# mala-lab/GGAD

Hardware: AMD Instinct MI355X
Metric: training nodes/sec (DGraph-Fin mini-batch GGAD) (higher is better)
Workload: dtype f32; 1 GPU; DGraph-Fin-size synthetic graph, mini-batch GGAD (GCN encoder); nodes=3700550, directed_entries=72953930, feat=17, emb=64, batch=150+50, graph=powerlaw(alpha=2.1,max_degree=2000), chunk_batches=150, hop2=ldsw, overlap=False, dense_cus=0, chain=0, dense_steps=XCD-resident chunk kernel: one launch per chunk on 28 CUs of one XCD, parallelism=dp1, optimizer=adam(lr=1e-3,wd=0.007), batch_streams=the reference's stream

## Files before the change

### ggad_amd/_lib.py

```python
from __future__ import annotations

import ctypes
import os
from ctypes import POINTER, c_char_p, c_float, c_int32, c_int64, c_uint32, c_uint64, c_void_p

HERE = os.path.dirname(os.path.abspath(__file__))
LIB_PATH = os.environ.get("GGAD_LIB_PATH") or os.path.join(HERE, "libggad_hip.so")


class GgadLibraryError(RuntimeError):
    pass


GGAD_OK, GGAD_E_INVALID, GGAD_E_LAUNCH, GGAD_E_CAPACITY, GGAD_E_UNSUPPORTED = 0, -1, -2, -3, -4


class GgadKernelError(RuntimeError):
    pass


GEMM_ROUTES = ("NONE", "SLAB", "BRES", "WGRAD_TN", "SMALL", "DMA", "DMA_SPLITK", "TILED", "TILED_SPLITK")


def gemm_last_route():
    v = int(load().ggad_gemm_last_route())
    return GEMM_ROUTES[v & 0xFF], v >> 8


ABI_VERSION = 11
_P = c_void_p
EXCHANGE_CB = ctypes.CFUNCTYPE(c_int32, c_void_p)
_I = c_int32
_L = c_int64
_F = c_float

SIGNATURES = {
    "ggad_abi_version": (c_int32, []),
    "ggad_last_error": (c_char_p, []),
    "ggad_max_embed_dim": (c_int32, []),
    "ggad_max_feat_dim": (c_int32, []),
    "ggad_mb_wide_max_embed_dim": (c_int32, []),
    "ggad_mb_wide_supported": (c_int32, [c_int32, c_int32]),
    "ggad_mb_supported": (c_int32, [c_int32, c_int32]),
    "ggad_scan_workspace_elems": (c_int64, [_L]),
    "ggad_exclusive_scan_i32": (c_int32, [_P, _P, _L, _P, _P]),
    "ggad_mb_chunk_len": (c_int32, []),
    "ggad_mb_slice_len": (c_int32, []),
    "ggad_mb_group_words": (c_int32, []),
    "ggad_mb_item_words": (c_int32, []),
    "ggad_mb_set_gather_options": (c_int32, [c_int32, c_int32]),
    "ggad_mb_plan_counter_elems": (c_int32, []),
    "ggad_mb_plan_build": (c_int32, [_P, _P, _P, _I, _P, _P, _P, _P, _P, _P]),
    "ggad_event_create": (c_int32, [_I, _P]),
    "ggad_event_destroy": (c_int32, [_P]),
    "ggad_event_record": (c_int32, [_P, _P]),
    "ggad_event_synchronize": (c_int32, [_P]),
    "ggad_event_elapsed_ms": (c_int32, [_P, _P, _P]),
    "ggad_mb_count2": (c_int32, [_P, _P, _P, _P, _P, _L, _L, _P, _P, _P]),
    "ggad_mb_gather2": (c_int32, [_P, _P, _P, _I, _I, _P, _P, _P, _P, _L, _L, _P, _P, _P]),
    "ggad_mb_plan_reset": (c_int32, [_P, _P, _P, _P, _P, _P, _L, _L, _P, _P, _I, _P]),
    "ggad_mb_tile_offsets_elems": (c_int64, [_L, _I]),
    "ggad_mb_tile_offsets": (c_int32, [_P, _P, _L, _I, _P, _P]),
    "ggad_mb_tile_major_workspace_elems": (c_int64, [_L, _I]),
    "ggad_mb_tile_major": (c_int32, [_P, _P, _L, _I, _P, _P, _P, _P, _P]),
    "ggad_mb_ldsw_tile_shift": (c_int32, []),
    "ggad_mb_ldsw_max_owners": (c_int32, []),
    "ggad_mb_ldsw_seg_elems": (c_int64, [_L, _L]),
    "ggad_mb_dw_part_elems": (c_int64, [_I, _I, _I]),
    "ggad_mb_train_chunk": (c_int32, [_P, _I, _P, _P, _P, _P, _I, _I, _P]),
    "ggad_mb_train_chunk_dp": (c_int32, [_P, _I, _P, _P, _P, _P, _I, c_float, EXCHANGE_CB, _P, _P]),
    "ggad_stream_create_cu_mask": (c_int32, [_P, _I, _P]),
    "ggad_stream_destroy": (c_int32, [_P]),
    "ggad_device_cu_count": (c_int32, [_I, _P]),
    "ggad_xchg_create": (c_int32, [_I, _I, _L, _P]),
    "ggad_xchg_handle_bytes": (c_int32, []),
    "ggad_xchg_handle": (c_int32, [_P, _P]),
    "ggad_xchg_connect": (c_int32, [_P, _P]),
    "ggad_xchg_error": (c_int32, [_P, _P]),
    "ggad_xchg_destroy": (c_int32, [_P]),
    "ggad_xchg_adam": (c_int32, [_P, _P, _P, _P, _I, _I, _F, _F, _F, _P, _P, _P]),
    "ggad_mb_train_chunk_xchg": (c_int32, [_P, _I, _P, _P, _P, _P, _I, c_float, _P, _P]),
    "ggad_mb_xcd_grid": (c_int32, []),
    "ggad_xcd_first_of_stream": (c_int32, [_P, _P]),
    "ggad_mb_xcd_workspace_elems": (c_int64, [_I, _I, _I, _L, _L]),
    "ggad_mb_train_chunk_xcd": (c_int32, [_P, _I, _P, _I, _I, _I, _I, _L, _L, _P, _I, _P, c_float, _P, _I, _P, _P]),
    "ggad_mb_xcd_record_elems": (c_int64, [_L, _L]),
    "ggad_mb_xcd_prepare": (c_int32, [_P, _I, _P, _I, _I, _I, _L, _L, _P, _P]),
    "ggad_mb_xcd_status": (c_int32, [_P, _P, _P]),
    "ggad_mb_xcd_clear_error": (c_int32, [_P, _I, _P]),
    "ggad_mb_param_count": (c_int64, [_I, _I]),
    "ggad_mb_param_block_elems": (c_int64, [_I, _I]),
    "ggad_mb_params_sync": (c_int32, [_P, _I, _I, _P]),
    "ggad_mb_project": (c_int32, [_P, _I, _I, _P, _P, _I, _I, _P, _P]),
    "ggad_mb_fwd_rows": (c_int32, [_P, _I, _I, _P, _P, _P, _P, _P, _I, _I, _I, _P, _P, _P, _P]),
    "ggad_mb_loss_workspace_elems": (c_int64, [_I]),
    "ggad_mb_loss": (c_int32, [_P, _I, _I, _P, _P, _P, _P, _P, _P, _P, _I, _I, _P, _P, _P, _P, _P, _P, _P, _P, _P, _P]),
    "ggad_mb_row_coefs": (c_int32, [_P, _I, _I, _P, _P, _I, _I, _P, _P, _P, _P, _P, _P, _P, _P, _P]),
    "ggad_mb_bwd_parts": (c_int32, []),
    "ggad_mb_bwd_flat": (c_int32, [_I, _I, _P, _P, _P, _P, _P, _I, _I, _I, _I, _P, _P, _P, _P]),
    "ggad_mb_grad_reduce": (c_int32, [_I, _I, _P, _I, _I, _P, _P, _P, _P, _P, _P, _P]),
    "ggad_mb_adam": (c_int32, [_P, _P, _P, _P, _I, _I, _F, _F, _F, _P, _P]),
    "ggad_mb_train_step": (c_int32, [_P, _I, _P]),
    "ggad_mb_encode": (c_int32, [_P, _I, _I, _P, _I, _P, _P]),
    "ggad_seg_mean": (c_int32, [_P, _I, _P, _P, _I, _P, _P]),
    "ggad_seg_wsum": (c_int32, [_P, _I, _P, _P, _P, _I, _P, _P]),
# ... 277 lines not shown
```

### ggad_amd/build.py

```python
from __future__ import annotations

import hashlib
import os
import shutil
import subprocess
import sys

HERE = os.path.dirname(os.path.abspath(__file__))
CSRC = os.path.join(HERE, "csrc")
LIB = os.path.join(HERE, "libggad_hip.so")
STAMP = os.path.join(HERE, ".libggad_hip.stamp")
SOURCES = ["runtime.cpp", "plan_build.cpp", "exchange.cpp", "sampler.cpp", "sampler_x86.cpp", "spmm_panel_build.cpp", "spmm_ring_build.cpp", "plan.hip", "hop2_ldsw.hip", "step.hip", "step_wide.hip", "step_xcd.hip", "fullgraph.hip", "gemm.hip", "gemm_slab.hip", "mlp.hip", "baselines.hip", "anomalydae.hip", "aegis.hip", "gaan.hip", "dominant.hip", "rng.hip", "pcgnn.hip", "pcgnn_head.hip", "sage.hip", "aegis_mb.hip", "recon_mb.hip", "tam.hip", "tam_nsgt.hip", "rank_metrics.hip", "topk.hip", "select.hip", "explain.hip"]
HOST_ONLY = {"sampler.cpp", "sampler_x86.cpp", "spmm_panel_build.cpp", "spmm_ring_build.cpp"}
HEADERS = ["common.h", "handoff.h", "step_common.h", "rank_common.h", "libggad_hip.map", os.path.join("..", "..", "include", "ggad_hip.h")]
FLAGS = ["--offload-arch=gfx950", "-O3", "-std=c++17", "-fPIC", "-ffp-contract=on", "-fno-fast-math",
         "-Wall", "-Wno-unused-function"] + os.environ.get("GGAD_EXTRA_HIPFLAGS", "").split()


def _hipcc() -> str:
    for c in (shutil.which("hipcc"), "/opt/rocm/bin/hipcc"):
        if c and os.path.exists(c):
            return c
    raise RuntimeError("hipcc not found; libggad_hip.so cannot be built")


def _digest(srcs) -> str:
    h = hashlib.sha256()
    for name in list(srcs) + HEADERS:
        with open(os.path.join(CSRC, name), "rb") as fh:
            h.update(fh.read())
    h.update(" ".join(FLAGS).encode())
    return h.hexdigest()


def build(force: bool = False, verbose: bool = True) -> str:
    srcs = [s for s in SOURCES if os.path.exists(os.path.join(CSRC, s))]
    dig = _digest(srcs)
    if not force and os.path.exists(LIB) and os.path.exists(STAMP) and open(STAMP).read().strip() == dig:
        return LIB
    hipcc = _hipcc()
    objs = []
    bdir = os.path.join(HERE, "build")
    os.makedirs(bdir, exist_ok=True)
    procs = []
    for s in srcs:
        obj = os.path.join(bdir, os.path.splitext(s)[0] + ".o")
        objs.append(obj)
        if s in HOST_ONLY:
            cmd = [hipcc, "-O3", "-std=c++17", "-fPIC", "-Wall", "-x", "c++", "-c", os.path.join(CSRC, s), "-o", obj]
        else:
            cmd = [hipcc] + FLAGS + ["-x", "hip", "-c", os.path.join(CSRC, s), "-o", obj]
        if verbose:
            print("[ggad build]", " ".join(cmd), flush=True)
        procs.append((s, subprocess.Popen(cmd)))
    for s, p in procs:
        if p.wait() != 0:
            raise RuntimeError(f"hipcc failed on {s}")
    cmd = [hipcc, "--offload-arch=gfx950", "-shared", "-fPIC", "-Wl,--version-script=" + os.path.join(CSRC, "libggad_hip.map"), "-o", LIB] + objs
    if verbose:
        print("[ggad build]", " ".join(cmd), flush=True)
    subprocess.check_call(cmd)
    with open(STAMP, "w") as fh:
        fh.write(dig)
    return LIB


if __name__ == "__main__":
# ... 2 lines not shown
```

### ggad_amd/csrc/common.h

```cpp
#pragma once
#include <hip/hip_runtime.h>
#include <stdint.h>
#include <mutex>
#include "../../include/ggad_hip.h"

#define GGAD_WAVE 64
#define GGAD_MAX_D 64
#define GGAD_MAX_F 1024

void ggad_set_error(hipError_t e, const char *where);

#define GGAD_CHECK_LAUNCH(where)                 \
  do {                                           \
    hipError_t _e = hipGetLastError();           \
    if (_e != hipSuccess) {                      \
      ggad_set_error(_e, where);                 \
      return GGAD_E_LAUNCH;                      \
    }                                            \
  } while (0)

#define GGAD_REQUIRE(cond) \
  do {                     \
    if (!(cond)) return GGAD_E_INVALID; \
  } while (0)
// ... 23 lines not shown
#pragma unroll
  for (int off = 32; off >= 1; off >>= 1) v += __shfl_xor(v, off, GGAD_WAVE);
  return v;
}
__device__ __forceinline__ int wave_sum_i(int v) {
#pragma unroll
  for (int off = 32; off >= 1; off >>= 1) v += __shfl_xor(v, off, GGAD_WAVE);
  return v;
}

__device__ __forceinline__ void ggad_adam_elem(float &pi, float &mi, float &vi, float g, float wd, float sc0, float sc1) {
  float gi = fmaf(wd, pi, g);
  mi = fmaf(gi - mi, 0.1f, mi);
  vi = fmaf(0.001f * gi, gi, vi * 0.999f);
  const float denom = sqrtf(vi) / sc1 + 1e-8f;
  pi = pi - sc0 * (mi / denom);
}

__device__ __forceinline__ int lower_bound_i32(const int32_t *__restrict__ a, int lo, int hi, int key) {
  while (lo < hi) {
    int mid = (lo + hi) >> 1;
    if (a[mid] < key) lo = mid + 1; else hi = mid;
  }
  return lo;
}

__device__ __forceinline__ bool ggad_vblock(int skip, unsigned &vb, unsigned &vg) {
  const unsigned b = blockIdx.x, n = gridDim.x;
  if (skip < 0) { vb = b; vg = n; return true; }
  const unsigned sk = (unsigned)skip;
  if ((b & 7u) == sk) return false;
  vb = b - ((b >> 3) + ((b & 7u) > sk ? 1u : 0u));
  vg = n - ((n >> 3) + ((n & 7u) > sk ? 1u : 0u));
  return true;
}
static inline unsigned ggad_skip_grid(unsigned want, int skip) { return skip < 0 ? want : (unsigned)(((uint64_t)(want + 1) * 8 + 6) / 7); }

constexpr int GGAD_CTR_STRIDE = 16;
constexpr int GGAD_CTR_GROUPS = 0 * GGAD_CTR_STRIDE, GGAD_CTR_ITEMS = 1 * GGAD_CTR_STRIDE, GGAD_CTR_PART = 2 * GGAD_CTR_STRIDE,
              GGAD_CTR_CURSOR = 3 * GGAD_CTR_STRIDE, GGAD_CTR_PC = 4 * GGAD_CTR_STRIDE,
              GGAD_CTR_BIG = 5 * GGAD_CTR_STRIDE,
              GGAD_CTR_RANGE0 = 6 * GGAD_CTR_STRIDE,
              GGAD_CTR_PROF = 14 * GGAD_CTR_STRIDE;
constexpr int GGAD_RANGES = 8;
constexpr int GGAD_RANGE_DEG = 256;
constexpr int GGAD_PLAN_COUNTERS = 16 * GGAD_CTR_STRIDE;

struct ggad_plan_view {
  const int32_t *batch_ptr, *batch_ent_ptr, *nodes, *row_slot, *ent_ptr, *row_ck_ptr, *ck_rc, *ck_e0;
  int32_t n_batches, n_rows, n_ents, n_chunks;
  int32_t seg_stride;
  int64_t pair_bound;
};
int ggad_int_hop1(const ggad_mb_plan *P, const ggad_plan_view &V, int ldsw, int reset_now, hipStream_t st);
int ggad_int_global_hop2(const ggad_mb_plan *P, const ggad_plan_view &V, hipStream_t st, hipEvent_t ev0, hipEvent_t ev1);
int ggad_int_ldsw_hop2(const ggad_mb_plan *P, const ggad_plan_view &V, hipStream_t st, hipEvent_t ev0, hipEvent_t ev1);
int ggad_int_range_deg();

int ggad_int_gemm_slab(const float *A, const float *B, float *C, int M, int N, int K, int64_t lda, int64_t sbk, int64_t sbn, int64_t ldc,
                       const float *bias, int relu, hipStream_t st, const float *prelu_a = nullptr, float *C2 = nullptr, int64_t ldc2 = 0);

int64_t ggad_int_wgrad_tn_ws(int R, int m, int n);
int ggad_int_wgrad_tn(const float *P, int64_t ldp, const float *Q, int64_t ldq, int R, int m, int n, float *D, float *ws, hipStream_t st,
                      int *vpq = nullptr);

constexpr int GGAD_MB_BWD_PARTS = 256;
struct ggad_xchg_view;
bool ggad_int_wide_ok(int D, int F);
int ggad_int_wide_project(const float *params, int32_t D, int32_t F, const float *x2, const int32_t *ent_own, int32_t ent0,
                          int32_t n_ents, float *h2, ggad_stream_t stream);
int ggad_int_wide_fwd_rows(const float *params, int32_t D, int32_t F, const float *x1, const float *h2, const int32_t *ent_ptr,
                           const int32_t *ent_own, const int32_t *labels, int32_t row0, int32_t n_rows, int32_t ent0, float *h1,
                           float *nbar, float *gen, ggad_stream_t stream);
int ggad_int_wide_loss(const float *params, int32_t D, int32_t F, const float *h1, const float *nbar, const float *gen,
                       const int32_t *labels, const int32_t *pos_meta, const int32_t *row_pos, const int32_t *ent_ptr,
                       int32_t row0, int32_t n_rows, float *loss_ws, float *losses8, float *d_h1, float *d_gen, float *d_nbar,
                       float *dz, float *coef_a, float *coef_g, int32_t *step_counter, ggad_stream_t stream);
int ggad_int_wide_row_coefs(const float *params, int32_t D, int32_t F, const int32_t *labels, const int32_t *ent_ptr,
                            int32_t row0, int32_t n_rows, const float *h1, const float *gen, const float *d_h1,
                            const float *d_gen, const float *d_nbar, float *dz, float *coef_a, float *coef_g,
                            ggad_stream_t stream);
int ggad_int_wide_bwd_flat(int32_t D, int32_t F, const float *x1, const float *x2, const float *h2, const int32_t *ent_own,
                           const int32_t *ent_row, int32_t row0, int32_t n_rows, int32_t ent0, int32_t n_ents,
                           const float *coef_a, const float *coef_g, float *dw_part, ggad_stream_t stream);
int ggad_int_wide_grad_reduce(int32_t D, int32_t F, const int32_t *pos_meta, int32_t row0, int32_t n_rows, const float *losses8,
                              const float *nbar, const float *dw_part, const float *dz, const float *loss_ws, float *grads,
                              int mode, float *params, float *m, float *v, float lr, float wd, const int32_t *step_counter,
                              const ggad_xchg_view *xv, uint32_t xstep, float grad_scale, ggad_stream_t stream);
int ggad_int_wide_rows(const float *params, int32_t D, int32_t F, const float *x1, int32_t n_rows, float *out, int score,
                       ggad_stream_t stream);

constexpr int GGAD_XCHG_MAX_WORLD = 16;
struct ggad_xchg_view {
  float *peer[GGAD_XCHG_MAX_WORLD];
  int32_t rank, world;
  int64_t n;
  int32_t *err;
  unsigned long long timeout_ticks;
};
struct ggad_xchg {
  ggad_xchg_view view;
  void *local;
  size_t bytes;
  uint32_t step;
  bool opened[GGAD_XCHG_MAX_WORLD];
};
static inline size_t ggad_xchg_granules(int world, int64_t n) { return (size_t)2 * world * (size_t)n; }
```

### ggad_amd/csrc/hop2_ldsw.hip

```cpp
#include <algorithm>
#include <atomic>
#include <climits>
#include <mutex>

#include "common.h"

namespace {

#ifdef GGAD_G2_PROF
struct G2Prof { unsigned long long a[8], t; };
#define G2_ARG , G2Prof &prof
#define G2_PASS , prof
#define G2_MARK(i) do { __builtin_amdgcn_sched_barrier(0); __builtin_amdgcn_s_waitcnt(0); const unsigned long long t_ = wall_clock64(); \
                        prof.a[i] += t_ - prof.t; prof.t = t_; __builtin_amdgcn_sched_barrier(0); } while (0)
#define TC_MARK(i) do { __syncthreads(); if (threadIdx.x == 0) { const unsigned long long t_ = wall_clock64(); tcp[i] += t_ - tct; tct = t_; } } while (0)
#else
#define G2_ARG
#define G2_PASS
#define G2_MARK(i)
#define TC_MARK(i)
#endif

constexpr int SLICE = 256;
constexpr int GRP_W = 10;
constexpr int ITEM_GRAB = 4;

__global__ void __launch_bounds__(256) k_tile_offsets(const int32_t *__restrict__ rowptr, const int32_t *__restrict__ col,
                                                      int64_t n_nodes, int n_tiles, int shift, int32_t *__restrict__ off) {
  const int64_t u = (int64_t)blockIdx.x * blockDim.x + threadIdx.x;
  if (u >= n_nodes) return;
  const int s = rowptr[u], e = rowptr[u + 1];
  int32_t *o = off + u * (n_tiles + 1);
  int t = 0;
  for (int i = s; i < e; ++i) {
    const int tile = col[i] >> shift;
    while (t <= tile) { o[t] = i - s; ++t; }
  }
  while (t <= n_tiles) { o[t] = e - s; ++t; }
}

__global__ void __launch_bounds__(256) k_tm_blocksum(const int32_t *__restrict__ off, int64_t n_nodes, int n_tiles, int32_t *__restrict__ bsum) {
  __shared__ int wsum[4][64];
  const int lane = lane_id(), w = threadIdx.x >> 6;
  const int NT1 = n_tiles + 1;
  const int64_t u0 = (int64_t)blockIdx.x * 256 + 64 * w;
  for (int t0 = 0; t0 < n_tiles; t0 += 64) {
    const int t = t0 + lane;
    int acc = 0;
    if (t < n_tiles)
      for (int i = 0; i < 64 && u0 + i < n_nodes; ++i) { const int32_t *o = off + (u0 + i) * NT1 + t; acc += o[1] - o[0]; }
    wsum[w][lane] = acc;
    __syncthreads();
    if (w == 0 && t < n_tiles) bsum[(int64_t)blockIdx.x * n_tiles + t] = wsum[0][lane] + wsum[1][lane] + wsum[2][lane] + wsum[3][lane];
    __syncthreads();
  }
}

__global__ void __launch_bounds__(1024) k_tm_scan(int32_t *__restrict__ bsum, int64_t n_blocks, int n_tiles, int32_t *__restrict__ tile_base) {
// ... 10 lines not shown
    }
    for (; b < n_blocks; ++b) { const int v = bsum[b * n_tiles + t]; bsum[b * n_tiles + t] = run; run += v; }
    tot[t] = run;
  }
  __syncthreads();
  if (threadIdx.x == 0) {
    int run = 0;
    for (int t = 0; t < n_tiles; ++t) { tile_base[t] = run; run += tot[t]; }
    tile_base[n_tiles] = run;
  }
}

__global__ void __launch_bounds__(256) k_tm_fill(const int32_t *__restrict__ rowptr, const int32_t *__restrict__ col,
                                                 const int32_t *__restrict__ off, int64_t n_nodes, int n_tiles,
                                                 const int32_t *__restrict__ bsum, const int32_t *__restrict__ tile_base,
                                                 int32_t *__restrict__ tile_start, int32_t *__restrict__ col_t) {
  __shared__ int wsum[4][64];
  const int lane = lane_id(), w = threadIdx.x >> 6;
  const int NT1 = n_tiles + 1;
  const int64_t u0 = (int64_t)blockIdx.x * 256 + 64 * w;
  for (int t0 = 0; t0 <= n_tiles; t0 += 64) {
    const int t = t0 + lane;
    int acc = 0;
    if (t < n_tiles)
      for (int i = 0; i < 64 && u0 + i < n_nodes; ++i) { const int32_t *o = off + (u0 + i) * NT1 + t; acc += o[1] - o[0]; }
    wsum[w][lane] = acc;
    __syncthreads();
    if (t < n_tiles) {
      int pos = tile_base[t] + bsum[(int64_t)blockIdx.x * n_tiles + t];
      for (int ww = 0; ww < w; ++ww) pos += wsum[ww][lane];
      for (int i = 0; i < 64 && u0 + i < n_nodes; ++i) {
        const int64_t u = u0 + i;
        const int32_t *o = off + u * NT1 + t;
        const int o0 = o[0], o1 = o[1];
        tile_start[u * NT1 + t] = pos;
        const int32_t *src = col + rowptr[u] + o0;
        for (int j = 0; j < o1 - o0; ++j) col_t[pos + j] = src[j];
        pos += o1 - o0;
      }
    } else if (t == n_tiles) {
      for (int i = 0; i < 64 && u0 + i < n_nodes; ++i) tile_start[(u0 + i) * NT1 + t] = 0;
    }
    __syncthreads();
  }
}

constexpr int TW_SHIFT = 15;
constexpr int TW_TILE = 1 << TW_SHIFT;
constexpr int TW_MAXOWN = 6144;
constexpr int TW_T = 1024;
constexpr int TW_BRK = 1536;

constexpr int TT_SLAB = 128;
__global__ void __launch_bounds__(256) k_seg_transpose(const int32_t *__restrict__ tile_off, const int32_t *__restrict__ tile_start,
                                                       int n_tiles, const int32_t *__restrict__ ent_own,
                                                       const int32_t *__restrict__ ent_col, int n_ents, int64_t seg_stride,
                                                       int32_t *__restrict__ seg_t, int skip) {
  __shared__ int tl[TT_SLAB][65];
  unsigned vbx, vgx;
  if (!ggad_vblock(skip, vbx, vgx)) return;
  const int p0 = vbx * 64;
  if (p0 >= n_ents) return;
  const int lane = lane_id(), wid = threadIdx.x >> 6;
  const int NT1 = n_tiles + 1;
  int u_l = 0, own_l = 0;
  if (p0 + lane < n_ents) { own_l = ent_own[p0 + lane] == p0 + lane ? 1 : 0; u_l = own_l ? ent_col[p0 + lane] : 0; }
  for (int which = 0; which < (tile_start ? 2 : 1); ++which) {
  const int32_t *table = which ? tile_start : tile_off;
  int32_t *plane = seg_t + (which ? (int64_t)NT1 * seg_stride : 0);
  for (int t0 = 0; t0 < NT1; t0 += TT_SLAB) {
    int v0[16], v1[16];
    const int c0 = min(t0 + lane, NT1 - 1), c1 = min(t0 + 64 + lane, NT1 - 1);
#pragma unroll
    for (int jj = 0; jj < 16; ++jj) {
      const int j = wid + 4 * jj;
      const int u = __shfl(u_l, j, GGAD_WAVE);
      const int32_t *row = table + (int64_t)u * NT1;
      v0[jj] = row[c0];
      v1[jj] = row[c1];
    }
#pragma unroll
    for (int jj = 0; jj < 16; ++jj) {
      const int j = wid + 4 * jj;
      const int own = __shfl(own_l, j, GGAD_WAVE);
      if (t0 + lane < NT1) tl[lane][j] = own ? v0[jj] : 0;
      if (t0 + 64 + lane < NT1) tl[64 + lane][j] = own ? v1[jj] : 0;
    }
    __syncthreads();
    const int nt = min(TT_SLAB, NT1 - t0);
    for (int idx = threadIdx.x; idx < nt * 64; idx += 256) {
      const int tt = idx >> 6, j = idx & 63;
      if (p0 + j < n_ents) plane[(int64_t)(t0 + tt) * seg_stride + p0 + j] = tl[tt][j];
    }
    __syncthreads();
  }
  }
}

__device__ __forceinline__ int block_excl_scan_1024(int v, int *warp_buf, int *total) {
  const int lane = lane_id(), wid = threadIdx.x >> 6;
  int inc = v;
#pragma unroll
  for (int off = 1; off < 64; off <<= 1) {
    const int t = __shfl_up(inc, off, 64);
    if (lane >= off) inc += t;
  }
  if (lane == 63) warp_buf[wid] = inc;
  __syncthreads();
  int base = 0, tot = 0;
#pragma unroll
  for (int w = 0; w < 16; ++w) { const int sv = warp_buf[w]; if (w < wid) base += sv; tot += sv; }
  __syncthreads();
  *total = tot;
  return base + inc - v;
}

__global__ void __launch_bounds__(TW_T) k_tile_counts(const int32_t *__restrict__ col, const int32_t *__restrict__ seg_t,
                                                      int64_t n_cap, const int32_t *__restrict__ own_rp,
                                                      const int32_t *__restrict__ batch_ent_ptr,
                                                      const int32_t *__restrict__ pw_base, uint16_t *__restrict__ pc, int n_tiles,
                                                      int n_batches, int32_t *__restrict__ counters, int skip, int tile_major) {
  extern __shared__ __attribute__((aligned(16))) uint32_t lds_u[];
  uint32_t *cnt = lds_u;
  int *offs = reinterpret_cast<int *>(lds_u + TW_TILE / 2);
  int *segbeg = offs + TW_MAXOWN + 1;
  int *dst = segbeg + TW_MAXOWN;
  int *brk = dst + TW_MAXOWN;
  __shared__ int wbuf[16];
  unsigned vbx, vgx;
  if (!ggad_vblock(skip, vbx, vgx)) return;
  int t, b;
  const bool class_map = (tile_major & 2) != 0;
  tile_major &= 1;
  if (class_map) {
    const int nx = skip < 0 ? 8 : 7, c = (int)(blockIdx.x & 7u);
    const int ci = c - ((skip >= 0 && c > skip) ? 1 : 0);
    const unsigned j = blockIdx.x >> 3;
    const int nt_c = ci < n_tiles ? (n_tiles - ci + nx - 1) / nx : 0;
    if (j >= (unsigned)nt_c * (unsigned)n_batches) return;
    t = ci + nx * (int)(j / (unsigned)n_batches);
    b = (int)(j % (unsigned)n_batches);
  } else {
    if (vbx >= (unsigned)n_tiles * (unsigned)n_batches) return;
    t = (int)(vbx % (unsigned)n_tiles); b = (int)(vbx / (unsigned)n_tiles);
  }
  const int o0 = batch_ent_ptr[b], o1 = batch_ent_ptr[b + 1];
  const int n_own_all = o1 - o0;
  const int32_t *seg_lo = seg_t + (int64_t)t * n_cap, *seg_hi = seg_lo + n_cap;
  const int32_t *seg_st = tile_major ? seg_t + (int64_t)(n_tiles + 1 + t) * n_cap : own_rp;
// ... 286 lines not shown
    const bool mine = blk + lane < n1;
    lids[lane] = k_nx;
    __builtin_amdgcn_fence(__ATOMIC_RELEASE, "wavefront");
    __builtin_amdgcn_wave_barrier();
    int id[16];
#pragma unroll
    for (int c = 0; c < 4; ++c) {
      const mi4 iv = *reinterpret_cast<const mi4 *>(lids + 16 * g + 4 * c);
#pragma unroll
      for (int q = 0; q < 4; ++q) id[4 * c + q] = iv[q];
    }
    mf2 x[16];
#pragma unroll
    for (int i = 0; i < 16; ++i) x[i] = *reinterpret_cast<const mf2 *>(fb + ((uint32_t)id[i] << 7));
#pragma unroll
    for (int j = 0; j < G; ++j)
      lw[j * MF_WS + lane] = (j < n_occ && mine) ? inv_sr / sqrtf((float)c_nx[j]) : 0.0f;
    __builtin_amdgcn_fence(__ATOMIC_RELEASE, "wavefront");
    __builtin_amdgcn_wave_barrier();
    float wa[16];
#pragma unroll
    for (int c = 0; c < 4; ++c) {
      const mf4 wv = *reinterpret_cast<const mf4 *>(lw + aa * MF_WS + 16 * g + 4 * c);
#pragma unroll
      for (int q = 0; q < 4; ++q) wa[4 * c + q] = a < G ? wv[q] : 0.0f;
    }
    __builtin_amdgcn_wave_barrier();
    {
      const int ix = min(blk + 64 + lane, last);
      k_nx = col[s + ix];
#pragma unroll
      for (int j = 0; j < G; ++j) c_nx[j] = pc[pb[j] + ix];
    }
    G2_MARK(3);
#pragma unroll
    for (int i = 0; i < 16; ++i) {
      acc0 = __builtin_amdgcn_mfma_f32_16x16x4f32(wa[i], x[i].x, acc0, 0, 0, 0);
      acc1 = __builtin_amdgcn_mfma_f32_16x16x4f32(wa[i], x[i].y, acc1, 0, 0, 0);
    }
    G2_MARK(4);
  }
#pragma unroll
  for (int j = 0; j < G; ++j) {
    const int src = (lane >> 1) + 16 * (j >> 2);
    const float v0 = __shfl(acc0[j & 3], src & 63, GGAD_WAVE), v1 = __shfl(acc1[j & 3], src & 63, GGAD_WAVE);
    tot[j] = (lane & 1) ? v1 : v0;
  }
}

__device__ __forceinline__ int range_tile(int r, int n_tiles) { return (int)(((int64_t)r * n_tiles) / GGAD_RANGES); }

__global__ void __launch_bounds__(256) k_build_groups(const int32_t *__restrict__ ent_own, const int32_t *__restrict__ ent_col,
                                                      const int32_t *__restrict__ own_deg, int n_ents,
                                                      int32_t *__restrict__ node_head, const int32_t *__restrict__ own_next,
                                                      const int32_t *__restrict__ tile_off, int n_tiles,
                                                      int32_t *__restrict__ grp, int32_t *__restrict__ items,
                                                      int32_t *__restrict__ big, int32_t *__restrict__ gbnd,
                                                      int32_t *__restrict__ counters, int range_deg, int skip) {
  unsigned vbx, vgx;
  if (!ggad_vblock(skip, vbx, vgx)) return;
  const int e = vbx * 256 + threadIdx.x;
  const int lane = lane_id();
  int u = 0, m = 0, ng = 0, ns = 0, deg = 0;
  if (e < n_ents && ent_own[e] == e) {
    u = ent_col[e];
    if (node_head[u] == e + 1) {
      for (int cur = e + 1; cur != 0; cur = own_next[cur - 1]) ++m;
      ng = (m + 7) >> 3;
      deg = own_deg[e];
      ns = deg > range_deg ? GGAD_RANGES : (deg > SLICE ? (deg + SLICE - 1) / SLICE : 1);
    }
  }
  const bool is_big = deg > range_deg;
  const int c1 = is_big ? 0 : ng * ns, c2 = ns > 1 ? m * ns : 0, c3 = is_big ? ng : 0;
  int v0 = ng, v1 = c1, v2 = c2, v3 = c3;
#pragma unroll
  for (int off = 1; off < GGAD_WAVE; off <<= 1) {
    const int t0 = __shfl_up(v0, off, GGAD_WAVE), t1 = __shfl_up(v1, off, GGAD_WAVE), t2 = __shfl_up(v2, off, GGAD_WAVE),
              t3 = __shfl_up(v3, off, GGAD_WAVE);
    if (lane >= off) { v0 += t0; v1 += t1; v2 += t2; v3 += t3; }
  }
  __shared__ int wg_tot[4][5];
  const int wid = threadIdx.x >> 6;
  if (lane == GGAD_WAVE - 1) { wg_tot[0][wid] = v0; wg_tot[1][wid] = v1; wg_tot[2][wid] = v2; wg_tot[3][wid] = v3; }
  __syncthreads();
  if (threadIdx.x < 4) {
    const int k = threadIdx.x;
    int sum = 0;
    for (int w = 0; w < 4; ++w) { const int t = wg_tot[k][w]; wg_tot[k][w] = sum; sum += t; }
    int32_t *ctr = counters + (k == 0 ? GGAD_CTR_GROUPS : (k == 1 ? GGAD_CTR_ITEMS : (k == 2 ? GGAD_CTR_PART : GGAD_CTR_BIG)));
    wg_tot[k][4] = sum > 0 ? atomicAdd(ctr, sum) : 0;
  }
  __syncthreads();
  const int b0 = wg_tot[0][4] + wg_tot[0][wid], b1 = wg_tot[1][4] + wg_tot[1][wid], b2 = wg_tot[2][4] + wg_tot[2][wid],
            b3 = wg_tot[3][4] + wg_tot[3][wid];
  if (ng == 0) return;
  const int gbase = b0 + v0 - ng, ibase = b1 + v1 - c1, pbase = b2 + v2 - c2, bbase = b3 + v3 - c3;
  int bnd[GGAD_RANGES + 1];
  if (is_big) {
    const int32_t *row = tile_off + (int64_t)u * (n_tiles + 1);
#pragma unroll
    for (int r = 0; r <= GGAD_RANGES; ++r) bnd[r] = row[range_tile(r, n_tiles)];
  }
  int cur = e + 1;
  for (int g = 0; g < ng; ++g) {
    int32_t *rec = grp + (int64_t)(gbase + g) * GRP_W;
#pragma unroll
    for (int j = 0; j < 8; ++j) {
      int v = -1;
      if (cur != 0) { v = cur - 1; cur = own_next[v]; }
      rec[j] = v;
    }
    rec[8] = pbase + g * 8 * ns;
    rec[9] = ns;
    if (is_big) {
      big[bbase + g] = gbase + g;
      int32_t *bo = gbnd + (int64_t)(bbase + g) * (GGAD_RANGES + 1);
#pragma unroll
      for (int r = 0; r <= GGAD_RANGES; ++r) bo[r] = bnd[r];
    } else {
      for (int sl = 0; sl < ns; ++sl) {
        int32_t *it = items + (int64_t)(ibase + sl * ng + g) * 2;
        it[0] = gbase + g;
        it[1] = sl;
      }
    }
  }
  node_head[u] = 0;
}

template <int FT, bool MF>
__global__ void __launch_bounds__(256) k_gather2_items(const int32_t *__restrict__ col, const float *__restrict__ feat, int F_rt,
                                                       int stride, const int32_t *__restrict__ own_rp,
                                                       const int32_t *__restrict__ own_deg, const int32_t *__restrict__ pw_base,
                                                       const uint16_t *__restrict__ pc, const int32_t *__restrict__ grp,
                                                       const int32_t *__restrict__ items, const int32_t *__restrict__ big,
                                                       const int32_t *__restrict__ gbnd, int32_t *__restrict__ counters,
                                                       float *__restrict__ x2, float *__restrict__ part2, int affine, int take_cap, int skip) {
  static_assert(ITEM_GRAB == 4 && GRP_W <= 10, "lane layout of the metadata loads: 16 lanes per item of a grab (10, 11: range bounds)");
  unsigned vbx, vgx;
  if (!ggad_vblock(skip, vbx, vgx)) return;
  const int F = FT ? FT : F_rt;
  const int lane = lane_id();
  __shared__ __attribute__((aligned(16))) float mf_lds[MF ? 4 * MF_LDS : 4];
  float *lw = mf_lds + (MF ? (threadIdx.x >> 6) * MF_LDS : 0);
  const int n_small = counters[GGAD_CTR_ITEMS], n_big = counters[GGAD_CTR_BIG];
  const int q_l = lane >> 4, r_l = lane & 15;
  unsigned xcc;
  asm volatile("s_getreg_b32 %0, hwreg(HW_REG_XCC_ID)" : "=s"(xcc));
  xcc &= GGAD_RANGES - 1;
  if (!affine) xcc = (vbx / GGAD_RANGES) & (GGAD_RANGES - 1);
  const int n_waves_all = (int)vgx * 4;
#ifdef GGAD_G2_PROF
  G2Prof prof = {};
  const unsigned long long t_begin = wall_clock64();
  prof.t = t_begin;
#endif
  for (int ph = 0; ph <= GGAD_RANGES; ++ph) {
    const int cls = ph == 0 ? (int)xcc : (ph == 1 ? GGAD_RANGES : (int)((xcc + ph - 1) & (GGAD_RANGES - 1)));
    const bool bigc = cls < GGAD_RANGES;
    const int n_items = bigc ? n_big : n_small;
    if (n_items == 0) continue;
    int32_t *cursor = counters + (bigc ? GGAD_CTR_RANGE0 + cls * GGAD_CTR_STRIDE : GGAD_CTR_CURSOR);
// ... 45 lines not shown
#pragma unroll
      for (int j = 0; j < 8; ++j) {
        e[j] = __builtin_amdgcn_readlane(rv, q * 16 + j);
        pb[j] = __builtin_amdgcn_readlane(pbv, q * 16 + j);
        n += e[j] >= 0 ? 1 : 0;
      }
      const int pbase = __builtin_amdgcn_readlane(rv, q * 16 + 8), ns = __builtin_amdgcn_readlane(rv, q * 16 + 9);
      const int sl = __builtin_amdgcn_readlane(iv, q * 16 + 1);
      int s, n0, n1, deg;
      item_span(q, s, n0, n1, deg);
      const float inv_sr = 1.0f / sqrtf((float)deg);
      const int k_first = k_ahead;
      if (q + 1 < ITEM_GRAB && base + q + 1 < last) {
        int s_, a_, b_, d_;
        item_span(q + 1, s_, a_, b_, d_);
        k_ahead = first_ids(s_, a_, b_);
      }
      float tot[8];
      if (MF) {
        if (n == 1) { float t1[1]; gather_slice_mfma<1>(col, feat, s, n0, n1, inv_sr, n, pb, pc, lane, lw, k_first, t1 G2_PASS); tot[0] = t1[0]; }
        else if (n == 2) { float t2[2]; gather_slice_mfma<2>(col, feat, s, n0, n1, inv_sr, n, pb, pc, lane, lw, k_first, t2 G2_PASS); tot[0] = t2[0]; tot[1] = t2[1]; }
        else if (n <= 4) { float t4[4]; gather_slice_mfma<4>(col, feat, s, n0, n1, inv_sr, n, pb, pc, lane, lw, k_first, t4 G2_PASS);
#pragma unroll
          for (int j = 0; j < 4; ++j) tot[j] = t4[j]; }
        else gather_slice_mfma<8>(col, feat, s, n0, n1, inv_sr, n, pb, pc, lane, lw, k_first, tot G2_PASS);
      } else
      if (n == 1) { float t1[1]; gather_slice<1, FT>(col, feat, F, stride, s, n0, n1, inv_sr, n, pb, pc, lane, k_first, t1 G2_PASS); tot[0] = t1[0]; }
      else if (n == 2) { float t2[2]; gather_slice<2, FT>(col, feat, F, stride, s, n0, n1, inv_sr, n, pb, pc, lane, k_first, t2 G2_PASS); tot[0] = t2[0]; tot[1] = t2[1]; }
      else if (n <= 4) { float t4[4]; gather_slice<4, FT>(col, feat, F, stride, s, n0, n1, inv_sr, n, pb, pc, lane, k_first, t4 G2_PASS);
#pragma unroll
        for (int j = 0; j < 4; ++j) tot[j] = t4[j]; }
      else gather_slice<8, FT>(col, feat, F, stride, s, n0, n1, inv_sr, n, pb, pc, lane, k_first, tot G2_PASS);
#pragma unroll
      for (int j = 0; j < 8; ++j) {
        if (j < n && lane < F) {
          if (ns == 1) x2[(int64_t)e[j] * F + lane] = (deg == 0) ? inv_sr * 0.0f : tot[j];
          else part2[((int64_t)pbase + (int64_t)j * ns + sl) * F + lane] = tot[j];
        }
      }
      G2_MARK(5);
    }
    }
  }
  }
#ifdef GGAD_G2_PROF
  if (lane == 0) {
    prof.a[6] = wall_clock64() - t_begin;
    unsigned long long *out = reinterpret_cast<unsigned long long *>(counters + GGAD_CTR_PROF);
    for (int k = 0; k < 7; ++k) atomicAdd(out + k, prof.a[k]);
  }
#endif
}

__global__ void __launch_bounds__(256) k_gather2_combine(const int32_t *__restrict__ grp, const int32_t *__restrict__ counters,
                                                         const float *__restrict__ part2, int F, float *__restrict__ x2, int skip) {
  unsigned vbx, vgx;
  if (!ggad_vblock(skip, vbx, vgx)) return;
  const int lane = lane_id();
  const int n_groups = counters[GGAD_CTR_GROUPS];
  const int rpi = 64 / F;
  const int g = lane / F, f = lane - g * F;
  for (int gi = vbx * 4 + (threadIdx.x >> 6); gi < n_groups; gi += vgx * 4) {
    const int rv = (lane < GRP_W) ? grp[(int64_t)gi * GRP_W + lane] : -1;
    const int ns = __builtin_amdgcn_readlane(rv, 9);
    if (ns <= 1) continue;
    const int pbase = __builtin_amdgcn_readlane(rv, 8);
    for (int j0 = 0; j0 < 8; j0 += rpi) {
      const int j = j0 + g;
      const int ej = __shfl(rv, j & 7, GGAD_WAVE);
      if (g < rpi && j < 8 && ej >= 0) {
        float acc = 0.0f;
#pragma unroll 4
        for (int sl = 0; sl < ns; ++sl) acc += part2[((int64_t)pbase + (int64_t)j * ns + sl) * F + f];
        x2[(int64_t)ej * F + f] = acc;
      }
    }
  }
}

__global__ void __launch_bounds__(256) k_gather2_w(const int32_t *__restrict__ col, const float *__restrict__ feat, int F, int stride,
                                                   const int32_t *__restrict__ ent_own, int n_ents,
                                                   const int32_t *__restrict__ own_rp, const int32_t *__restrict__ own_deg,
                                                   const int32_t *__restrict__ pw_base, const uint16_t *__restrict__ pc,
                                                   float *__restrict__ x2, int skip) {
  unsigned vbx, vgx;
  if (!ggad_vblock(skip, vbx, vgx)) return;
  const int e0 = vbx * 4 + (threadIdx.x >> 6);
  if (e0 >= n_ents || ent_own[e0] != e0) return;
  const int lane = lane_id();
  const int s = own_rp[e0];
  const int deg = own_deg[e0];
  const int pb0 = pw_base[e0];
  const float inv_sr = 1.0f / sqrtf((float)deg);
  if (F <= 64) {
    const int pb[8] = {pb0, 0, 0, 0, 0, 0, 0, 0};
    float total = 0.0f;
#ifdef GGAD_G2_PROF
    G2Prof prof = {};
#endif
    for (int n0 = 0; n0 < deg; n0 += SLICE) {
      float t1[1];
      const int kf = col[s + min(n0 + lane, max(min(deg, n0 + SLICE) - 1, 0))];
      if (F == 17) gather_slice<1, 17>(col, feat, F, stride, s, n0, min(deg, n0 + SLICE), inv_sr, 1, pb, pc, lane, kf, t1 G2_PASS);
      else gather_slice<1, 0>(col, feat, F, stride, s, n0, min(deg, n0 + SLICE), inv_sr, 1, pb, pc, lane, kf, t1 G2_PASS);
      total += t1[0];
    }
    if (deg == 0) total = inv_sr * 0.0f;
    if (lane < F) x2[(int64_t)e0 * F + lane] = total;
    return;
  }
  for (int fbase = 0; fbase < F; fbase += 64) {
    const int fw = min(64, F - fbase);
    float total = 0.0f;
    for (int n0 = 0; n0 < deg; n0 += SLICE) {
      const int n1 = min(deg, n0 + SLICE);
      float acc = 0.0f;
      for (int blk = n0; blk < n1; blk += 64) {
        const int idx = blk + lane;
        int k = 0;
        float w = 0.0f;
        if (idx < n1) { k = col[s + idx]; w = inv_sr / sqrtf((float)pc[pb0 + idx]); }
        const int count = min(64, n1 - blk);
        for (int t = 0; t < count; ++t) {
          const int kk = __shfl(k, t, GGAD_WAVE);
          const float ws = __shfl(w, t, GGAD_WAVE);
          const float x = lane < fw ? feat[(int64_t)kk * stride + fbase + lane] : 0.0f;
          acc = fmaf(ws, x, acc);
        }
      }
      total += acc;
    }
    if (deg == 0) total = inv_sr * 0.0f;
    if (lane < fw) x2[(int64_t)e0 * F + fbase + lane] = total;
  }
}

std::atomic<int> g_mfma_batches{[] { const char *e = getenv("GGAD_GATHER_MFMA_BATCHES"); return e ? atoi(e) : 0; }()};
std::atomic<int> g_range_deg{[] { const char *e = getenv("GGAD_RANGE_DEG"); return e ? atoi(e) : 0; }()};

}

int ggad_int_range_deg() { return g_range_deg.load() > 0 ? std::max(g_range_deg.load(), GGAD_RANGE_DEG) : INT32_MAX; }

int ggad_int_ldsw_hop2(const ggad_mb_plan *P, const ggad_plan_view &V, hipStream_t st, hipEvent_t ev0, hipEvent_t ev1) {
  if (V.n_ents == 0 || V.n_batches == 0) return GGAD_OK;
  const int n_tiles = (int)((P->n_nodes + TW_TILE - 1) >> TW_SHIFT);
  const int skip = P->xcd_skip >= 0 && P->xcd_skip < 8 ? P->xcd_skip : -1;
  const bool tile_major = P->tile_start != nullptr && P->col_t != nullptr;
  k_seg_transpose<<<dim3(ggad_skip_grid((unsigned)((V.n_ents + 63) / 64), skip)), dim3(256), 0, st>>>(
      P->tile_off, tile_major ? P->tile_start : nullptr, n_tiles, P->ent_own, P->ent_col, V.n_ents, V.seg_stride, P->seg_t, skip);
  const size_t lds = (size_t)(TW_TILE / 2) * 4 + (size_t)(3 * TW_MAXOWN + 1) * 4 + (size_t)TW_BRK * 4;
  {
    static std::mutex mu;
    static int state[64] = {};
    int dev = 0;
    if (hipGetDevice(&dev) != hipSuccess || dev < 0 || dev >= 64) return GGAD_E_INVALID;
    std::lock_guard<std::mutex> lock(mu);
    if (state[dev] == 0) {
      const bool ok = hipFuncSetAttribute((const void *)k_tile_counts, hipFuncAttributeMaxDynamicSharedMemorySize, (int)lds) == hipSuccess;
      (void)hipGetLastError();
      state[dev] = ok ? 1 : -1;
    }
    if (state[dev] != 1) { ggad_set_error(hipErrorInvalidValue, "mb_plan_build: this device cannot give k_tile_counts its LDS"); return GGAD_E_LAUNCH; }
  }
  if (P->ev_tile0) (void)hipEventRecord(static_cast<hipEvent_t>(P->ev_tile0), st);
  static const int tc_map = [] { const char *e = getenv("GGAD_TC_MAP"); return e ? atoi(e) : -1; }();
  const bool class_map = tc_map >= 0 ? tc_map != 0 : tile_major;
  const unsigned tc_grid = class_map ? 8u * (unsigned)((n_tiles + (skip < 0 ? 8 : 7) - 1) / (skip < 0 ? 8 : 7)) * (unsigned)V.n_batches
                                      : ggad_skip_grid((unsigned)n_tiles * (unsigned)V.n_batches, skip);
  k_tile_counts<<<dim3(tc_grid), dim3(TW_T), lds, st>>>(tile_major ? P->col_t : P->col, P->seg_t, V.seg_stride, P->own_rp, V.batch_ent_ptr,
                                                        P->pw_base, P->pc, n_tiles, V.n_batches, P->counters, skip, (tile_major ? 1 : 0) | (class_map ? 2 : 0));
  if (P->ev_tile1) (void)hipEventRecord(static_cast<hipEvent_t>(P->ev_tile1), st);
  if (ev0) (void)hipEventRecord(ev0, st);
  const int F = P->feat_dim;
  if (P->node_major && F <= 64) {
    const int range_deg = ggad_int_range_deg();
    static const int affine = [] { const char *e = getenv("GGAD_RANGE_AFFINE"); return e ? atoi(e) : 1; }();
    int32_t *big = P->items + 2 * (int64_t)P->item_cap, *gbnd = P->items + 3 * (int64_t)P->item_cap;
    k_build_groups<<<dim3(ggad_skip_grid((unsigned)((V.n_ents + 255) / 256), skip)), dim3(256), 0, st>>>(
        P->ent_own, P->ent_col, P->own_deg, V.n_ents, P->node_head, P->own_next, P->tile_off, n_tiles, P->grp, P->items, big, gbnd,
        P->counters, range_deg, skip);
    const int64_t max_items = (int64_t)V.n_ents + (V.pair_bound > 0 ? V.pair_bound : P->pair_cap) / SLICE;
    static const int env_wg = [] { const char *e = getenv("GGAD_G2_WG_PER_CU"); return e ? atoi(e) : 0; }();
    static const int env_cap = [] { const char *e = getenv("GGAD_G2_TAKE_CAP"); return e ? atoi(e) : 0; }();
    const bool small_launch = V.n_batches <= 32;
    const int wg_per_cu = env_wg > 0 ? env_wg : (small_launch ? 3 : 4);
    const int take_cap = env_cap > 0 ? env_cap : (small_launch ? 8 : 12);
    const unsigned wgs = (unsigned)std::min<int64_t>((max_items + 4 * ITEM_GRAB - 1) / (4 * ITEM_GRAB), 256 * wg_per_cu);
    if (F == 17 && P->feat_stride == 32 && V.n_batches >= g_mfma_batches.load())
      k_gather2_items<17, true><<<dim3(ggad_skip_grid(wgs, skip)), dim3(256), 0, st>>>(P->col, P->feat, F, P->feat_stride, P->own_rp, P->own_deg,
                                                                                       P->pw_base, P->pc, P->grp, P->items, big, gbnd, P->counters,
                                                                                       P->x2, P->part2, affine, take_cap, skip);
    else if (F == 17)
      k_gather2_items<17, false><<<dim3(ggad_skip_grid(wgs, skip)), dim3(256), 0, st>>>(P->col, P->feat, F, P->feat_stride, P->own_rp, P->own_deg,
                                                                                 P->pw_base, P->pc, P->grp, P->items, big, gbnd, P->counters,
                                                                                 P->x2, P->part2, affine, take_cap, skip);
    else
      k_gather2_items<0, false><<<dim3(ggad_skip_grid(wgs, skip)), dim3(256), 0, st>>>(P->col, P->feat, F, P->feat_stride, P->own_rp, P->own_deg,
                                                                                P->pw_base, P->pc, P->grp, P->items, big, gbnd, P->counters,
                                                                                P->x2, P->part2, affine, take_cap, skip);
    const unsigned cg = (unsigned)std::min<int64_t>(((int64_t)V.n_ents + 3) / 4, 16384);
    k_gather2_combine<<<dim3(ggad_skip_grid(cg, skip)), dim3(256), 0, st>>>(P->grp, P->counters, P->part2, F, P->x2, skip);
  } else {
    k_gather2_w<<<dim3(ggad_skip_grid((unsigned)((V.n_ents + 3) / 4), skip)), dim3(256), 0, st>>>(
        P->col, P->feat, F, P->feat_stride, P->ent_own, V.n_ents, P->own_rp, P->own_deg, P->pw_base, P->pc, P->x2, skip);
  }
  if (ev1) (void)hipEventRecord(ev1, st);
  GGAD_CHECK_LAUNCH("mb_plan_build (ldsw 2-hop)");
  return GGAD_OK;
}

extern "C" {

int ggad_mb_ldsw_tile_shift(void) { return TW_SHIFT; }
int ggad_mb_ldsw_max_owners(void) { return TW_MAXOWN; }
int32_t ggad_mb_slice_len(void) { return SLICE; }
int32_t ggad_mb_group_words(void) { return GRP_W; }
int ggad_mb_set_gather_options(int32_t mfma_min_batches, int32_t range_deg) {
  if (mfma_min_batches >= 0) g_mfma_batches.store(mfma_min_batches);
  if (range_deg >= 0) g_range_deg.store(range_deg);
  return GGAD_OK;
}
int32_t ggad_mb_item_words(void) { return 3 + GGAD_RANGES + 1; }
int32_t ggad_mb_plan_counter_elems(void) { return GGAD_PLAN_COUNTERS; }
int64_t ggad_mb_tile_offsets_elems(int64_t n_nodes, int32_t tile_shift) {
  return n_nodes * (((n_nodes + (1LL << tile_shift) - 1) >> tile_shift) + 1);
}
int64_t ggad_mb_ldsw_seg_elems(int64_t n_nodes, int64_t n_entries_cap) {
  return 2 * (((n_nodes + TW_TILE - 1) >> TW_SHIFT) + 1) * ((n_entries_cap + 63) / 64 * 64);
}

int ggad_mb_tile_offsets(const int32_t *rowptr, const int32_t *col, int64_t n_nodes, int32_t tile_shift, int32_t *tile_off,
                         ggad_stream_t stream) {
  GGAD_REQUIRE(rowptr && col && tile_off && n_nodes >= 0 && tile_shift >= 8 && tile_shift <= 24);
  if (n_nodes == 0) return GGAD_OK;
  const int n_tiles = (int)((n_nodes + (1LL << tile_shift) - 1) >> tile_shift);
  k_tile_offsets<<<dim3((unsigned)((n_nodes + 255) / 256)), dim3(256), 0, as_stream(stream)>>>(rowptr, col, n_nodes, n_tiles,
                                                                                               tile_shift, tile_off);
  GGAD_CHECK_LAUNCH("mb_tile_offsets");
  return GGAD_OK;
}


int64_t ggad_mb_tile_major_workspace_elems(int64_t n_nodes, int32_t tile_shift) {
  if (n_nodes < 0 || tile_shift < 8 || tile_shift > 24) return 0;
  const int64_t n_tiles = (n_nodes + (1LL << tile_shift) - 1) >> tile_shift;
  return ((n_nodes + 255) / 256) * n_tiles + n_tiles + 1;
}

int ggad_mb_tile_major(const int32_t *rowptr, const int32_t *col, int64_t n_nodes, int32_t tile_shift, const int32_t *tile_off,
                       int32_t *tile_start, int32_t *col_t, int32_t *workspace, ggad_stream_t stream) {
  GGAD_REQUIRE(rowptr && col && tile_off && tile_start && col_t && workspace && n_nodes >= 0 && tile_shift >= 8 && tile_shift <= 24);
  if (n_nodes == 0) return GGAD_OK;
  const int n_tiles = (int)((n_nodes + (1LL << tile_shift) - 1) >> tile_shift);
  const int64_t n_blocks = (n_nodes + 255) / 256;
// ... 12 lines not shown
```

### ggad_amd/csrc/plan.hip

```cpp
#include "common.h"

namespace {

constexpr int SCAN_T = 256;
constexpr int SCAN_ITEMS = 8;
constexpr int SCAN_TILE = SCAN_T * SCAN_ITEMS;

__device__ __forceinline__ int block_exclusive_scan(int v, int *total) {
  __shared__ int wsum[SCAN_T / GGAD_WAVE];
  const int lane = lane_id(), wid = threadIdx.x / GGAD_WAVE;
  int inc = v;
#pragma unroll
  for (int off = 1; off < GGAD_WAVE; off <<= 1) {
    int t = __shfl_up(inc, off, GGAD_WAVE);
    if (lane >= off) inc += t;
  }
  if (lane == GGAD_WAVE - 1) wsum[wid] = inc;
  __syncthreads();
  int base = 0, tot = 0;
#pragma unroll
  for (int w = 0; w < SCAN_T / GGAD_WAVE; ++w) {
    int s = wsum[w];
    if (w < wid) base += s;
    tot += s;
  }
  __syncthreads();
  *total = tot;
  return base + inc - v;
}

__global__ void __launch_bounds__(SCAN_T) scan_tile_sums(const int32_t *__restrict__ in, int64_t n, int32_t *__restrict__ tile_sum) {
  const int64_t base = (int64_t)blockIdx.x * SCAN_TILE + (int64_t)threadIdx.x * SCAN_ITEMS;
  int s = 0;
#pragma unroll
  for (int i = 0; i < SCAN_ITEMS; ++i) s += (base + i < n) ? in[base + i] : 0;
  int tot;
  block_exclusive_scan(s, &tot);
  if (threadIdx.x == 0) tile_sum[blockIdx.x] = tot;
}

__global__ void __launch_bounds__(SCAN_T) scan_tile_offsets(int32_t *__restrict__ tile_sum, int n_tiles, int32_t *__restrict__ total_out) {
  int v[SCAN_ITEMS];
  const int base = threadIdx.x * SCAN_ITEMS;
  int s = 0;
#pragma unroll
  for (int i = 0; i < SCAN_ITEMS; ++i) { v[i] = (base + i < n_tiles) ? tile_sum[base + i] : 0; s += v[i]; }
  int tot;
  int ex = block_exclusive_scan(s, &tot);
#pragma unroll
  for (int i = 0; i < SCAN_ITEMS; ++i) { if (base + i < n_tiles) tile_sum[base + i] = ex; ex += v[i]; }
  if (threadIdx.x == 0) *total_out = tot;
}

__global__ void __launch_bounds__(SCAN_T) scan_apply(const int32_t *__restrict__ in, int32_t *__restrict__ out, int64_t n,
                                                     const int32_t *__restrict__ tile_off) {
  const int64_t base = (int64_t)blockIdx.x * SCAN_TILE + (int64_t)threadIdx.x * SCAN_ITEMS;
  int v[SCAN_ITEMS];
  int s = 0;
#pragma unroll
  for (int i = 0; i < SCAN_ITEMS; ++i) { v[i] = (base + i < n) ? in[base + i] : 0; s += v[i]; }
  int tot;
  int ex = block_exclusive_scan(s, &tot) + tile_off[blockIdx.x];
#pragma unroll
  for (int i = 0; i < SCAN_ITEMS; ++i) { if (base + i < n) out[base + i] = ex; ex += v[i]; }
}

__device__ __forceinline__ void gather_block(const float *__restrict__ feat, int F, int fbase, int rpi, int g, int f,
                                             bool lane_active, int j, float w, int count, float &acc) {
  const int iters = (count + rpi - 1) / rpi;
  int t = 0;
  for (; t + 4 <= iters; t += 4) {
    float x[4], ww[4];
#pragma unroll
    for (int u = 0; u < 4; ++u) {
      const int src = (t + u) * rpi + g;
      const int jj = __shfl(j, src & 63, GGAD_WAVE);
      const float ws = __shfl(w, src & 63, GGAD_WAVE);
      ww[u] = (src < count) ? ws : 0.0f;
      x[u] = (lane_active && src < count) ? feat[(int64_t)jj * F + fbase + f] : 0.0f;
    }
#pragma unroll
    for (int u = 0; u < 4; ++u) acc = fmaf(ww[u], x[u], acc);
  }
  for (; t < iters; ++t) {
    const int src = t * rpi + g;
    const int jj = __shfl(j, src & 63, GGAD_WAVE);
    const float ws = __shfl(w, src & 63, GGAD_WAVE);
    const float ww = (src < count) ? ws : 0.0f;
    const float x = (lane_active && src < count) ? feat[(int64_t)jj * F + fbase + f] : 0.0f;
    acc = fmaf(ww, x, acc);
  }
}

__device__ __forceinline__ float reduce_groups(float acc, int F, int rpi) {
  float tot = acc;
  for (int gg = 1; gg < rpi; ++gg) tot += __shfl(acc, (lane_id() + gg * F) & 63, GGAD_WAVE);
  return tot;
}

__global__ void __launch_bounds__(256) k_expand(const int32_t *__restrict__ rowptr, const int32_t *__restrict__ col,
                                                const int32_t *__restrict__ nodes, const int32_t *__restrict__ row_slot,
                                                const int32_t *__restrict__ ent_ptr, const int32_t *__restrict__ ck_rc,
                                                const int32_t *__restrict__ ck_e0, int n_chunks, int64_t n_nodes,
                                                int32_t *__restrict__ ent_col, int32_t *__restrict__ ent_slot,
                                                int32_t *__restrict__ ent_row, int32_t *__restrict__ cnt1,
                                                int32_t *__restrict__ own1, int32_t *__restrict__ counters, int skip) {
  unsigned vbx, vgx;
  if (!ggad_vblock(skip, vbx, vgx)) return;
  if (vbx == 0 && threadIdx.x < GGAD_PLAN_COUNTERS && counters != nullptr) counters[threadIdx.x] = 0;
  const int ck = (int)((vbx * 256u + threadIdx.x) >> 4);
  const int i = threadIdx.x & 15;
  if (ck >= n_chunks) return;
  const int rc = ck_rc[ck];
  if (i >= (rc & 63)) return;
  const int row = rc >> 6;
  const int e = ck_e0[ck] + i;
  const int e_row = ent_ptr[row];
  const int r = ent_ptr[row + 1] - e_row;
  const int idx = e - e_row;
  const int v = nodes[row];
  const int s = rowptr[v];
  const int deg = rowptr[v + 1] - s;
  int j;
  if (r == deg) {
    j = col[s + idx];
  } else {
    const int a = idx > 0 ? col[s + idx - 1] : -1;
    const int b = idx < deg ? col[s + idx] : 0x7fffffff;
    j = (b < v) ? b : (a < v ? v : a);
  }
  const int slot = row_slot[row];
  ent_col[e] = j;
  ent_slot[e] = slot;
  ent_row[e] = row;
  const int64_t soff = (int64_t)slot * n_nodes;
  const int old = atomicAdd(&cnt1[soff + j], 1);
  if (old == 0) own1[soff + j] = e;
}

__global__ void __launch_bounds__(256) k_gather1c(const float *__restrict__ feat, int F, int stride,
                                                  const int32_t *__restrict__ row_slot, const int32_t *__restrict__ ent_ptr,
                                                  const int32_t *__restrict__ row_ck_ptr, const int32_t *__restrict__ ck_rc,
                                                  const int32_t *__restrict__ ck_e0, int n_chunks, int64_t n_nodes,
                                                  const int32_t *__restrict__ cnt1, const int32_t *__restrict__ own1,
                                                  const int32_t *__restrict__ ent_col, int32_t *__restrict__ ent_own,
                                                  int32_t *__restrict__ ent_c1, float *__restrict__ part1, int pstride,
                                                  float *__restrict__ x1, const int32_t *__restrict__ rowptr,
                                                  int32_t *__restrict__ own_deg, int32_t *__restrict__ own_rp,
                                                  int32_t *__restrict__ pw_base, int32_t *__restrict__ node_head,
                                                  int32_t *__restrict__ own_next, int32_t *__restrict__ counters, int ldsw, int skip) {
// ... 59 lines not shown
  for (int c4 = 0; c4 < 4; ++c4) {
    const int len_c = __shfl(len, c4 * 16, GGAD_WAVE);
    if (len_c == 0) continue;
    const int row_c = __shfl(row, c4 * 16, GGAD_WAVE);
    const bool single = (row_ck_ptr[row_c + 1] - row_ck_ptr[row_c]) == 1;
    const int iters = (len_c + rpi - 1) / rpi;
    for (int fc = 0; fc < fchunks; ++fc) {
      const int fbase = fc * 64;
      const int fw = F <= 64 ? F : min(64, F - fbase);
      const int g = lane / fw, f = lane - g * fw;
      const bool act = g < rpi;
      const int gl = act ? g : rpi - 1;
      const int fo = act ? f : 0;
      float acc = 0.0f;
      int t = 0;
      for (; t + 6 <= iters; t += 6) {
        float x[6], ww[6];
#pragma unroll
        for (int q = 0; q < 6; ++q) {
          const int si = (t + q) * rpi + g;
          const int jj = __shfl(j, (c4 * 16 + (t + q) * rpi + gl) & 63, GGAD_WAVE);
          const float ws = __shfl(w, (c4 * 16 + si) & 63, GGAD_WAVE);
          ww[q] = (act && si < len_c) ? ws : 0.0f;
          x[q] = feat[(int64_t)jj * stride + fbase + fo];
        }
#pragma unroll
        for (int q = 0; q < 6; ++q) acc = fmaf(ww[q], ww[q] != 0.0f ? x[q] : 0.0f, acc);
      }
      for (; t < iters; ++t) {
        const int si = t * rpi + g;
        const int jj = __shfl(j, (c4 * 16 + t * rpi + gl) & 63, GGAD_WAVE);
        const float ws = __shfl(w, (c4 * 16 + si) & 63, GGAD_WAVE);
        const float wv = (act && si < len_c) ? ws : 0.0f;
        const float x = feat[(int64_t)jj * stride + fbase + fo];
        acc = fmaf(wv, wv != 0.0f ? x : 0.0f, acc);
      }
      const float tot = (F <= 64) ? reduce_groups(acc, fw, rpi) : acc;
      if (lane < fw) {
        if (single) x1[(int64_t)row_c * F + fbase + lane] = tot;
        else part1[(int64_t)(wave * 4 + c4) * pstride + fbase + lane] = tot;
      }
    }
  }
}

__global__ void __launch_bounds__(256) k_combine1_reset(int row_blocks, int n_rows, const int32_t *__restrict__ row_ck_ptr,
                                                        const float *__restrict__ part1, int pstride, int F,
                                                        float *__restrict__ x1, int do_reset, int n_ents,
                                                        const int32_t *__restrict__ ent_col,
                                                        const int32_t *__restrict__ ent_slot, int64_t n_nodes,
                                                        int32_t *__restrict__ cnt1, int skip) {
  unsigned vbx, vgx;
  if (!ggad_vblock(skip, vbx, vgx)) return;
  if ((int)vbx >= row_blocks) {
    if (!do_reset) return;
    const int e = (vbx - row_blocks) * 256 + threadIdx.x;
    if (e < n_ents) cnt1[(int64_t)ent_slot[e] * n_nodes + ent_col[e]] = 0;
    return;
  }
  const int row = vbx * 4 + (threadIdx.x >> 6);
  if (row >= n_rows) return;
  const int c0 = row_ck_ptr[row];
  const int nck = row_ck_ptr[row + 1] - c0;
  if (nck <= 1) return;
  const int lane = lane_id();
  const int rpi = F <= 64 ? 64 / F : 1;
  const int fchunks = F <= 64 ? 1 : (F + 63) / 64;
  for (int fc = 0; fc < fchunks; ++fc) {
    const int fbase = fc * 64;
    const int fw = F <= 64 ? F : min(64, F - fbase);
    const int g = lane / fw, f = lane - g * fw;
    float acc = 0.0f;
    if (g < rpi) {
      const float *__restrict__ src = part1 + (int64_t)c0 * pstride + fbase + f;
      int c = g;
      for (; c + 7 * rpi < nck; c += 8 * rpi) {
        float v[8];
#pragma unroll
        for (int u = 0; u < 8; ++u) v[u] = src[(int64_t)(c + u * rpi) * pstride];
#pragma unroll
        for (int u = 0; u < 8; ++u) acc += v[u];
      }
      for (; c < nck; c += rpi) acc += src[(int64_t)c * pstride];
    }
    const float tot = (F <= 64) ? reduce_groups(acc, fw, rpi) : acc;
    if (lane < fw) x1[(int64_t)row * F + fbase + lane] = tot;
  }
}

__global__ void __launch_bounds__(256) k_seg_mean(const float *__restrict__ feat, int F, const int32_t *__restrict__ seg_ptr,
                                                  const int32_t *__restrict__ seg_col, const float *__restrict__ seg_w,
                                                  int n_rows, float *__restrict__ out) {
  const int row = blockIdx.x * (blockDim.x / GGAD_WAVE) + threadIdx.x / GGAD_WAVE;
  if (row >= n_rows) return;
  const int lane = lane_id();
  const int e0 = seg_ptr[row], e1 = seg_ptr[row + 1];
  const int r = e1 - e0;
  const float inv = 1.0f / (float)r;
  const int rpi = F <= 64 ? 64 / F : 1;
  const int fchunks = F <= 64 ? 1 : (F + 63) / 64;
  for (int fc = 0; fc < fchunks; ++fc) {
    const int fbase = fc * 64;
    const int fw = F <= 64 ? F : min(64, F - fbase);
    const int g = lane / fw, f = lane - g * fw;
    const bool lane_active = g < rpi;
    float acc = 0.0f;
    for (int blk = 0; blk < r; blk += GGAD_WAVE) {
      const int idx = blk + lane;
      int j = 0; float w = 0.0f;
      if (idx < r) { j = seg_col[e0 + idx]; w = seg_w ? seg_w[e0 + idx] : inv; }
      gather_block(feat, F, fbase, rpi, g, f, lane_active, j, w, min(GGAD_WAVE, r - blk), acc);
    }
    float tot = (F <= 64) ? reduce_groups(acc, fw, rpi) : acc;
    if (r == 0) tot = inv * 0.0f;
    if (lane < fw) out[(int64_t)row * F + fbase + lane] = tot;
  }
}

__global__ void __launch_bounds__(256) k_count2(const int32_t *__restrict__ rowptr, const int32_t *__restrict__ col,
                                                const int32_t *__restrict__ ent_col, const int32_t *__restrict__ ent_slot,
                                                const int32_t *__restrict__ ent_total, int64_t n_nodes,
                                                const int32_t *__restrict__ own1, int32_t *__restrict__ cnt2) {
  const int e = blockIdx.x * (blockDim.x / GGAD_WAVE) + threadIdx.x / GGAD_WAVE;
  if (e >= *ent_total) return;
  const int u = ent_col[e];
  const int64_t soff = (int64_t)ent_slot[e] * n_nodes;
  if (own1[soff + u] != e) return;
  const int s = rowptr[u], t = rowptr[u + 1];
  for (int i = s + lane_id(); i < t; i += GGAD_WAVE) atomicAdd(&cnt2[soff + col[i]], 1);
}

__global__ void __launch_bounds__(256) k_gather2(const int32_t *__restrict__ rowptr, const int32_t *__restrict__ col,
                                                 const float *__restrict__ feat, int F, int stride, const int32_t *__restrict__ ent_col,
                                                 const int32_t *__restrict__ ent_slot, const int32_t *__restrict__ ent_own,
                                                 const int32_t *__restrict__ ent_total, int64_t n_nodes,
                                                 const int32_t *__restrict__ cnt2, float *__restrict__ x2) {
  const int e = blockIdx.x * (blockDim.x / GGAD_WAVE) + threadIdx.x / GGAD_WAVE;
  if (e >= *ent_total) return;
  if (ent_own[e] != e) return;
  const int lane = lane_id();
  const int u = ent_col[e];
  const int64_t soff = (int64_t)ent_slot[e] * n_nodes;
  const int s = rowptr[u], t = rowptr[u + 1];
  const int deg = t - s;
  const float inv_sr = 1.0f / sqrtf((float)deg);
  const int rpi = F <= 64 ? 64 / F : 1;
  const int fchunks = F <= 64 ? 1 : (F + 63) / 64;
  for (int fc = 0; fc < fchunks; ++fc) {
    const int fbase = fc * 64;
    const int fw = F <= 64 ? F : min(64, F - fbase);
    const int g = lane / fw, f = lane - g * fw;
    const bool lane_active = g < rpi;
    float acc = 0.0f;
    for (int blk = 0; blk < deg; blk += GGAD_WAVE) {
      const int idx = blk + lane;
      int k = 0; float w = 0.0f;
      if (idx < deg) {
        k = col[s + idx];
        w = inv_sr / sqrtf((float)cnt2[soff + k]);
      }
      gather_block(feat, stride, fbase, rpi, g, f, lane_active, k, w, min(GGAD_WAVE, deg - blk), acc);
    }
    float tot = (F <= 64) ? reduce_groups(acc, fw, rpi) : acc;
    if (deg == 0) tot = inv_sr * 0.0f;
    if (lane < fw) x2[(int64_t)e * F + fbase + lane] = tot;
  }
}

__global__ void __launch_bounds__(256) k_plan_reset(const int32_t *__restrict__ rowptr, const int32_t *__restrict__ col,
                                                    const int32_t *__restrict__ ent_col, const int32_t *__restrict__ ent_slot,
                                                    const int32_t *__restrict__ ent_own, const int32_t *__restrict__ ent_total,
                                                    int64_t n_nodes, int32_t *__restrict__ cnt1, int32_t *__restrict__ cnt2,
                                                    int with_hop2) {
  const int e = blockIdx.x * (blockDim.x / GGAD_WAVE) + threadIdx.x / GGAD_WAVE;
  if (e >= *ent_total) return;
  const int u = ent_col[e];
  const int64_t soff = (int64_t)ent_slot[e] * n_nodes;
  if (lane_id() == 0) cnt1[soff + u] = 0;
  if (!with_hop2 || ent_own[e] != e) return;
  const int s = rowptr[u], t = rowptr[u + 1];
  for (int i = s + lane_id(); i < t; i += GGAD_WAVE) cnt2[soff + col[i]] = 0;
}

}

int ggad_int_hop1(const ggad_mb_plan *P, const ggad_plan_view &V, int ldsw, int reset_now, hipStream_t st) {
  if (V.n_chunks == 0) return GGAD_OK;
  const unsigned eb = (unsigned)((V.n_chunks + 15) / 16);
  const int skip = P->xcd_skip >= 0 && P->xcd_skip < 8 ? P->xcd_skip : -1;
  if (ldsw && !(P->node_major && P->feat_dim <= 64)) ldsw = 2;
  k_expand<<<dim3(ggad_skip_grid(eb, skip)), dim3(256), 0, st>>>(P->rowptr, P->col, V.nodes, V.row_slot, V.ent_ptr, V.ck_rc, V.ck_e0, V.n_chunks,
                                            P->n_nodes, P->ent_col, P->ent_slot, P->ent_row, P->cnt1, P->own1, P->counters, skip);
  k_gather1c<<<dim3(ggad_skip_grid(eb, skip)), dim3(256), 0, st>>>(P->feat, P->feat_dim, P->feat_stride, V.row_slot, V.ent_ptr, V.row_ck_ptr, V.ck_rc,
                                              V.ck_e0, V.n_chunks, P->n_nodes, P->cnt1, P->own1, P->ent_col, P->ent_own, P->ent_c1,
                                              P->ck_part, P->ck_part_stride, P->x1, P->rowptr, P->own_deg, P->own_rp, P->pw_base,
                                              P->node_head, P->own_next, P->counters, ldsw, skip);
  const int row_blocks = (V.n_rows + 3) / 4;
  const int ent_blocks = reset_now ? (V.n_ents + 255) / 256 : 0;
  k_combine1_reset<<<dim3(ggad_skip_grid((unsigned)(row_blocks + ent_blocks), skip)), dim3(256), 0, st>>>(
      row_blocks, V.n_rows, V.row_ck_ptr, P->ck_part, P->ck_part_stride, P->feat_dim, P->x1, reset_now, V.n_ents, P->ent_col,
      P->ent_slot, P->n_nodes, P->cnt1, skip);
  GGAD_CHECK_LAUNCH("mb_plan_build (1-hop)");
  return GGAD_OK;
}

int ggad_int_global_hop2(const ggad_mb_plan *P, const ggad_plan_view &V, hipStream_t st, hipEvent_t ev0, hipEvent_t ev1) {
  if (V.n_ents == 0) return GGAD_OK;
  const int32_t *tot = V.ent_ptr + V.n_rows;
  ggad_stream_t s = reinterpret_cast<ggad_stream_t>(st);
  int rc = ggad_mb_count2(P->rowptr, P->col, P->ent_col, P->ent_slot, tot, V.n_ents, P->n_nodes, P->own1, P->cnt2, s);
  if (rc) return rc;
  if (ev0) (void)hipEventRecord(ev0, st);
  rc = ggad_mb_gather2(P->rowptr, P->col, P->feat, P->feat_dim, P->feat_stride, P->ent_col, P->ent_slot, P->ent_own, tot, V.n_ents,
                       P->n_nodes, P->cnt2, P->x2, s);
  if (rc) return rc;
  if (ev1) (void)hipEventRecord(ev1, st);
  const double walk_bytes = (double)V.n_ents * (double)P->mean_nbr_deg * 64.0;
  const bool memset_cnt2 = walk_bytes > (double)V.n_batches * (double)P->n_nodes * 8.0;
  if (memset_cnt2) {
    const hipError_t me = hipMemsetAsync(P->cnt2, 0, (size_t)V.n_batches * (size_t)P->n_nodes * sizeof(int32_t), st);
    if (me != hipSuccess) { ggad_set_error(me, "mb_plan_build (memset cnt2)"); return GGAD_E_LAUNCH; }
  }
  return ggad_mb_plan_reset(P->rowptr, P->col, P->ent_col, P->ent_slot, P->ent_own, tot, V.n_ents, P->n_nodes, P->cnt1, P->cnt2,
                            memset_cnt2 ? 0 : 1, s);
}

extern "C" {

int64_t ggad_scan_workspace_elems(int64_t n) { return (n + SCAN_TILE - 1) / SCAN_TILE + 1; }

int ggad_exclusive_scan_i32(const int32_t *in, int32_t *out, int64_t n, int32_t *workspace, ggad_stream_t stream) {
  GGAD_REQUIRE(in && out && workspace && n >= 0);
  const int64_t tiles = (n + SCAN_TILE - 1) / SCAN_TILE;
  GGAD_REQUIRE(tiles <= SCAN_TILE);
  hipStream_t st = as_stream(stream);
  if (n == 0) {
    (void)hipMemsetAsync(out, 0, sizeof(int32_t), st);
    GGAD_CHECK_LAUNCH("scan memset");
    return GGAD_OK;
  }
  scan_tile_sums<<<dim3((unsigned)tiles), dim3(SCAN_T), 0, st>>>(in, n, workspace);
  scan_tile_offsets<<<dim3(1), dim3(SCAN_T), 0, st>>>(workspace, (int)tiles, out + n);
  scan_apply<<<dim3((unsigned)tiles), dim3(SCAN_T), 0, st>>>(in, out, n, workspace);
  GGAD_CHECK_LAUNCH("exclusive_scan");
  return GGAD_OK;
}

int32_t ggad_mb_chunk_len(void) { return 16; }

// ... 54 lines not shown
```

### ggad_amd/csrc/plan_build.cpp

```cpp
#include <algorithm>
#include <chrono>
#include <cstdint>
#include <cstdio>
#include <cstdlib>
#include <cstring>
#include <vector>

#include "common.h"

namespace {
inline int64_t align4(int64_t x) { return (x + 3) & ~(int64_t)3; }
}

extern "C" {

int ggad_event_create(int32_t timing, void **out) {
  if (!out) return GGAD_E_INVALID;
  hipEvent_t ev = nullptr;
  const hipError_t e = hipEventCreateWithFlags(&ev, timing ? hipEventDefault : hipEventDisableTiming);
  if (e != hipSuccess) { ggad_set_error(e, "event_create"); return GGAD_E_LAUNCH; }
  *out = ev;
  return GGAD_OK;
}
int ggad_event_destroy(void *event) {
  if (!event) return GGAD_OK;
  const hipError_t e = hipEventDestroy(static_cast<hipEvent_t>(event));
  if (e != hipSuccess) { ggad_set_error(e, "event_destroy"); return GGAD_E_LAUNCH; }
  return GGAD_OK;
}
int ggad_event_record(void *event, ggad_stream_t stream) {
  if (!event) return GGAD_E_INVALID;
  const hipError_t e = hipEventRecord(static_cast<hipEvent_t>(event), as_stream(stream));
  if (e != hipSuccess) { ggad_set_error(e, "event_record"); return GGAD_E_LAUNCH; }
  return GGAD_OK;
}
int ggad_event_synchronize(void *event) {
  if (!event) return GGAD_E_INVALID;
  const hipError_t e = hipEventSynchronize(static_cast<hipEvent_t>(event));
  if (e != hipSuccess) { ggad_set_error(e, "event_synchronize"); return GGAD_E_LAUNCH; }
  return GGAD_OK;
}
int ggad_event_elapsed_ms(void *start, void *stop, float *ms_host) {
  if (!start || !stop || !ms_host) return GGAD_E_INVALID;
  const hipError_t e = hipEventElapsedTime(ms_host, static_cast<hipEvent_t>(start), static_cast<hipEvent_t>(stop));
  if (e != hipSuccess) { ggad_set_error(e, "event_elapsed_ms"); return GGAD_E_LAUNCH; }
  return GGAD_OK;
}

int ggad_mb_plan_build(const ggad_mb_plan *P, const int64_t *nodes_host, const int32_t *batch_ptr_host, int32_t n_batches,
                       const int64_t *labels_host, ggad_mb_plan_info *info, int64_t *ent_ptr_host_out,
                       int64_t *batch_ent_ptr_host_out, int32_t *batch_max_row_host_out, ggad_stream_t stream) {
  GGAD_REQUIRE(P && nodes_host && batch_ptr_host && info);
  GGAD_REQUIRE(P->rowptr && P->col && P->feat && P->closed_deg_host && P->stage_host && P->stage && P->stage_event);
  GGAD_REQUIRE(P->cnt1 && P->own1 && P->ent_col && P->ent_slot && P->ent_row && P->ent_own && P->ent_c1 && P->x1 && P->ck_part);
  GGAD_REQUIRE(P->feat_dim >= 1 && P->feat_dim <= GGAD_MAX_F && P->feat_stride >= P->feat_dim && P->n_nodes >= 1);
  GGAD_REQUIRE(P->ck_part_stride >= (P->feat_dim < 64 ? 64 : P->feat_dim));
  GGAD_REQUIRE(n_batches >= 1 && n_batches <= P->max_batches && batch_ptr_host[0] == 0);
  const bool train = P->train != 0;
  if (train) GGAD_REQUIRE(labels_host && P->x2 && (P->hop2 == 1 || P->hop2 == 2));
  std::memset(info, 0, sizeof(*info));
  static const bool timing = getenv("GGAD_BUILD_TIMING") != nullptr;
  const auto tt0 = std::chrono::steady_clock::now();
  const int nb = n_batches;
  const int64_t rows = batch_ptr_host[nb];
  GGAD_REQUIRE(rows >= 1 && rows < (1 << 25));
  for (int b = 0; b < nb; ++b) GGAD_REQUIRE(batch_ptr_host[b + 1] > batch_ptr_host[b]);
  const int CL = 16;
  const int SL = ggad_mb_slice_len();

  int64_t n_ents = 0, n_chunks = 0, bound = 0;
  int64_t max_batch_ents = 0;
  const bool want_ldsw = train && P->hop2 == 1;
  if (want_ldsw) GGAD_REQUIRE(P->pair_bound_host && P->tile_off && P->own_deg && P->own_rp && P->pw_base && P->node_head &&
                              P->own_next && P->grp && P->counters);
  static thread_local std::vector<int32_t> row_deg;
  if ((int64_t)row_deg.size() < rows) row_deg.resize((size_t)rows);
  constexpr int PF = 24;
  const int64_t *pack = P->node_pack_host;
  constexpr int64_t PACK_MASK = (1LL << 40) - 1;
  for (int64_t i = 0; i < rows && i < PF; ++i) {
    const int64_t v = nodes_host[i];
    GGAD_REQUIRE(v >= 0 && v < P->n_nodes);
    if (pack) { __builtin_prefetch(&pack[v]); continue; }
    __builtin_prefetch(&P->closed_deg_host[v]);
    if (want_ldsw) __builtin_prefetch(&P->pair_bound_host[v]);
  }
  for (int b = 0; b < nb; ++b) {
    int64_t be = 0;
    for (int64_t i = batch_ptr_host[b]; i < batch_ptr_host[b + 1]; ++i) {
      if (i + PF < rows) {
        const int64_t vn = nodes_host[i + PF];
        GGAD_REQUIRE(vn >= 0 && vn < P->n_nodes);
        if (pack) __builtin_prefetch(&pack[vn]);
        else {
          __builtin_prefetch(&P->closed_deg_host[vn]);
          if (want_ldsw) __builtin_prefetch(&P->pair_bound_host[vn]);
        }
      }
      const int64_t v = nodes_host[i];
      const int64_t pk = pack ? pack[v] : 0;
      const int64_t r = pack ? (pk >> 40) : P->closed_deg_host[v];
      row_deg[(size_t)i] = (int32_t)r;
      be += r;
      n_chunks += (r + CL - 1) / CL;
      if (want_ldsw) bound += pack ? (pk & PACK_MASK) : P->pair_bound_host[v];
    }
    n_ents += be;
    max_batch_ents = std::max(max_batch_ents, be);
  }
  GGAD_REQUIRE(n_ents < (1LL << 31) - 1);
  int mode = train ? P->hop2 : 0;
  if (mode == 1 && (max_batch_ents >= 65536 || bound >= (1LL << 31) - 1 || P->n_nodes * (int64_t)P->feat_stride * 4 >= (1LL << 32)))
    mode = 2;
  const int64_t off_bp = 0, off_bep = align4(nb + 1), off_nodes = off_bep + align4(nb + 1), off_labels = off_nodes + align4(rows),
                off_meta = off_labels + align4(rows), off_rpos = off_meta + align4(rows), off_slot = off_rpos + align4(rows),
                off_eptr = off_slot + align4(rows), off_ckp = off_eptr + align4(rows + 1), off_ckrc = off_ckp + align4(rows + 1),
                off_cke0 = off_ckrc + align4(n_chunks), stage_need = off_cke0 + align4(n_chunks);
  const int64_t seg_stride = (n_ents + 63) / 64 * 64;
  const int64_t n_tiles1 = ((P->n_nodes + (1LL << ggad_mb_ldsw_tile_shift()) - 1) >> ggad_mb_ldsw_tile_shift()) + 1;
  info->pair_bound = bound;
  info->n_batches = nb;
  info->n_rows = (int32_t)rows;
  info->n_ents = (int32_t)n_ents;
  info->n_chunks = (int32_t)n_chunks;
  info->mode = mode;
  info->off_batch_ptr = off_bp; info->off_batch_ent_ptr = off_bep; info->off_nodes = off_nodes; info->off_labels = off_labels;
  info->off_pos_meta = off_meta; info->off_row_pos = off_rpos; info->off_row_slot = off_slot; info->off_ent_ptr = off_eptr;
  info->off_row_ck_ptr = off_ckp; info->off_ck_rc = off_ckrc; info->off_ck_e0 = off_cke0;
  info->need_rows = rows; info->need_ents = n_ents; info->need_chunks = n_chunks; info->need_stage = stage_need;
  if (mode == 1) {
    info->need_pairs = bound;
    info->need_items = n_ents + bound / SL;
    info->need_part2 = (2 + (ggad_int_range_deg() == INT32_MAX ? 0 : (int64_t)GGAD_RANGES * SL / GGAD_RANGE_DEG)) * (bound / SL) + 8;
    info->need_seg = ((P->tile_start && P->col_t) ? 2 : 1) * n_tiles1 * seg_stride;
  }
  info->need_cnt2 = (mode == 2 && P->cnt2 == nullptr) ? 1 : 0;
  if (rows > P->rows_cap || n_ents > P->ent_cap || n_chunks > P->ck_cap || stage_need > P->stage_cap || info->need_cnt2 ||
      (mode == 1 && (info->need_pairs > P->pair_cap || info->need_items > P->item_cap || info->need_part2 > P->part2_cap ||
                     info->need_seg > P->seg_cap)))
    return GGAD_E_CAPACITY;
  if (mode == 1) GGAD_REQUIRE(P->seg_t && P->pc && P->items && P->part2);

  const auto tt1 = std::chrono::steady_clock::now();
  hipStream_t st = as_stream(stream);
  hipError_t he = hipEventSynchronize(static_cast<hipEvent_t>(P->stage_event));
  if (he != hipSuccess) { ggad_set_error(he, "mb_plan_build (stage event)"); return GGAD_E_LAUNCH; }
  const auto tt2 = std::chrono::steady_clock::now();
  int32_t *S = P->stage_host;
  int32_t *bp = S + off_bp, *bep = S + off_bep, *nd = S + off_nodes, *lb = S + off_labels, *meta = S + off_meta,
          *rpos = S + off_rpos, *slot = S + off_slot, *eptr = S + off_eptr, *ckp = S + off_ckp, *ckrc = S + off_ckrc,
          *cke0 = S + off_cke0;
  int64_t e = 0, c = 0;
  for (int b = 0; b < nb; ++b) {
    const int r0 = batch_ptr_host[b], r1 = batch_ptr_host[b + 1];
    bp[b] = r0;
    bep[b] = (int32_t)e;
    if (batch_ent_ptr_host_out) batch_ent_ptr_host_out[b] = e;
    int max_r = 0;
    for (int i = r0; i < r1; ++i) {
      const int32_t v = (int32_t)nodes_host[i];
      const int r = row_deg[(size_t)i];
      nd[i] = v;
      slot[i] = b;
      eptr[i] = (int32_t)e;
      ckp[i] = (int32_t)c;
      if (ent_ptr_host_out) ent_ptr_host_out[i] = e;
      for (int k = 0; k < r; k += CL) {
        ckrc[c] = (i << 6) | std::min(CL, r - k);
        cke0[c] = (int32_t)(e + k);
        ++c;
      }
      e += r;
      max_r = std::max(max_r, r);
    }
    if (batch_max_row_host_out) batch_max_row_host_out[b] = max_r;
    if (train) {
      int q = 0;
      for (int pass = 0; pass < 2; ++pass)
        for (int i = r0; i < r1; ++i) {
          const int64_t l = labels_host[i];
          if (l != 0 && l != 1) return GGAD_E_INVALID;
          if ((int)l != pass) continue;
          meta[r0 + q] = (i << 2) | ((int)l << 1);
          rpos[i] = q;
          ++q;
        }
      for (int i = r0; i < r1; ++i) {
        lb[i] = (int32_t)labels_host[i];
        meta[i] |= (int32_t)labels_host[i];
      }
    }
  }
  bp[nb] = (int32_t)rows;
  bep[nb] = (int32_t)e;
  eptr[rows] = (int32_t)e;
  ckp[rows] = (int32_t)c;
  if (batch_ent_ptr_host_out) batch_ent_ptr_host_out[nb] = e;
  if (ent_ptr_host_out) ent_ptr_host_out[rows] = e;
  const auto tt3 = std::chrono::steady_clock::now();
  he = hipMemcpyAsync(P->stage, S, (size_t)stage_need * sizeof(int32_t), hipMemcpyHostToDevice, st);
  if (he != hipSuccess) { ggad_set_error(he, "mb_plan_build (upload)"); return GGAD_E_LAUNCH; }
  he = hipEventRecord(static_cast<hipEvent_t>(P->stage_event), st);
  if (he != hipSuccess) { ggad_set_error(he, "mb_plan_build (stage event record)"); return GGAD_E_LAUNCH; }

  const auto tt4 = std::chrono::steady_clock::now();
  ggad_plan_view V;
  const int32_t *D = P->stage;
  V.batch_ptr = D + off_bp; V.batch_ent_ptr = D + off_bep; V.nodes = D + off_nodes; V.row_slot = D + off_slot;
  V.ent_ptr = D + off_eptr; V.row_ck_ptr = D + off_ckp; V.ck_rc = D + off_ckrc; V.ck_e0 = D + off_cke0;
  V.n_batches = nb; V.n_rows = (int32_t)rows; V.n_ents = (int32_t)n_ents; V.n_chunks = (int32_t)n_chunks;
  V.seg_stride = (int32_t)seg_stride;
  V.pair_bound = bound;
  int rc = ggad_int_hop1(P, V, mode == 1 ? 1 : 0, mode != 2 ? 1 : 0, st);
  if (rc) return rc;
  hipEvent_t ev0 = static_cast<hipEvent_t>(P->ev_gather0), ev1 = static_cast<hipEvent_t>(P->ev_gather1);
  if (mode == 1) rc = ggad_int_ldsw_hop2(P, V, st, ev0, ev1);
  else if (mode == 2) rc = ggad_int_global_hop2(P, V, st, ev0, ev1);
  if (timing) {
    const auto tt5 = std::chrono::steady_clock::now();
    auto us = [](auto a, auto b) { return std::chrono::duration<double, std::micro>(b - a).count(); };
    fprintf(stderr, "[ggad_mb_plan_build] %d batches: sizes %.1f  stage-event wait %.1f  fill %.1f  copy + event %.1f  launches %.1f us (%lld KB staged)\n", nb,
            us(tt0, tt1), us(tt1, tt2), us(tt2, tt3), us(tt3, tt4), us(tt4, tt5), (long long)(stage_need * 4 / 1024));
  }
  return rc;
}

}
```

### ggad_amd/csrc/step_xcd.hip

```cpp
#include <algorithm>
#include <cstdlib>

#include "common.h"
#include <cstddef>
#include "step_common.h"

namespace {

constexpr int GGAD_MAX_DEVICES = 16;
constexpr int XW = 8;
constexpr int XT = XW * GGAD_WAVE;
constexpr int XMAXWG = 32;
constexpr int XMINWG = 18;
constexpr int XFT = 17;

constexpr int XPC = 2;
constexpr int XHUB = 32;
constexpr int XRA = 512;
constexpr int XBT = 256;
constexpr int FCS = GGAD_MAX_D + 1;

struct XcdCtrl {
  unsigned reg[8][16];
  unsigned slot[64];
  unsigned err, survivors, xcc, placed;
  unsigned long long prof[16];
  unsigned done, helpers, pad[2];
};
static_assert(sizeof(XcdCtrl) <= 1020 && sizeof(XcdCtrl) % 16 == 0, "control block is 256 floats of the workspace");
constexpr int XCD_STICKY_WORD = 255;
__device__ __forceinline__ void xcd_fail(XcdCtrl *C, unsigned code) {
  C->err = code;
  atomicCAS(reinterpret_cast<unsigned *>(C) + XCD_STICKY_WORD, 0u, code);
}

struct XcdArgs {
  ggad_mb_step s;
  const int32_t *batch_ptr;
  int n_batches, log_base, ld_o;
  float *loss_log;
  XcdCtrl *ctrl;
  float *pos_scal, *pos_o, *gw_row, *dw_part;
  const int32_t *ck_rec, *pos_rec;
  const int32_t *batch_n0;
  const float *adam_sc;
  ggad_xchg_view X;
  uint32_t xstep0;
  float grad_scale;
  unsigned long long timeout_ticks;
  unsigned launch_id;
  int dbg;
  int nv, want_xcd;
};

__device__ __forceinline__ float cld(const float *p) { return __hip_atomic_load(p, __ATOMIC_RELAXED, __HIP_MEMORY_SCOPE_AGENT); }
struct f2 { float x, y; };
// ... 48 lines not shown
  float a[XKS];
  float b[4];
};
__device__ __forceinline__ void load_piece_raw(const float *__restrict__ xp, int n, int lane, PieceX &P) {
  const int a = lane & 15, g = lane >> 4;
  const unsigned ra = (unsigned)min(a, n - 1) * XFT;
#pragma unroll
  for (int j = 0; j < XKS; ++j) {
    const int f = 4 * j + g;
    P.a[j] = *lane_at(xp, 4u * (ra + (unsigned)(f < XFT ? f : 0)));
  }
#pragma unroll
  for (int v = 0; v < 4; ++v) {
    const int e = 4 * g + v;
    P.b[v] = *lane_at(xp, 4u * ((unsigned)min(e, n - 1) * XFT + (unsigned)a));
  }
}
__device__ __forceinline__ void mask_piece_x(int n, int lane, PieceX &P) {
  const int a = lane & 15, g = lane >> 4;
#pragma unroll
  for (int j = 0; j < XKS; ++j) P.a[j] = (a < n && 4 * j + g < XFT) ? P.a[j] : 0.0f;
#pragma unroll
  for (int v = 0; v < 4; ++v) P.b[v] = 4 * g + v < n ? P.b[v] : 0.0f;
}
__device__ __forceinline__ void load_piece_x(const float *__restrict__ xp, int n, int lane, PieceX &P) {
  load_piece_raw(xp, n, lane, P);
  __builtin_amdgcn_sched_barrier(0);
  mask_piece_x(n, lane, P);
}
__device__ __forceinline__ void piece_fwd(const PieceX &P, const float (&WB)[XKS][XNT], f4 (&h)[XNT]) {
#pragma unroll
  for (int t = 0; t < XNT; ++t) h[t] = f4{0.0f, 0.0f, 0.0f, 0.0f};
#pragma unroll
  for (int j = 0; j < XKS; ++j)
#pragma unroll
    for (int t = 0; t < XNT; ++t) h[t] = __builtin_amdgcn_mfma_f32_16x16x4f32(P.a[j], WB[j][t], h[t], 0, 0, 0);
}

__device__ __forceinline__ float lds_matvec(const float *m, int stride, float v) {
  float a = 0.0f;
#pragma unroll
  for (int c = 0; c < GGAD_MAX_D; c += 16) {
    float fv[16];
#pragma unroll
    for (int k = 0; k < 16; ++k) fv[k] = m[(c + k) * stride];
    __builtin_amdgcn_sched_barrier(0);
#pragma unroll
    for (int k = 0; k < 16; ++k) a = fmaf(fv[k], rl(v, c + k), a);
    __builtin_amdgcn_sched_barrier(0);
  }
  return a;
}

constexpr int REC = 8;
struct RowIn { float H1, NB, Gl, pp, nbq, c2, xr; };

__device__ __forceinline__ void adam_apply(float *__restrict__ params, float *__restrict__ m, float *__restrict__ v, ParamLayout L,
                                           int i, float p, float mi, float vi, float g, float wd, float step_size, float bc2s) {
  g = fmaf(wd, p, g);
  mi = fmaf(g - mi, 0.1f, mi);
  vi = fmaf(0.001f * g, g, vi * 0.999f);
  const float denom = sqrtf(vi) / bc2s + 1e-8f;
  p = p - step_size * (mi / denom);
  const int D = L.D, F = L.F;
  int it = -1;
  if (i >= L.o_W() && i < L.o_fc()) {
    const int u = i - L.o_W(); const int d = u / F, f = u - d * F;
    it = L.o_Wt() + f * D + d;
  } else if (i >= L.o_fc()) {
    const int u = i - L.o_fc(); const int d = u / D, d2 = u - d * D;
    it = L.o_fcT() + d2 * D + d;
  }
  *lane_at(params, 4u * (unsigned)i) = p; *lane_at(m, 4u * (unsigned)i) = mi; *lane_at(v, 4u * (unsigned)i) = vi;
  if (it >= 0) *lane_at(params, 4u * (unsigned)it) = p;
}

template <int MODE, int DT>
__global__ void __launch_bounds__(XT) k_train_chunk_xcd(XcdArgs A) {
  __shared__ int s_rank;
  __shared__ float wt_lds[XFT * GGAD_MAX_D];
  __shared__ float w_lds[GGAD_MAX_D];
  __shared__ float fct[GGAD_MAX_D * FCS];
  __shared__ float accw[XW][XFT * XLS];
  __shared__ int ra_lds[XRA];
  __shared__ float t_lds[8];
  __shared__ float sc[2];
  __shared__ int hub_first[2 * XW], hub_n[2 * XW], hub_any;
  __shared__ float hub_part[XW][GGAD_WAVE];
  __shared__ int bt_row0[XBT + 1], bt_ck0[XBT + 1], bt_n0[XBT + 1];
  XcdCtrl *C = A.ctrl;
  if (threadIdx.x == 0) {
    unsigned xcc;
    asm volatile("s_getreg_b32 %0, hwreg(HW_REG_XCC_ID)" : "=s"(xcc));
    xcc &= 7u;
    int r = -1;
    if ((int)xcc == A.want_xcd) {
      r = (int)__hip_atomic_fetch_add(&C->reg[xcc][0], 1u, __ATOMIC_RELAXED, __HIP_MEMORY_SCOPE_AGENT);
      const unsigned long long t0 = wall_clock64();
      while (r < A.nv && cldu(&C->reg[xcc][0]) < (unsigned)A.nv) {
        __builtin_amdgcn_s_sleep(2);
        if (cldu(&C->err) != 0 || wall_clock64() - t0 > A.timeout_ticks) { xcd_fail(C, 2); C->done = 1; r = -1; break; }
      }
      if (r >= A.nv) { xcd_fail(C, 3); r = -1; }
      if (r == 0) {
        C->survivors = (unsigned)A.nv; C->xcc = xcc;
        __hip_atomic_store(&C->placed, A.launch_id, __ATOMIC_RELEASE, __HIP_MEMORY_SCOPE_AGENT);
      }
// ... 540 lines not shown
            nbr[u] = cld(lane_at(S.nbar + (int64_t)ra * D, d4));
          }
#pragma unroll
          for (int u = 0; u < EU; ++u) {
            if (j0 + u * XW < n1) {
              const float dzm = on ? dzr[u] : 0.0f;
#pragma unroll
              for (int k = 0; k < 3; ++k) gf[k] = fmaf(rl(dzm, min(ddk[k], GGAD_MAX_D - 1)), nbr[u], gf[k]);
            }
          }
        }
      }
      if (vw < XFT) {
#pragma unroll
        for (int k = 0; k < PWN; ++k) gW += (wid * PWN + k < nv) ? pw[k] : 0.0f;
      } else if (vw == XFT) {
        for (int i0 = wid; i0 < B; i0 += XW * EU) {
          float gr[EU];
#pragma unroll
          for (int u = 0; u < EU; ++u) gr[u] = cld(lane_at(A.gw_row + (int64_t)min(i0 + u * XW, B - 1) * GGAD_WAVE, lane4));
#pragma unroll
          for (int u = 0; u < EU; ++u) gw += (i0 + u * XW < B) ? gr[u] : 0.0f;
        }
      }
      asm volatile("" : "+v"(ap), "+v"(am), "+v"(av));
      __syncthreads();
      accw[wid][lane] = gW; accw[wid][64 + lane] = gw;
#pragma unroll
      for (int k = 0; k < 3; ++k) accw[wid][128 + 64 * k + lane] = gf[k];
      __syncthreads();
      if (pidx >= 0) {
        float g = 0.0f;
#pragma unroll
        for (int k = 0; k < XW; ++k) g += accw[k][sel + lane];
        *lane_at(S.grads, 4u * (unsigned)pidx) = g;
        if (MODE == 2) g = xchg_sum(A.X, A.xstep0 + (uint32_t)b + 1u, pidx, g) * A.grad_scale;
        adam_apply(params, S.exp_avg, S.exp_avg_sq, L, pidx, ap, am, av, g, S.weight_decay, sc[0], sc[1]);
      }
    }
    XCD_TICK(6)
    XCD_BARRIER()
    XCD_TICK(7)
    if (more) {
#pragma unroll
      for (int j = 0; j < XPC; ++j) { recv[j] = recn[j]; xc[j] = xn[j]; mask_piece_x(piece_n(recv[j]), lane, xc[j]); }
      posv = posn;
    }
  }
  if (prof_on && rank == prof_rank && threadIdx.x == prof_thread)
    for (int k = 0; k < 16; ++k) C->prof[k] = prof_lds[k];
  if (rank == 0 && threadIdx.x == 0) C->done = 1;
}

struct XcdPrepArgs {
  const int32_t *batch_ptr, *ent_ptr, *row_ck_ptr, *ck_rc, *ck_e0, *ent_own, *labels, *pos_meta, *row_pos;
  float *x2;
  int32_t *ck_rec, *pos_rec, *batch_n0;
  float *adam_sc;
  const int32_t *step_counter;
  float lr;
  int n_batches, n_rows, n_pieces, n_ents;
  unsigned *ctrl_clear;
  int ctrl_words;
};
__global__ void __launch_bounds__(256) k_xcd_prep(XcdPrepArgs P) {
  const int tid = blockIdx.x * 256 + threadIdx.x;
  if (P.ctrl_clear && tid < P.ctrl_words) P.ctrl_clear[tid] = 0u;
  auto batch_row0 = [&](int row) {
    int lo = 0, hi = P.n_batches;
    while (hi - lo > 1) { const int mid = (lo + hi) >> 1; if (P.batch_ptr[mid] <= row) lo = mid; else hi = mid; }
    return P.batch_ptr[lo];
  };
  if (P.adam_sc && tid < P.n_batches) {
    const double ts = (double)(*P.step_counter + tid + 1);
    const double bc1 = 1.0 - pow(0.9, ts), bc2 = 1.0 - pow(0.999, ts);
    P.adam_sc[2 * tid] = (float)((double)P.lr / bc1);
    P.adam_sc[2 * tid + 1] = (float)sqrt(bc2);
  }
  if (tid < P.n_pieces) {
    const int c = tid;
    const int rc = P.ck_rc[c], row = rc >> 6;
    const int row0 = batch_row0(row);
    const int q1 = P.row_pos[row];
    int32_t *o = P.ck_rec + (int64_t)c * REC;
    o[0] = rc;
    o[1] = P.ck_e0[c];
    o[2] = (P.labels[row] & 1) | ((c == P.row_ck_ptr[row]) ? 2 : 0) | ((P.pos_meta[row0 + q1] & 1) << 2);
    o[3] = P.ent_ptr[row + 1] - P.ent_ptr[row];
    o[4] = q1;
    o[5] = P.pos_meta[row];
    o[6] = 0; o[7] = 0;
  }
  if (tid < P.n_rows) {
    const int row = tid;
    const int meta = P.pos_meta[row];
    int32_t *o = P.pos_rec + (int64_t)row * REC;
    o[0] = meta;
    o[1] = P.row_ck_ptr[row];
    o[2] = P.row_ck_ptr[row + 1] - P.row_ck_ptr[row];
    o[3] = P.ent_ptr[row + 1] - P.ent_ptr[row];
    int sa = 0, ns = 0, rs = 1;
    if (meta & 2) {
      const int src = meta >> 2;
      sa = P.row_ck_ptr[src]; ns = P.row_ck_ptr[src + 1] - sa; rs = P.ent_ptr[src + 1] - P.ent_ptr[src];
    }
    o[4] = sa; o[5] = ns; o[6] = rs; o[7] = 0;
    int lo = 0, hi = P.n_batches;
    while (hi - lo > 1) { const int mid = (lo + hi) >> 1; if (P.batch_ptr[mid] <= row) lo = mid; else hi = mid; }
    const int r0 = P.batch_ptr[lo], r1 = P.batch_ptr[lo + 1];
    if ((meta & 2) && (row == r0 || !(P.pos_meta[row - 1] & 2))) P.batch_n0[lo] = row - r0;
    if (!(meta & 2) && row == r1 - 1) P.batch_n0[lo] = r1 - r0;
  }
  const int f = min((int)(threadIdx.x & 31), XFT - 1);
  const bool fl = (threadIdx.x & 31) < XFT;
  const int64_t stride = ((int64_t)gridDim.x * 256) >> 5;
  for (int64_t e0 = tid >> 5; e0 < P.n_ents; e0 += 4 * stride) {
    int64_t e[4];
    int o[4];
    float v[4];
#pragma unroll
    for (int q = 0; q < 4; ++q) { e[q] = min(e0 + q * stride, (int64_t)P.n_ents - 1); o[q] = P.ent_own[e[q]]; }
#pragma unroll
    for (int q = 0; q < 4; ++q) v[q] = P.x2[(int64_t)o[q] * XFT + f];
#pragma unroll
    for (int q = 0; q < 4; ++q)
      if (fl && e0 + q * stride < P.n_ents && o[q] != (int)e[q]) P.x2[e[q] * XFT + f] = v[q];
  }
}

struct XcdWarmArgs {
  XcdCtrl *ctrl;
  const int32_t *batch_ptr, *ent_ptr, *row_ck_ptr, *ck_rc, *ck_e0, *ent_own, *labels, *pos_meta, *row_pos;
  const float *x1, *x2;
  int n_batches, ahead;
  unsigned launch_id;
  unsigned long long timeout_ticks;
};
constexpr int XWARM = 8;

__device__ __forceinline__ void warm_range(const void *base, int64_t byte0, int64_t byte1, int r, int lane) {
  const char *p = reinterpret_cast<const char *>(base);
  const int64_t l0 = byte0 >> 7, l1 = (byte1 + 127) >> 7;
  for (int64_t l = l0 + r + (int64_t)XWARM * lane; l < l1; l += (int64_t)XWARM * GGAD_WAVE) {
    const int v = *reinterpret_cast<const volatile int *>(p + (l << 7));
    asm volatile("" ::"v"(v));
  }
}

__global__ void __launch_bounds__(GGAD_WAVE) k_xcd_warm(XcdWarmArgs P) {
  XcdCtrl *C = P.ctrl;
  const int lane = lane_id();
  unsigned xcc;
  asm volatile("s_getreg_b32 %0, hwreg(HW_REG_XCC_ID)" : "=s"(xcc));
  xcc &= 7u;
  const unsigned long long t0 = wall_clock64();
  while (__hip_atomic_load(&C->placed, __ATOMIC_ACQUIRE, __HIP_MEMORY_SCOPE_AGENT) != P.launch_id) {
    __builtin_amdgcn_s_sleep(8);
    if (cldu(&C->done) != 0 || cldu(&C->err) != 0 || wall_clock64() - t0 > P.timeout_ticks) return;
  }
  if (cldu(&C->xcc) != xcc) return;
  int r = 0;
  if (lane == 0) r = (int)__hip_atomic_fetch_add(&C->helpers, 1u, __ATOMIC_RELAXED, __HIP_MEMORY_SCOPE_AGENT);
  r = __builtin_amdgcn_readfirstlane(r);
  if (r >= XWARM) return;
  for (int s = 0; s < P.n_batches; ++s) {
// ... 13 lines not shown
    warm_range(P.pos_meta, (int64_t)row0 * 4, (int64_t)row1 * 4, r, lane);
    warm_range(P.row_pos, (int64_t)row0 * 4, (int64_t)row1 * 4, r, lane);
    warm_range(P.ent_ptr, (int64_t)row0 * 4, (int64_t)row1 * 4 + 4, r, lane);
    warm_range(P.row_ck_ptr, (int64_t)row0 * 4, (int64_t)row1 * 4 + 4, r, lane);
  }
}

}

__global__ void k_xcd_probe(int32_t *out) {
  if (threadIdx.x == 0) {
    unsigned xcc;
    asm volatile("s_getreg_b32 %0, hwreg(HW_REG_XCC_ID)" : "=s"(xcc));
    out[blockIdx.x] = (int32_t)(xcc & 7u);
  }
}

extern "C" {

int32_t ggad_mb_xcd_grid(void) { return 8 * XMAXWG; }

int ggad_xcd_first_of_stream(int32_t *first_host, ggad_stream_t stream) {
  GGAD_REQUIRE(first_host);
  int32_t *d = nullptr;
  if (hipMalloc(&d, 16 * sizeof(int32_t)) != hipSuccess) return GGAD_E_LAUNCH;
  hipStream_t st = as_stream(stream);
  int32_t h[16];
  int rc = GGAD_OK;
  k_xcd_probe<<<dim3(16), dim3(GGAD_WAVE), 0, st>>>(d);
  if (hipGetLastError() != hipSuccess || hipMemcpyAsync(h, d, sizeof(h), hipMemcpyDeviceToHost, st) != hipSuccess ||
      hipStreamSynchronize(st) != hipSuccess)
    rc = GGAD_E_LAUNCH;
  (void)hipFree(d);
  if (rc != GGAD_OK) return rc;
  for (int b = 0; b < 16; ++b)
    if (h[b] != ((h[0] + b) & 7)) return GGAD_E_INVALID;
  *first_host = h[0];
  return GGAD_OK;
}

int64_t ggad_mb_xcd_workspace_elems(int32_t max_rows, int32_t D, int32_t F, int64_t rows_cap, int64_t pieces_cap) {
  if (max_rows < 1 || D < 1 || F < 1 || rows_cap < 0 || pieces_cap < 0) return 0;
  const int64_t ld = ((int64_t)max_rows + 3) / 4 * 4;
  return 256 + (int64_t)max_rows * 8 + 8 * ld + (int64_t)max_rows * GGAD_WAVE + (int64_t)XMAXWG * F * GGAD_WAVE +
         (rows_cap + pieces_cap + 2) * REC + 3 * (rows_cap + 1);
}

int64_t ggad_mb_xcd_record_elems(int64_t rows_cap, int64_t pieces_cap) {
  if (rows_cap < 0 || pieces_cap < 0) return 0;
  return (rows_cap + pieces_cap + 2) * REC + (rows_cap + 1);
}

namespace {
inline void record_views(int32_t *recs, int64_t rows_cap, int64_t pieces_cap, int32_t *&pos_rec, int32_t *&ck_rec, int32_t *&batch_n0) {
  pos_rec = recs;
  ck_rec = recs + (rows_cap + 1) * REC;
  batch_n0 = recs + (rows_cap + pieces_cap + 2) * REC;
}
int launch_records(const ggad_mb_step &s, int32_t n_batches, const int32_t *batch_ptr_dev, int32_t n_rows, int32_t n_pieces, int32_t n_ents,
                   int32_t *pos_rec, int32_t *ck_rec, int32_t *batch_n0, float *adam_sc, hipStream_t st, void *ctrl_clear = nullptr) {
  XcdPrepArgs Q;
  Q.ctrl_clear = static_cast<unsigned *>(ctrl_clear);
  Q.ctrl_words = (int)(sizeof(XcdCtrl) / sizeof(unsigned));
  Q.batch_ptr = batch_ptr_dev; Q.ent_ptr = s.ent_ptr; Q.row_ck_ptr = s.row_ck_ptr; Q.ck_rc = s.ck_rc; Q.ck_e0 = s.ck_e0;
  Q.ent_own = s.ent_own; Q.labels = s.labels; Q.pos_meta = s.pos_meta; Q.row_pos = s.row_pos;
  Q.x2 = const_cast<float *>(s.x2);
  Q.ck_rec = ck_rec; Q.pos_rec = pos_rec; Q.batch_n0 = batch_n0;
  Q.adam_sc = adam_sc; Q.step_counter = s.step_counter; Q.lr = s.lr;
  Q.n_batches = n_batches; Q.n_rows = n_rows; Q.n_pieces = n_pieces; Q.n_ents = n_ents;
  const int64_t work = std::max<int64_t>(std::max<int64_t>(std::max<int64_t>(std::max<int64_t>(n_rows, n_pieces), (int64_t)n_ents * 8), n_batches),
                                         ctrl_clear ? Q.ctrl_words : 0);
  const unsigned blocks = (unsigned)std::min<int64_t>((work + 255) / 256, 8192);
  k_xcd_prep<<<dim3(blocks > 0 ? blocks : 1), dim3(256), 0, st>>>(Q);
  GGAD_CHECK_LAUNCH("mb_train_chunk_xcd (records)");
  return GGAD_OK;
}
}

int ggad_mb_xcd_prepare(const ggad_mb_step *tmpl, int32_t n_batches, const int32_t *batch_ptr_dev, int32_t n_rows, int32_t n_pieces,
                        int32_t n_ents, int64_t rows_cap, int64_t pieces_cap, int32_t *records, ggad_stream_t stream) {
  GGAD_REQUIRE(tmpl && batch_ptr_dev && records && n_batches >= 0 && n_rows >= 0 && n_pieces >= 0 && n_ents >= 0);
  GGAD_REQUIRE(n_rows <= rows_cap && n_pieces <= pieces_cap && (int64_t)n_ents * XFT < ((int64_t)1 << 31));
  const ggad_mb_step &s = *tmpl;
  GGAD_REQUIRE(s.x2 && s.ent_ptr && s.ent_own && s.labels && s.pos_meta && s.row_pos && s.row_ck_ptr && s.ck_rc && s.ck_e0 && s.F == XFT);
  if (n_batches == 0) return GGAD_OK;
  int32_t *pos_rec, *ck_rec, *batch_n0;
  record_views(records, rows_cap, pieces_cap, pos_rec, ck_rec, batch_n0);
  return launch_records(s, n_batches, batch_ptr_dev, n_rows, n_pieces, n_ents, pos_rec, ck_rec, batch_n0, nullptr, as_stream(stream));
}

int ggad_mb_train_chunk_xcd(const ggad_mb_step *tmpl, int32_t n_batches, const int32_t *batch_ptr_dev, int32_t max_rows,
                            int32_t n_rows, int32_t n_pieces, int32_t n_ents, int64_t rows_cap, int64_t pieces_cap, float *loss_log,
                            int32_t log_base, float *workspace, float grad_scale, ggad_xchg *xchg, int32_t n_wg, const int32_t *records,
                            ggad_stream_t stream) {
  GGAD_REQUIRE(tmpl && batch_ptr_dev && loss_log && workspace && n_batches >= 0 && log_base >= 0 && max_rows >= 1);
  GGAD_REQUIRE(n_rows >= 0 && n_pieces >= 0 && n_ents >= 0 && n_rows <= rows_cap && n_pieces <= pieces_cap);
  GGAD_REQUIRE((int64_t)n_ents * XFT < ((int64_t)1 << 31) && (int64_t)n_pieces * 64 < ((int64_t)1 << 31));
  const ggad_mb_step &s = *tmpl;
  GGAD_REQUIRE(s.params && s.exp_avg && s.exp_avg_sq && s.grads && s.step_counter && s.x1 && s.x2 && s.ent_ptr && s.ent_own &&
               s.labels && s.pos_meta && s.row_pos && s.h1 && s.nbar && s.gen && s.dz && s.row_ck_ptr && s.ck_rc && s.ck_e0 &&
               s.chunk_part);
  GGAD_REQUIRE(s.F == XFT && s.D >= 1 && s.D <= GGAD_MAX_D && ((uintptr_t)workspace & 15) == 0);
  GGAD_REQUIRE(max_rows <= (1 << 24));
  if (n_batches == 0) return GGAD_OK;
  XcdArgs A;
  A.s = s;
  A.batch_ptr = batch_ptr_dev;
  A.n_batches = n_batches; A.log_base = log_base;
  A.ld_o = (max_rows + 3) / 4 * 4;
  A.loss_log = loss_log;
  A.ctrl = reinterpret_cast<XcdCtrl *>(workspace);
// ... 113 lines not shown
```

### ggad_amd/minibatch.py

```python
from __future__ import annotations

import ctypes
import os
import sys
import time
from typing import Callable, Optional, Sequence

import numpy as np
import torch

from . import _lib
from ._lib import call, ptr
from .graph import DeviceGraph


def _i32(n, device):
    return torch.empty(int(max(n, 1)), dtype=torch.int32, device=device)


def _f32(n, device):
    return torch.empty(int(max(n, 1)), dtype=torch.float32, device=device)


_BUILD_TIMING = bool(os.environ.get("GGAD_BUILD_TIMING"))
# ... 57 lines not shown
        return base[r0:r0 + nb].reshape(-1)
    except (AttributeError, IndexError, TypeError):
        return None


def _check_i32(x: int) -> None:
    if x >= 2 ** 31:
        raise ValueError("chunk too large for int32 entry indices; use fewer batches per chunk")


class BatchChunk:

    HOP2_MODES = {"ldsw": 1, "global": 2}

    def __init__(self, graph: DeviceGraph, feat: torch.Tensor, embed_dim: int, max_batches: int,
                 rows_cap: int, ent_cap: int, train: bool = True, feat_dim: Optional[int] = None,
                 hop2: str = "ldsw", node_major: bool = True):
        self.lib = _lib.load()
        self.g = graph
        self.feat = feat
        self.stride = int(feat.shape[1])
        self.F = int(feat_dim) if feat_dim is not None else self.stride
        if hop2 not in self.HOP2_MODES:
            raise ValueError("hop2 must be 'ldsw' (LDS counting, default) or 'global' (device atomics)")
        self.hop2 = hop2
        self.node_major = bool(node_major)
        self.xcd_skip = -1
        self.D = int(embed_dim)
        self.dev = feat.device
        self.train = bool(train)
        self.max_batches = int(max_batches)
        _check_i32(self.max_batches * graph.n)
        d = self.dev
        self.cnt1 = torch.zeros(self.max_batches * graph.n, dtype=torch.int32, device=d)
        self.own1 = torch.zeros(self.max_batches * graph.n, dtype=torch.int32, device=d)
        self.cnt2 = None
        if self.train and self.hop2 == "global":
            self.cnt2 = torch.zeros(self.max_batches * graph.n, dtype=torch.int32, device=d)
        self.counters = torch.zeros(int(self.lib.ggad_mb_plan_counter_elems()), dtype=torch.int32, device=d)
        self.cl = int(self.lib.ggad_mb_chunk_len())
        self.part_stride = max(64, self.F)
        self.generation = 0
        self.rows_cap = self.ent_cap = self.ck_cap = self.stage_cap = 0
        self.pair_cap = self.item_cap = self.part2_cap = self.seg_cap = 0
        self._stage_event = ctypes.c_void_p()
        _lib.check(self.lib.ggad_event_create(0, ctypes.byref(self._stage_event)), "ggad_event_create")
        self.info = _lib.MbPlanInfo()
        self.plan = _lib.MbPlan()
        self.gather2_events = None
        self.tile_events = None
        self.n_batches = self.n_rows = self.n_ents = self.n_chunks = 0
        self.last_hop2 = "none"
        self.build_count = 0
        self.x2 = self.pc = self.part2 = self.seg_t = self.items = self.grp = None
        if self.train and self.hop2 == "ldsw":
            self.node_head = torch.zeros(graph.n, dtype=torch.int32, device=d)
        self._alloc(rows_cap, ent_cap, ent_cap // self.cl + rows_cap + 8, 0, 0, 0, 0, 0)
        self._bp_host = np.zeros(self.max_batches + 1, dtype=np.int32)
        self._bep_host = np.zeros(self.max_batches + 1, dtype=np.int64)
        self._bmr_host = np.zeros(self.max_batches, dtype=np.int32)

    @property
    def batch_ptr_host(self) -> np.ndarray:
        return self._bp_host[:self.n_batches + 1]

    @property
    def batch_ent_host(self) -> np.ndarray:
        return self._bep_host[:self.n_batches + 1]

    @property
    def batch_max_row(self) -> np.ndarray:
        return self._bmr_host[:self.n_batches]

    @property
    def ent_ptr_host(self) -> np.ndarray:
        return self._ep_host[:self.n_rows + 1]

    def __del__(self):
        try:
            if getattr(self, "_stage_event", None) is not None and self._stage_event.value:
                self.lib.ggad_event_destroy(self._stage_event)
        except Exception:
            pass

    def _alloc(self, rows, ents, chunks, stage, pairs, items, part2, seg) -> None:
        d = self.dev
        if self.generation > 0 and d.type == "cuda":
            torch.cuda.synchronize(d)
        grow = lambda need, have: int(need * 1.25) + 64 if need > have else have
        rows_cap, ent_cap, ck_cap = grow(rows, self.rows_cap), grow(ents, self.ent_cap), grow(chunks, self.ck_cap)
        stage_need = max(stage, 2 * (self.max_batches + 8) + 7 * (rows_cap + 8) + 2 * (ck_cap + 8))
        if rows_cap != self.rows_cap:
            self.rows_cap = rows_cap
            self.x1 = _f32(rows_cap * self.F, d)
            self._ep_host = np.zeros(rows_cap + 1, dtype=np.int64)
            if self.train:
                n = rows_cap * self.D
                self.h1, self.nbar, self.gen = _f32(n, d), _f32(n, d), _f32(n, d)
                self.dz, self.coef_a, self.coef_g = _f32(n, d), _f32(n, d), _f32(n, d)
        if ent_cap != self.ent_cap:
            self.ent_cap = ent_cap
            self.ent_col, self.ent_slot, self.ent_row = _i32(ent_cap, d), _i32(ent_cap, d), _i32(ent_cap, d)
            self.ent_own, self.ent_c1 = _i32(ent_cap, d), _i32(ent_cap, d)
            if self.train:
                self.x2 = _f32(ent_cap * self.F, d)
                if self.hop2 == "ldsw":
# ... 51 lines not shown
        P.pair_cap, P.item_cap, P.part2_cap, P.seg_cap = self.pair_cap, self.item_cap, self.part2_cap, self.seg_cap
        P.feat_dim, P.feat_stride, P.max_batches, P.rows_cap = self.F, self.stride, self.max_batches, self.rows_cap
        P.ck_part_stride = self.part_stride
        P.train, P.hop2, P.node_major = int(self.train), self.HOP2_MODES[self.hop2], int(self.node_major)
        P.mean_nbr_deg = float(g.mean_nbr_deg)
        P.xcd_skip = int(getattr(self, "xcd_skip", -1))

    def build(self, batches: Sequence[np.ndarray], labels: Optional[Sequence[np.ndarray]] = None) -> None:
        nb = len(batches)
        if nb > self.max_batches or nb == 0:
            raise ValueError(f"chunk holds 1..{self.max_batches} batches, got {nb}")
        self._t_build0 = time.perf_counter()
        bp = self._bp_host
        nodes = _rows_as_flat(batches)
        if nodes is not None and (not self.train or labels is not None):
            lab = _rows_as_flat(labels) if self.train else None
            if not self.train or (lab is not None and len(lab) == len(nodes)):
                w = len(batches[0])
                bp[:nb + 1] = np.arange(0, (nb + 1) * w, w, dtype=np.int32) if w > 0 else 0
                if w == 0:
                    raise ValueError("empty batch")
                self.build_arrays(nodes, bp, nb, lab)
                return
        sizes = np.fromiter((len(b) for b in batches), dtype=np.int64, count=nb)
        if (sizes == 0).any():
            raise ValueError("empty batch")
        nodes = np.concatenate(batches).astype(np.int64, copy=False)
        lab = None
        if self.train:
            if labels is None:
                raise ValueError("training chunk needs labels")
            lab = np.concatenate(labels).astype(np.int64, copy=False)
            if len(lab) != len(nodes):
                raise ValueError("labels / batches length mismatch")
        bp[0] = 0
        np.cumsum(sizes, out=bp[1:nb + 1])
        self.build_arrays(nodes, bp, nb, lab)

    def build_arrays(self, nodes: np.ndarray, bp: np.ndarray, nb: int, lab: Optional[np.ndarray]) -> None:
        if bp is not self._bp_host:
            self._bp_host[:nb + 1] = bp[:nb + 1]
            bp = self._bp_host
        rows = int(bp[nb])
        if rows > self.rows_cap:
            self._alloc(rows, 0, 0, 0, 0, 0, 0, 0)
        P, I = self.plan, self.info
        P.xcd_skip = int(self.xcd_skip)
        if self.gather2_events is not None:
            P.ev_gather0, P.ev_gather1 = self.gather2_events
        else:
            P.ev_gather0 = P.ev_gather1 = None
        P.ev_tile0, P.ev_tile1 = self.tile_events if self.tile_events is not None else (None, None)
        stream = _lib.current_stream()
        for attempt in range(3):
            if _BUILD_TIMING:
                print("[BatchChunk.build] python before the native call %.1f us" % ((time.perf_counter() - self._t_build0) * 1e6), file=sys.stderr)
            rc = self.lib.ggad_mb_plan_build(ctypes.byref(P), _addr(nodes), _addr(bp), nb, _addr(lab) if lab is not None else None,
                                             ctypes.byref(I), _addr(self._ep_host), _addr(self._bep_host), _addr(self._bmr_host), stream)
            if rc != -3:
                break
            _check_i32(int(I.need_ents))
            if I.need_cnt2 and self.cnt2 is None:
                self.cnt2 = torch.zeros(self.max_batches * self.g.n, dtype=torch.int32, device=self.dev)
            f = 1.1 * min(64.0, self.max_batches / max(1, nb)) if nb < self.max_batches else 1.0
            lim = 1_600_000_000
            if self.dev.type == "cuda":
                free = torch.cuda.mem_get_info(self.dev)[0]
                per_f = 2.0 * int(I.need_pairs) + 48.0 * int(I.need_items) + 4.0 * self.stride * int(I.need_part2) + 1.0
                f = max(1.0, min(f, 0.25 * free / per_f))
            self._alloc(I.need_rows, I.need_ents, I.need_chunks, I.need_stage, max(int(I.need_pairs), min(lim, int(I.need_pairs * f))),
                        max(int(I.need_items), min(lim // 16, int(I.need_items * f))),
                        max(int(I.need_part2), min(lim // 32, int(I.need_part2 * f))), max(int(I.need_seg), int(I.need_seg * min(f, self.ent_cap / max(1, int(I.need_ents))))))
        if rc == -1:
            raise ValueError("ggad_mb_plan_build: a batch node id is out of range, a label is not 0/1, or the plan descriptor is incomplete")
        _lib.check(rc, "ggad_mb_plan_build")
        self.n_batches, self.n_rows, self.n_ents, self.n_chunks = nb, int(I.n_rows), int(I.n_ents), int(I.n_chunks)
        self.last_hop2 = ("none", "ldsw", "global")[int(I.mode)]
        self.build_count += 1
        st = self.stage
        R, C = self.n_rows, self.n_chunks
        self.batch_ptr = st[I.off_batch_ptr:I.off_batch_ptr + nb + 1]
        self.batch_ent_ptr = st[I.off_batch_ent_ptr:I.off_batch_ent_ptr + nb + 1]
        self.nodes = st[I.off_nodes:I.off_nodes + R]
        self.labels = st[I.off_labels:I.off_labels + R]
        self.pos_meta = st[I.off_pos_meta:I.off_pos_meta + R]
        self.row_pos = st[I.off_row_pos:I.off_row_pos + R]
        self.row_slot = st[I.off_row_slot:I.off_row_slot + R]
        self.ent_ptr = st[I.off_ent_ptr:I.off_ent_ptr + R + 1]
        self.row_ck_ptr = st[I.off_row_ck_ptr:I.off_row_ck_ptr + R + 1]
        self.ck_rc = st[I.off_ck_rc:I.off_ck_rc + max(C, 1)]
        self.ck_e0 = st[I.off_ck_e0:I.off_ck_e0 + max(C, 1)]

    def reset(self) -> None:
        """Kept for callers of the previous interface: the plan leaves its counter slots clean by itself."""

    def owner_entries(self) -> torch.Tensor:
        e = torch.arange(self.n_ents, device=self.dev, dtype=torch.int32)
        return e[self.ent_own[:self.n_ents] == e].long()

    def ent_total_ptr(self) -> int:
        return self.ent_ptr.data_ptr() + 4 * self.n_rows

    def batch_rows(self, b: int):
        return int(self.batch_ptr_host[b]), int(self.batch_ptr_host[b + 1])

    def batch_ents(self, b: int):
        return int(self.batch_ent_host[b]), int(self.batch_ent_host[b + 1])

    def max_batch_ents(self) -> int:
        return int(np.diff(self.batch_ent_host).max()) if self.n_batches else 0


def reduce_gradients(grads: torch.Tensor, world_size: int, allreduce: Optional[Callable]) -> float:
    if world_size > 1:
        if allreduce is None:
            raise ValueError("world_size > 1 needs an all-reduce callable")
        allreduce(grads)
    return 1.0 / world_size


class MiniBatchEngine:

    def __init__(self, feat_dim: int, embed_dim: int, device, lr: float = 1e-3, weight_decay: float = 0.007,
                 chain: int = 0, resident: Optional[bool] = None):
        self.lib = _lib.load()
        self.chain = int(chain)
        if self.chain not in (0, 2, 3):
            raise ValueError("chain must be 0, 2 or 3")
        self.F, self.D = int(feat_dim), int(embed_dim)
        import os
        can = int(feat_dim) == 17 and int(embed_dim) <= 64 and self.chain == 0
# ... 113 lines not shown
        self.ensure_capacity(ch, log_base + ch.n_batches)
        stream = _lib.current_stream()
        if self.resident and allreduce is None and (world_size == 1 or exchange is not None) \
                and getattr(ch, "row_ck_ptr", None) is not None:
            s = self.step_desc(ch, 0, log_base)
            recs = None
            if getattr(ch, "xcd_prepared", None) == (ch.build_count, self._xcd_caps):
                recs = ptr(ch.xcd_recs)
            _lib.check(self.lib.ggad_mb_train_chunk_xcd(ctypes.byref(s), ch.n_batches, ptr(ch.batch_ptr), self._xcd_rows,
                                                         ch.n_rows, ch.n_chunks, ch.n_ents, self._xcd_caps[0], self._xcd_caps[1],
                                                         self.loss_log.data_ptr(), log_base, ptr(self.xcd_ws), 1.0 / world_size,
                                                         exchange.handle if exchange is not None else None, int(self.xcd_wgs), recs,
                                                         stream),
                       "ggad_mb_train_chunk_xcd")
            return
        if exchange is not None:
            if self.D > int(self.lib.ggad_max_embed_dim()):
                raise ValueError(f"the one-shot exchange takes emb_size <= {int(self.lib.ggad_max_embed_dim())}; use the all-reduce path")
            s = self.step_desc(ch, 0, log_base)
            bp, ep, mr = ch._bp_host, ch._bep_host, ch._bmr_host
            _lib.check(self.lib.ggad_mb_train_chunk_xchg(ctypes.byref(s), ch.n_batches, bp.ctypes.data, ep.ctypes.data,
                                                         mr.ctypes.data, self.loss_log.data_ptr(), log_base, 1.0 / world_size,
                                                         exchange.handle, stream), "ggad_mb_train_chunk_xchg")
            return
        fuse = 1 if (allreduce is None and world_size == 1) else 0
        if fuse:
            s = self.step_desc(ch, 0, log_base)
            bp, ep, mr = ch._bp_host, ch._bep_host, ch._bmr_host
            _lib.check(self.lib.ggad_mb_train_chunk(ctypes.byref(s), ch.n_batches, bp.ctypes.data, ep.ctypes.data, mr.ctypes.data,
                                                    self.loss_log.data_ptr(), log_base, 1, stream), "ggad_mb_train_chunk")
            return
        scale = 1.0 / world_size
        if world_size > 1 and allreduce is None:
            raise ValueError("world_size > 1 needs an all-reduce callable")
        err = []

        def exchange(_user):
            try:
                if allreduce is not None:
                    allreduce(self.grads)
                return 0
            except BaseException as exc:
                err.append(exc)
                return 1
        cb = _lib.EXCHANGE_CB(exchange)
        s = self.step_desc(ch, 0, log_base)
        bp, ep, mr = ch._bp_host, ch._bep_host, ch._bmr_host
        rc = self.lib.ggad_mb_train_chunk_dp(ctypes.byref(s), ch.n_batches, bp.ctypes.data, ep.ctypes.data, mr.ctypes.data,
                                             self.loss_log.data_ptr(), log_base, scale, cb, None, stream)
        if err:
            raise err[0]
        _lib.check(rc, "ggad_mb_train_chunk_dp")

    def xcd_prepare(self, ch: BatchChunk) -> None:
        if not (self.resident and ch.train and getattr(ch, "row_ck_ptr", None) is not None and ch.n_batches > 0):
            return
        if os.environ.get("GGAD_XCD_PREP_ON_PLAN", "1") == "0":
            return
        caps = self._xcd_caps
        if self.xcd_ws is None or caps[0] < ch.n_rows or caps[1] < ch.n_chunks:
            return
        need = int(self.lib.ggad_mb_xcd_record_elems(*caps))
        recs = getattr(ch, "xcd_recs", None)
        if recs is None or recs.numel() < need:
            if recs is not None:
                torch.cuda.synchronize(self.dev)
            ch.xcd_recs = torch.empty(need, dtype=torch.int32, device=self.dev)
        s = self.step_desc(ch, 0, 0)
        _lib.check(self.lib.ggad_mb_xcd_prepare(ctypes.byref(s), ch.n_batches, ptr(ch.batch_ptr), ch.n_rows, ch.n_chunks, ch.n_ents,
                                                caps[0], caps[1], ptr(ch.xcd_recs), _lib.current_stream()), "ggad_mb_xcd_prepare")
        ch.xcd_prepared = (ch.build_count, caps)

    def xcd_status(self) -> dict:
        if self.xcd_ws is None:
            raise RuntimeError("no XCD-resident launch has run")
        out = (ctypes.c_int64 * 19)()
        _lib.check(self.lib.ggad_mb_xcd_status(ptr(self.xcd_ws), out, _lib.current_stream()), "ggad_mb_xcd_status")
        names = ("A", "bar1", "R", "bar2", "C", "bar3", "E", "bar4")
        return dict(error=int(out[0]), workgroups=int(out[1]), xcc=int(out[2]),
                    phase_us={n: out[3 + k] / 100.0 for k, n in enumerate(names)},
                    sub_us=[out[11 + k] / 100.0 for k in range(8)])

    def set_resident_error(self, code: int = 0) -> None:
        if self.xcd_ws is not None:
            _lib.check(self.lib.ggad_mb_xcd_clear_error(ptr(self.xcd_ws), int(code), _lib.current_stream()), "ggad_mb_xcd_clear_error")

    def check_resident(self) -> None:
        if self.xcd_ws is not None:
            st = self.xcd_status()
            if st["error"]:
                raise RuntimeError(f"ggad_amd: XCD-resident chunk kernel timed out (code {st['error']}, {st['workgroups']} workgroups)")

    def forward_batch(self, ch: BatchChunk, b: int) -> None:
        self.ensure_capacity(ch, 1)
        r0, r1 = ch.batch_rows(b)
        e0, e1 = ch.batch_ents(b)
        call("ggad_mb_project", ptr(self.params), self.D, self.F, ptr(ch.x2), ptr(ch.ent_own), e0, e1 - e0, ptr(self.h2))
        call("ggad_mb_fwd_rows", ptr(self.params), self.D, self.F, ptr(ch.x1), ptr(self.h2), ptr(ch.ent_ptr), ptr(ch.ent_own),
             ptr(ch.labels), r0, r1 - r0, e0, ptr(ch.h1), ptr(ch.nbar), ptr(ch.gen))

    def score_chunk(self, ch: BatchChunk, out: torch.Tensor) -> None:
        call("ggad_mb_score", ptr(self.params), self.D, self.F, ptr(ch.x1), ch.n_rows, ptr(out))

    def losses(self, n: int) -> np.ndarray:
        return self.loss_log[:8 * n].view(n, 8)[:, :4].cpu().numpy()
```

### ggad_amd/trainer.py

```python
from __future__ import annotations

import os
import sys
import time
from typing import Callable, List, Optional, Sequence, Tuple

import numpy as np
import torch

from .graph import DeviceGraph
from .minibatch import BatchChunk, MiniBatchEngine, RowList, reduce_gradients
from .sampler import PyCompatRandom


def _other_llc_cpus():
    import ctypes
    if os.environ.get("GGAD_SAMPLER_LLC", "other") == "same":
        return None
    try:
        here = ctypes.CDLL(None).sched_getcpu()
        allowed = os.sched_getaffinity(0)
        groups = {}
        for cpu in sorted(allowed):
            with open(f"/sys/devices/system/cpu/cpu{cpu}/cache/index3/shared_cpu_list") as fh:
# ... 309 lines not shown
                  gather_hook=None) -> int:
        t_entry = time.perf_counter()
        sizes = self.default_ramp(n_steps)
        pos = [0]
        record = self._replay_begin()

        producer = None
        stream = getattr(self, "_stream", None) if prepared is None else None
        if stream is not None and n_steps > stream["left"]:
            raise RuntimeError("run_steps beyond the end of the running batch stream")
        if prepared is None and stream is None and self.prefetch and len(sizes) > 1:
            import queue
            import threading
            q = queue.Queue(maxsize=2)

            home = _other_llc_cpus()

            def produce():
                try:
                    if home:
                        try:
                            os.sched_setaffinity(threading.get_native_id(), home)
                        except OSError:
                            pass
                    for k in sizes:
                        q.put(self.schedule.next_batches(k, self.sched_rank, self.sched_world))
                except BaseException as exc:
                    q.put(exc)
            producer = threading.Thread(target=produce, daemon=True)
            producer.start()

        def take_raw(k):
            if prepared is not None:
                bn, bl = prepared[0][pos[0]:pos[0] + k], prepared[1][pos[0]:pos[0] + k]
                pos[0] += k
                return bn, bl
            if stream is not None:
                return self._stream_take(k)
            if producer is not None:
                item = q.get()
                if isinstance(item, BaseException):
                    raise item
                return item
            return self.schedule.next_batches(k, self.sched_rank, self.sched_world)

        def take(k):
            bn, bl = take_raw(k)
            if record is not None:
                record[1].extend(bn)
                record[2].extend(bl)
            return bn, bl

        def build(ch, bn, bl):
            ch.build(bn, bl) if gather_hook is None else gather_hook(ch, bn, bl)
            self._t_built = time.perf_counter()
            self.engine.xcd_prepare(ch)

        nodes_seen, done = 0, 0
        split = getattr(self, "resident_split", False)
        if not self.overlap or len(sizes) == 1:
            if split:
                self.chunk.xcd_skip = -1
            timing = os.environ.get("GGAD_RUN_TIMING")
            for k in sizes:
                if timing:
                    ev_a, ev_b = torch.cuda.Event(enable_timing=True), torch.cuda.Event(enable_timing=True)
                    ev_a.record()
                t0 = time.perf_counter()
                bn, bl = take(k)
                t1 = time.perf_counter()
                build(self.chunk, bn, bl)
                t2 = time.perf_counter()
                self.engine.train_chunk(self.chunk, self.allreduce, self.world, log_base=done, exchange=self.exchange)
                if timing:
                    ev_b.record()
                    t3 = time.perf_counter()
                    torch.cuda.synchronize()
                    t4 = time.perf_counter()
                    print("[run_steps] device: first event -> last event %.1f us" % (ev_a.elapsed_time(ev_b) * 1e3), file=sys.stderr)
                    print("[run_steps] %d batches: entry -> loop %.1f  take %.1f  build + xcd_prepare %.1f (build %.1f)  train_chunk call %.1f  device drain %.1f us"
                          % (k, (t0 - t_entry) * 1e6, (t1 - t0) * 1e6, (t2 - t1) * 1e6, (self._t_built - t1) * 1e6, (t3 - t2) * 1e6, (t4 - t3) * 1e6), file=sys.stderr, flush=True)
                nodes_seen += sum(len(b) for b in bn)
                done += k
        else:
            if split:
                for ch in self.chunks:
                    ch.xcd_skip = self._xcd_skip
            outer = torch.cuda.current_stream()
            main = self.hi
            main.wait_stream(outer)
            side = self.side
            built = [torch.cuda.Event(), torch.cuda.Event()]
            freed = [torch.cuda.Event(), torch.cuda.Event()]
            side.wait_stream(main)
            bn, bl = take(sizes[0])
            with torch.cuda.stream(side):
                build(self.chunks[0], bn, bl)
                built[0].record(side)
            for c, k in enumerate(sizes):
                cur, nxt = c % 2, (c + 1) % 2
                nodes_seen += sum(len(b) for b in bn)
                if c + 1 < len(sizes):
                    bn, bl = take(sizes[c + 1])
                    with torch.cuda.stream(side):
                        if c >= 1:
                            side.wait_event(freed[nxt])
# ... 56 lines not shown
```

### include/ggad_hip.h

```cpp
#ifndef GGAD_HIP_H
#define GGAD_HIP_H

#include <stdint.h>

#ifdef __cplusplus
extern "C" {
#endif

#define GGAD_OK 0
#define GGAD_E_INVALID (-1)
#define GGAD_E_LAUNCH (-2)
#define GGAD_E_CAPACITY (-3)
#define GGAD_E_UNSUPPORTED (-4)

typedef void *ggad_stream_t;

int ggad_abi_version(void);
const char *ggad_last_error(void);
int ggad_max_embed_dim(void);
int ggad_max_feat_dim(void);
int ggad_mb_wide_max_embed_dim(void);
int ggad_mb_wide_supported(int32_t D, int32_t F);
int ggad_mb_supported(int32_t D, int32_t F);


int64_t ggad_scan_workspace_elems(int64_t n);
int ggad_exclusive_scan_i32(const int32_t *in, int32_t *out, int64_t n, int32_t *workspace, ggad_stream_t stream);


typedef struct ggad_mb_plan {
  const int32_t *rowptr, *col;
  const float *feat;
  const int32_t *tile_off;
  const int32_t *closed_deg_host;
  const int64_t *pair_bound_host;
  int32_t *stage_host, *stage;
  void *stage_event;
  int32_t *cnt1, *own1, *cnt2;
  int32_t *ent_col, *ent_slot, *ent_row, *ent_own, *ent_c1;
  float *x1, *x2;
  float *ck_part;
  int32_t *own_deg, *own_rp, *pw_base, *seg_t, *node_head, *own_next, *grp, *items, *counters;
  uint16_t *pc;
  float *part2;
  void *ev_gather0, *ev_gather1;
  int64_t n_nodes, ent_cap, ck_cap, pair_cap, item_cap, part2_cap, stage_cap, seg_cap;
  int32_t feat_dim, feat_stride, max_batches, rows_cap, ck_part_stride;
  int32_t train;
  int32_t hop2;
  int32_t node_major;
  float mean_nbr_deg;
  int32_t xcd_skip;
  void *ev_tile0, *ev_tile1;
  const int64_t *node_pack_host;
  const int32_t *tile_start, *col_t;
} ggad_mb_plan;

typedef struct ggad_mb_plan_info {
  int64_t pair_bound;
  int64_t off_batch_ptr, off_batch_ent_ptr, off_nodes, off_labels, off_pos_meta, off_row_pos, off_row_slot, off_ent_ptr,
      off_row_ck_ptr, off_ck_rc, off_ck_e0;
  int64_t need_rows, need_ents, need_chunks, need_pairs, need_items, need_part2, need_stage, need_seg;
  int32_t n_batches, n_rows, n_ents, n_chunks;
  int32_t mode;
  int32_t need_cnt2;
} ggad_mb_plan_info;

int32_t ggad_mb_chunk_len(void);
int32_t ggad_mb_slice_len(void);
int32_t ggad_mb_group_words(void);
int ggad_mb_set_gather_options(int32_t mfma_min_batches, int32_t range_deg);
int32_t ggad_mb_item_words(void);
int32_t ggad_mb_plan_counter_elems(void);
int ggad_mb_plan_build(const ggad_mb_plan *plan, const int64_t *nodes_host, const int32_t *batch_ptr_host, int32_t n_batches,
                       const int64_t *labels_host, ggad_mb_plan_info *info, int64_t *ent_ptr_host_out,
                       int64_t *batch_ent_ptr_host_out, int32_t *batch_max_row_host_out, ggad_stream_t stream);

int ggad_event_create(int32_t timing, void **out);
int ggad_event_destroy(void *event);
int ggad_event_record(void *event, ggad_stream_t stream);
int ggad_event_synchronize(void *event);
int ggad_event_elapsed_ms(void *start, void *stop, float *ms_host);

int ggad_seg_mean(const float *feat, int32_t feat_dim, const int32_t *seg_ptr, const int32_t *seg_col, int32_t n_rows,
                  float *out, ggad_stream_t stream);
int ggad_seg_wsum(const float *feat, int32_t feat_dim, const int32_t *seg_ptr, const int32_t *seg_col, const float *seg_w,
                  int32_t n_rows, float *out, ggad_stream_t stream);

int ggad_recon_cols_f32(const float *a, const float *t, int32_t n_rows, int32_t n_cols, float w_pos, float w_neg, float *loss,
                        float *col_sum, float *da, ggad_stream_t stream);
int ggad_recon_rows_f32(const float *a, const float *t, int64_t n_rows, int32_t n_cols, float *out, ggad_stream_t stream);

int ggad_ocgnn_loss_f32(const float *emb, const int64_t *idx, int64_t n_idx, int32_t h, const float *center, float r, float beta,
                        float *loss, float *score, float *demb, ggad_stream_t stream);

int ggad_adae_gat_alpha_f32(const float *y, const float *a_s, const float *a_d, int32_t n, int32_t F, float *als, float *ald,
                            ggad_stream_t stream);
int ggad_adae_gat_fwd_f32(const int32_t *tptr, const int32_t *tcol, const float *tval, const float *y, const float *als,
                          const float *ald, const float *bias, int32_t n, int32_t F, float *z, float *rmax, float *rsum,
                          ggad_stream_t stream);
int ggad_adae_gat_bwd_f32(const int32_t *tptr, const int32_t *tcol, const float *tval, const int32_t *aptr, const int32_t *acol,
                          const float *aval, const int32_t *tmap, const float *y, const float *als, const float *ald,
                          const float *rmax, const float *rsum, const float *a_s, const float *a_d, const float *g, int32_t n,
                          int32_t F, float *dpre, float *dals, float *dald, float *dy, ggad_stream_t stream);
int64_t ggad_adae_colsum_workspace_elems(int32_t F);
int ggad_adae_colsum_f32(const float *M, const float *w, int64_t n, int32_t F, float *out, float *ws, ggad_stream_t stream);
int64_t ggad_adae_stru_fwd_workspace_elems(int32_t n_rows, int32_t n);
int ggad_adae_stru_fwd_f32(const float *z, int32_t n, int32_t F, const int64_t *rows, int32_t n_rows, const int32_t *rptr,
                           const int32_t *rcol, const float *rval, const float *x, const float *xhat, float *ws, float *s_edge,
                           float *attr, float *stru, float *score, float *loss, ggad_stream_t stream);
int64_t ggad_adae_stru_bwd_workspace_elems(int32_t n_rows, int32_t n, int32_t F);
int ggad_adae_stru_bwd_f32(const float *z, int32_t n, int32_t F, const int64_t *rows, int32_t n_rows, const int32_t *rptr,
                           const int32_t *rcol, const float *rval, const float *s_edge, const int32_t *pos, const int32_t *tptr,
                           const int32_t *trow, const int32_t *tedge, const float *stru, const float *gloss, float *ws, float *dz,
                           ggad_stream_t stream);
int ggad_adae_attr_bwd_f32(const float *x, const float *xhat, const int64_t *rows, int32_t n_rows, int32_t F, const float *attr,
                           const float *gloss, float *dxhat, ggad_stream_t stream);

int32_t ggad_aegis_bn_channels(void);
int32_t ggad_aegis_bn_groups(int64_t M);
int32_t ggad_aegis_bn_rows_per_group(void);
int64_t ggad_aegis_bn_workspace_elems(int64_t M, int32_t C);
int ggad_aegis_bn_fwd_f32(const float *h1, int64_t m1, int64_t ld1, const float *h2, int64_t m2, int64_t ld2, int32_t C,
                          const float *gamma, const float *beta, float eps, float momentum, float *running_mean, float *running_var,
                          int64_t *num_batches_tracked, int32_t act, const int64_t *rows, int64_t n_out, float *y, int64_t ldy,
                          const float *w2, const float *b2, float *p, float *mean, float *invstd, float *ws, int32_t *ticket,
                          ggad_stream_t stream);
int ggad_aegis_bn_bwd_f32(const float *h, int64_t M, int64_t ldh, int32_t C, const float *gamma, const float *beta, const float *mean,
                          const float *invstd, int32_t act, const float *dy, int64_t lddy, const float *w2, const float *p,
// ... 459 lines not shown
```

Baseline: 3.288 million nodes/s.

## Fuse XCD record prep and hop-1 combine into plan-build hop-2 kernels

Adds a plan-build entry point that writes the XCD-resident per-row and per-chunk records inside the hop-2 LDSW pipeline. The hop-1 combine/reset work and the record writing become extra block roles in one kernel alongside the segment transpose. Record writing can also move into a combined gather2 finish kernel, which additionally fills duplicate-entry x2 rows from the partial slots left in own_next. This removes separate xcd_prepare and combine launches per chunk, at the cost of more complex multi-role kernels and reuse of the own_next buffer.

```diff
diff --git a/ggad_amd/_lib.py b/ggad_amd/_lib.py
--- a/ggad_amd/_lib.py
+++ b/ggad_amd/_lib.py
@@ -51,6 +51,7 @@
     "ggad_mb_set_gather_options": (c_int32, [c_int32, c_int32]),
     "ggad_mb_plan_counter_elems": (c_int32, []),
     "ggad_mb_plan_build": (c_int32, [_P, _P, _P, _I, _P, _P, _P, _P, _P, _P]),
+    "ggad_mb_plan_build_records": (c_int32, [_P, _P, _P, _I, _P, _P, _P, _P, _P, _P, _L, _L, _P, _P]),
     "ggad_event_create": (c_int32, [_I, _P]),
     "ggad_event_destroy": (c_int32, [_P]),
     "ggad_event_record": (c_int32, [_P, _P]),
diff --git a/ggad_amd/build.py b/ggad_amd/build.py
--- a/ggad_amd/build.py
+++ b/ggad_amd/build.py
@@ -12,7 +12,7 @@
 STAMP = os.path.join(HERE, ".libggad_hip.stamp")
 SOURCES = ["runtime.cpp", "plan_build.cpp", "exchange.cpp", "sampler.cpp", "sampler_x86.cpp", "spmm_panel_build.cpp", "spmm_ring_build.cpp", "plan.hip", "hop2_ldsw.hip", "step.hip", "step_wide.hip", "step_xcd.hip", "fullgraph.hip", "gemm.hip", "gemm_slab.hip", "mlp.hip", "baselines.hip", "anomalydae.hip", "aegis.hip", "gaan.hip", "dominant.hip", "rng.hip", "pcgnn.hip", "pcgnn_head.hip", "sage.hip", "aegis_mb.hip", "recon_mb.hip", "tam.hip", "tam_nsgt.hip", "rank_metrics.hip", "topk.hip", "select.hip", "explain.hip"]
 HOST_ONLY = {"sampler.cpp", "sampler_x86.cpp", "spmm_panel_build.cpp", "spmm_ring_build.cpp"}
-HEADERS = ["common.h", "handoff.h", "step_common.h", "rank_common.h", "libggad_hip.map", os.path.join("..", "..", "include", "ggad_hip.h")]
+HEADERS = ["common.h", "plan_roles.h", "handoff.h", "step_common.h", "rank_common.h", "libggad_hip.map", os.path.join("..", "..", "include", "ggad_hip.h")]
 FLAGS = ["--offload-arch=gfx950", "-O3", "-std=c++17", "-fPIC", "-ffp-contract=on", "-fno-fast-math",
          "-Wall", "-Wno-unused-function"] + os.environ.get("GGAD_EXTRA_HIPFLAGS", "").split()
 
diff --git a/ggad_amd/csrc/common.h b/ggad_amd/csrc/common.h
--- a/ggad_amd/csrc/common.h
+++ b/ggad_amd/csrc/common.h
@@ -99,9 +99,17 @@
   int32_t seg_stride;
   int64_t pair_bound;
 };
-int ggad_int_hop1(const ggad_mb_plan *P, const ggad_plan_view &V, int ldsw, int reset_now, hipStream_t st);
+struct ggad_plan_fuse {
+  bool after_gather1 = false;
+  int reset_now = 0;
+  bool records_late = false;
+  int32_t *pos_rec = nullptr, *ck_rec = nullptr, *batch_n0 = nullptr;
+  const int32_t *labels = nullptr, *pos_meta = nullptr, *row_pos = nullptr;
+};
+int ggad_int_hop1(const ggad_mb_plan *P, const ggad_plan_view &V, int ldsw, int reset_now, hipStream_t st, bool combine_later = false);
 int ggad_int_global_hop2(const ggad_mb_plan *P, const ggad_plan_view &V, hipStream_t st, hipEvent_t ev0, hipEvent_t ev1);
-int ggad_int_ldsw_hop2(const ggad_mb_plan *P, const ggad_plan_view &V, hipStream_t st, hipEvent_t ev0, hipEvent_t ev1);
+int ggad_int_ldsw_hop2(const ggad_mb_plan *P, const ggad_plan_view &V, hipStream_t st, hipEvent_t ev0, hipEvent_t ev1,
+                       const ggad_plan_fuse &Z = ggad_plan_fuse());
 int ggad_int_range_deg();
 
 int ggad_int_gemm_slab(const float *A, const float *B, float *C, int M, int N, int K, int64_t lda, int64_t sbk, int64_t sbn, int64_t ldc,
diff --git a/ggad_amd/csrc/hop2_ldsw.hip b/ggad_amd/csrc/hop2_ldsw.hip
--- a/ggad_amd/csrc/hop2_ldsw.hip
+++ b/ggad_amd/csrc/hop2_ldsw.hip
@@ -4,6 +4,7 @@
 #include <mutex>
 
 #include "common.h"
+#include "plan_roles.h"
 
 namespace {
 
@@ -120,13 +121,10 @@
 constexpr int TW_BRK = 1536;
 
 constexpr int TT_SLAB = 128;
-__global__ void __launch_bounds__(256) k_seg_transpose(const int32_t *__restrict__ tile_off, const int32_t *__restrict__ tile_start,
-                                                       int n_tiles, const int32_t *__restrict__ ent_own,
-                                                       const int32_t *__restrict__ ent_col, int n_ents, int64_t seg_stride,
-                                                       int32_t *__restrict__ seg_t, int skip) {
-  __shared__ int tl[TT_SLAB][65];
-  unsigned vbx, vgx;
-  if (!ggad_vblock(skip, vbx, vgx)) return;
+__device__ __forceinline__ void seg_transpose_role(unsigned vbx, int (*tl)[65], const int32_t *__restrict__ tile_off,
+                                                   const int32_t *__restrict__ tile_start, int n_tiles,
+                                                   const int32_t *__restrict__ ent_own, const int32_t *__restrict__ ent_col,
+                                                   int n_ents, int64_t seg_stride, int32_t *__restrict__ seg_t) {
   const int p0 = vbx * 64;
   if (p0 >= n_ents) return;
   const int lane = lane_id(), wid = threadIdx.x >> 6;
@@ -163,6 +161,42 @@
     __syncthreads();
   }
   }
+}
+
+__global__ void __launch_bounds__(256) k_seg_transpose(const int32_t *__restrict__ tile_off, const int32_t *__restrict__ tile_start,
+                                                       int n_tiles, const int32_t *__restrict__ ent_own,
+                                                       const int32_t *__restrict__ ent_col, int n_ents, int64_t seg_stride,
+                                                       int32_t *__restrict__ seg_t, int skip) {
+  __shared__ int tl[TT_SLAB][65];
+  unsigned vbx, vgx;
+  if (!ggad_vblock(skip, vbx, vgx)) return;
+  seg_transpose_role(vbx, tl, tile_off, tile_start, n_tiles, ent_own, ent_col, n_ents, seg_stride, seg_t);
+}
+
+__global__ void __launch_bounds__(256) k_after_gather1(int seg_blocks, int c1_blocks, int rec_blocks,
+                                                       const int32_t *__restrict__ tile_off, const int32_t *__restrict__ tile_start,
+                                                       int n_tiles, const int32_t *__restrict__ ent_own,
+                                                       const int32_t *__restrict__ ent_col, int n_ents, int64_t seg_stride,
+                                                       int32_t *__restrict__ seg_t, int row_blocks, int n_rows,
+                                                       const int32_t *__restrict__ row_ck_ptr, const float *__restrict__ part1,
+                                                       int pstride, int F, float *__restrict__ x1, int do_reset,
+                                                       const int32_t *__restrict__ ent_slot, int64_t n_nodes,
+                                                       int32_t *__restrict__ cnt1, ggad_roles::XcdPrepArgs R, int skip) {
+  __shared__ int tl[TT_SLAB][65];
+  unsigned vbx, vgx;
+  if (!ggad_vblock(skip, vbx, vgx)) return;
+  if (vbx < (unsigned)c1_blocks) {
+    ggad_roles::combine1_reset_role(vbx, row_blocks, n_rows, row_ck_ptr, part1, pstride, F, x1, do_reset, n_ents, ent_col, ent_slot,
+                                    n_nodes, cnt1);
+    return;
+  }
+  vbx -= (unsigned)c1_blocks;
+  if (vbx < (unsigned)rec_blocks) {
+    ggad_roles::records_role((int)(vbx * 256u + threadIdx.x), R);
+    return;
+  }
+  vbx -= (unsigned)rec_blocks;
+  if (vbx < (unsigned)seg_blocks) seg_transpose_role(vbx, tl, tile_off, tile_start, n_tiles, ent_own, ent_col, n_ents, seg_stride, seg_t);
 }
 
 __device__ __forceinline__ int block_excl_scan_1024(int v, int *warp_buf, int *total) {
@@ -555,11 +589,11 @@
 
 __global__ void __launch_bounds__(256) k_build_groups(const int32_t *__restrict__ ent_own, const int32_t *__restrict__ ent_col,
                                                       const int32_t *__restrict__ own_deg, int n_ents,
-                                                      int32_t *__restrict__ node_head, const int32_t *__restrict__ own_next,
+                                                      int32_t *__restrict__ node_head, int32_t *own_next,
                                                       const int32_t *__restrict__ tile_off, int n_tiles,
                                                       int32_t *__restrict__ grp, int32_t *__restrict__ items,
                                                       int32_t *__restrict__ big, int32_t *__restrict__ gbnd,
-                                                      int32_t *__restrict__ counters, int range_deg, int skip) {
+                                                      int32_t *__restrict__ counters, int range_deg, int leave_part, int skip) {
   unsigned vbx, vgx;
   if (!ggad_vblock(skip, vbx, vgx)) return;
   const int e = vbx * 256 + threadIdx.x;
@@ -611,7 +645,11 @@
 #pragma unroll
     for (int j = 0; j < 8; ++j) {
       int v = -1;
-      if (cur != 0) { v = cur - 1; cur = own_next[v]; }
+      if (cur != 0) {
+        v = cur - 1;
+        cur = own_next[v];
+        if (leave_part && ns > 1) own_next[v] = pbase + (g * 8 + j) * ns;
+      }
       rec[j] = v;
     }
     rec[8] = pbase + g * 8 * ns;
@@ -763,10 +801,9 @@
 #endif
 }
 
-__global__ void __launch_bounds__(256) k_gather2_combine(const int32_t *__restrict__ grp, const int32_t *__restrict__ counters,
-                                                         const float *__restrict__ part2, int F, float *__restrict__ x2, int skip) {
-  unsigned vbx, vgx;
-  if (!ggad_vblock(skip, vbx, vgx)) return;
+__device__ __forceinline__ void gather2_combine_role(unsigned vbx, unsigned vgx, const int32_t *__restrict__ grp,
+                                                     const int32_t *__restrict__ counters, const float *__restrict__ part2, int F,
+                                                     float *__restrict__ x2) {
   const int lane = lane_id();
   const int n_groups = counters[GGAD_CTR_GROUPS];
   const int rpi = 64 / F;
@@ -787,6 +824,67 @@
       }
     }
   }
+}
+
+__global__ void __launch_bounds__(256) k_gather2_combine(const int32_t *__restrict__ grp, const int32_t *__restrict__ counters,
+                                                         const float *__restrict__ part2, int F, float *__restrict__ x2, int skip) {
+  unsigned vbx, vgx;
+  if (!ggad_vblock(skip, vbx, vgx)) return;
+  gather2_combine_role(vbx, vgx, grp, counters, part2, F, x2);
+}
+
+__device__ __forceinline__ void x2_complete_role(unsigned vbx, const int32_t *__restrict__ ent_own,
+                                                 const int32_t *__restrict__ own_deg, const int32_t *__restrict__ own_part,
+                                                 const float *__restrict__ part2, int F, float *__restrict__ x2, int n_ents,
+                                                 int range_deg) {
+  const int lane = lane_id();
+  const int e = (int)(vbx * 256u + threadIdx.x);
+  int o = e, ns = 1, slot = 0;
+  if (e < n_ents) o = ent_own[e];
+  const bool dup = e < n_ents && o != e;
+  if (dup) {
+    const int deg = own_deg[o];
+    ns = deg > range_deg ? GGAD_RANGES : (deg > SLICE ? (deg + SLICE - 1) / SLICE : 1);
+    if (ns > 1) slot = own_part[o];
+  }
+  unsigned long long todo = __ballot(dup);
+  while (todo) {
+    const int l = __builtin_ctzll(todo);
+    todo &= todo - 1;
+    const int oo = __shfl(o, l, GGAD_WAVE), nn = __shfl(ns, l, GGAD_WAVE), ss = __shfl(slot, l, GGAD_WAVE);
+    const int64_t ee = (int64_t)(e - lane + l);
+    if (lane < F) {
+      float acc;
+      if (nn == 1) {
+        acc = x2[(int64_t)oo * F + lane];
+      } else {
+        acc = 0.0f;
+#pragma unroll 4
+        for (int sl = 0; sl < nn; ++sl) acc += part2[((int64_t)ss + sl) * F + lane];
+      }
+      x2[ee * F + lane] = acc;
+    }
+  }
+}
+
+__global__ void __launch_bounds__(256) k_gather2_finish(int cg, int x2_blocks, const int32_t *__restrict__ grp,
+                                                        const int32_t *__restrict__ counters, const float *__restrict__ part2, int F,
+                                                        float *__restrict__ x2, const int32_t *__restrict__ ent_own,
+                                                        const int32_t *__restrict__ own_deg, const int32_t *__restrict__ own_part,
+                                                        int n_ents, int range_deg, int rec_blocks, ggad_roles::XcdPrepArgs R, int skip) {
+  unsigned vbx, vgx;
+  if (!ggad_vblock(skip, vbx, vgx)) return;
+  if (vbx < (unsigned)x2_blocks) {
+    x2_complete_role(vbx, ent_own, own_deg, own_part, part2, F, x2, n_ents, range_deg);
+    return;
+  }
+  vbx -= (unsigned)x2_blocks;
+  if (vbx < (unsigned)rec_blocks) {
+    ggad_roles::records_role((int)(vbx * 256u + threadIdx.x), R);
+    return;
+  }
+  vbx -= (unsigned)rec_blocks;
+  if (vbx < (unsigned)cg) gather2_combine_role(vbx, (unsigned)cg, grp, counters, part2, F, x2);
 }
 
 __global__ void __launch_bounds__(256) k_gather2_w(const int32_t *__restrict__ col, const float *__restrict__ feat, int F, int stride,
@@ -853,13 +951,39 @@
 
 int ggad_int_range_deg() { return g_range_deg.load() > 0 ? std::max(g_range_deg.load(), GGAD_RANGE_DEG) : INT32_MAX; }
 
-int ggad_int_ldsw_hop2(const ggad_mb_plan *P, const ggad_plan_view &V, hipStream_t st, hipEvent_t ev0, hipEvent_t ev1) {
+int ggad_int_ldsw_hop2(const ggad_mb_plan *P, const ggad_plan_view &V, hipStream_t st, hipEvent_t ev0, hipEvent_t ev1,
+                       const ggad_plan_fuse &Z) {
   if (V.n_ents == 0 || V.n_batches == 0) return GGAD_OK;
   const int n_tiles = (int)((P->n_nodes + TW_TILE - 1) >> TW_SHIFT);
   const int skip = P->xcd_skip >= 0 && P->xcd_skip < 8 ? P->xcd_skip : -1;
   const bool tile_major = P->tile_start != nullptr && P->col_t != nullptr;
-  k_seg_transpose<<<dim3(ggad_skip_grid((unsigned)((V.n_ents + 63) / 64), skip)), dim3(256), 0, st>>>(
-      P->tile_off, tile_major ? P->tile_start : nullptr, n_tiles, P->ent_own, P->ent_col, V.n_ents, V.seg_stride, P->seg_t, skip);
+  const bool with_records = Z.pos_rec != nullptr;
+  ggad_roles::XcdPrepArgs Rl = {};
+  int rec_late = 0;
+  if (with_records && !(Z.after_gather1 && P->node_major && P->feat_dim <= 64)) return GGAD_E_INVALID;
+  if (Z.after_gather1) {
+    const int seg_blocks = (V.n_ents + 63) / 64;
+    const int row_blocks = (V.n_rows + 3) / 4;
+    const int c1_blocks = row_blocks + (Z.reset_now ? (V.n_ents + 255) / 256 : 0);
+    ggad_roles::XcdPrepArgs R = {};
+    int rec_blocks = 0;
+    if (with_records) {
+      R.batch_ptr = V.batch_ptr; R.ent_ptr = V.ent_ptr; R.row_ck_ptr = V.row_ck_ptr; R.ck_rc = V.ck_rc; R.ck_e0 = V.ck_e0;
+      R.labels = Z.labels; R.pos_meta = Z.pos_meta; R.row_pos = Z.row_pos;
+      R.pos_rec = Z.pos_rec; R.ck_rec = Z.ck_rec; R.batch_n0 = Z.batch_n0;
+      R.n_batches = V.n_batches; R.n_rows = V.n_rows; R.n_pieces = V.n_chunks;
+      rec_blocks = (std::max(V.n_rows, V.n_chunks) + 255) / 256;
+    }
+    Rl = R; rec_late = Z.records_late ? rec_blocks : 0;
+    if (Z.records_late) rec_blocks = 0;
+    k_after_gather1<<<dim3(ggad_skip_grid((unsigned)(seg_blocks + c1_blocks + rec_blocks), skip)), dim3(256), 0, st>>>(
+        seg_blocks, c1_blocks, rec_blocks, P->tile_off, tile_major ? P->tile_start : nullptr, n_tiles, P->ent_own, P->ent_col, V.n_ents,
+        V.seg_stride, P->seg_t, row_blocks, V.n_rows, V.row_ck_ptr, P->ck_part, P->ck_part_stride, P->feat_dim, P->x1, Z.reset_now,
+        P->ent_slot, P->n_nodes, P->cnt1, R, skip);
+  } else {
+    k_seg_transpose<<<dim3(ggad_skip_grid((unsigned)((V.n_ents + 63) / 64), skip)), dim3(256), 0, st>>>(
+        P->tile_off, tile_major ? P->tile_start : nullptr, n_tiles, P->ent_own, P->ent_col, V.n_ents, V.seg_stride, P->seg_t, skip);
+  }
   const size_t lds = (size_t)(TW_TILE / 2) * 4 + (size_t)(3 * TW_MAXOWN + 1) * 4 + (size_t)TW_BRK * 4;
   {
     static std::mutex mu;
@@ -890,7 +1014,7 @@
     int32_t *big = P->items + 2 * (int64_t)P->item_cap, *gbnd = P->items + 3 * (int64_t)P->item_cap;
     k_build_groups<<<dim3(ggad_skip_grid((unsigned)((V.n_ents + 255) / 256), skip)), dim3(256), 0, st>>>(
         P->ent_own, P->ent_col, P->own_deg, V.n_ents, P->node_head, P->own_next, P->tile_off, n_tiles, P->grp, P->items, big, gbnd,
-        P->counters, range_deg, skip);
+        P->counters, range_deg, with_records ? 1 : 0, skip);
     const int64_t max_items = (int64_t)V.n_ents + (V.pair_bound > 0 ? V.pair_bound : P->pair_cap) / SLICE;
     static const int env_wg = [] { const char *e = getenv("GGAD_G2_WG_PER_CU"); return e ? atoi(e) : 0; }();
     static const int env_cap = [] { const char *e = getenv("GGAD_G2_TAKE_CAP"); return e ? atoi(e) : 0; }();
@@ -911,7 +1035,13 @@
                                                                                 P->pw_base, P->pc, P->grp, P->items, big, gbnd, P->counters,
                                                                                 P->x2, P->part2, affine, take_cap, skip);
     const unsigned cg = (unsigned)std::min<int64_t>(((int64_t)V.n_ents + 3) / 4, 16384);
-    k_gather2_combine<<<dim3(ggad_skip_grid(cg, skip)), dim3(256), 0, st>>>(P->grp, P->counters, P->part2, F, P->x2, skip);
+    if (with_records) {
+      const unsigned xb = (unsigned)((V.n_ents + 255) / 256);
+      k_gather2_finish<<<dim3(ggad_skip_grid(cg + xb + (unsigned)rec_late, skip)), dim3(256), 0, st>>>(
+          (int)cg, (int)xb, P->grp, P->counters, P->part2, F, P->x2, P->ent_own, P->own_deg, P->own_next, V.n_ents, range_deg, rec_late, Rl, skip);
+    } else {
+      k_gather2_combine<<<dim3(ggad_skip_grid(cg, skip)), dim3(256), 0, st>>>(P->grp, P->counters, P->part2, F, P->x2, skip);
+    }
   } else {
     k_gather2_w<<<dim3(ggad_skip_grid((unsigned)((V.n_ents + 3) / 4), skip)), dim3(256), 0, st>>>(
         P->col, P->feat, F, P->feat_stride, P->ent_own, V.n_ents, P->own_rp, P->own_deg, P->pw_base, P->pc, P->x2, skip);
diff --git a/ggad_amd/csrc/plan.hip b/ggad_amd/csrc/plan.hip
--- a/ggad_amd/csrc/plan.hip
+++ b/ggad_amd/csrc/plan.hip
@@ -1,6 +1,8 @@
 #include "common.h"
+#include "plan_roles.h"
 
 namespace {
+using ggad_roles::reduce_groups;
 
 constexpr int SCAN_T = 256;
 constexpr int SCAN_ITEMS = 8;
@@ -90,12 +92,6 @@
     const float x = (lane_active && src < count) ? feat[(int64_t)jj * F + fbase + f] : 0.0f;
     acc = fmaf(ww, x, acc);
   }
-}
-
-__device__ __forceinline__ float reduce_groups(float acc, int F, int rpi) {
-  float tot = acc;
-  for (int gg = 1; gg < rpi; ++gg) tot += __shfl(acc, (lane_id() + gg * F) & 63, GGAD_WAVE);
-  return tot;
 }
 
 __global__ void __launch_bounds__(256) k_expand(const int32_t *__restrict__ rowptr, const int32_t *__restrict__ col,
@@ -261,40 +257,8 @@
                                                         int32_t *__restrict__ cnt1, int skip) {
   unsigned vbx, vgx;
   if (!ggad_vblock(skip, vbx, vgx)) return;
-  if ((int)vbx >= row_blocks) {
-    if (!do_reset) return;
-    const int e = (vbx - row_blocks) * 256 + threadIdx.x;
-    if (e < n_ents) cnt1[(int64_t)ent_slot[e] * n_nodes + ent_col[e]] = 0;
-    return;
-  }
-  const int row = vbx * 4 + (threadIdx.x >> 6);
-  if (row >= n_rows) return;
-  const int c0 = row_ck_ptr[row];
-  const int nck = row_ck_ptr[row + 1] - c0;
-  if (nck <= 1) return;
-  const int lane = lane_id();
-  const int rpi = F <= 64 ? 64 / F : 1;
-  const int fchunks = F <= 64 ? 1 : (F + 63) / 64;
-  for (int fc = 0; fc < fchunks; ++fc) {
-    const int fbase = fc * 64;
-    const int fw = F <= 64 ? F : min(64, F - fbase);
-    const int g = lane / fw, f = lane - g * fw;
-    float acc = 0.0f;
-    if (g < rpi) {
-      const float *__restrict__ src = part1 + (int64_t)c0 * pstride + fbase + f;
-      int c = g;
-      for (; c + 7 * rpi < nck; c += 8 * rpi) {
-        float v[8];
-#pragma unroll
-        for (int u = 0; u < 8; ++u) v[u] = src[(int64_t)(c + u * rpi) * pstride];
-#pragma unroll
-        for (int u = 0; u < 8; ++u) acc += v[u];
-      }
-      for (; c < nck; c += rpi) acc += src[(int64_t)c * pstride];
-    }
-    const float tot = (F <= 64) ? reduce_groups(acc, fw, rpi) : acc;
-    if (lane < fw) x1[(int64_t)row * F + fbase + lane] = tot;
-  }
+  ggad_roles::combine1_reset_role(vbx, row_blocks, n_rows, row_ck_ptr, part1, pstride, F, x1, do_reset, n_ents, ent_col, ent_slot, n_nodes,
+                                  cnt1);
 }
 
 __global__ void __launch_bounds__(256) k_seg_mean(const float *__restrict__ feat, int F, const int32_t *__restrict__ seg_ptr,
@@ -393,7 +357,7 @@
 
 }
 
-int ggad_int_hop1(const ggad_mb_plan *P, const ggad_plan_view &V, int ldsw, int reset_now, hipStream_t st) {
+int ggad_int_hop1(const ggad_mb_plan *P, const ggad_plan_view &V, int ldsw, int reset_now, hipStream_t st, bool combine_later) {
   if (V.n_chunks == 0) return GGAD_OK;
   const unsigned eb = (unsigned)((V.n_chunks + 15) / 16);
   const int skip = P->xcd_skip >= 0 && P->xcd_skip < 8 ? P->xcd_skip : -1;
@@ -404,6 +368,10 @@
                                               V.ck_e0, V.n_chunks, P->n_nodes, P->cnt1, P->own1, P->ent_col, P->ent_own, P->ent_c1,
                                               P->ck_part, P->ck_part_stride, P->x1, P->rowptr, P->own_deg, P->own_rp, P->pw_base,
                                               P->node_head, P->own_next, P->counters, ldsw, skip);
+  if (combine_later) {
+    GGAD_CHECK_LAUNCH("mb_plan_build (1-hop)");
+    return GGAD_OK;
+  }
   const int row_blocks = (V.n_rows + 3) / 4;
   const int ent_blocks = reset_now ? (V.n_ents + 255) / 256 : 0;
   k_combine1_reset<<<dim3(ggad_skip_grid((unsigned)(row_blocks + ent_blocks), skip)), dim3(256), 0, st>>>(
diff --git a/ggad_amd/csrc/plan_build.cpp b/ggad_amd/csrc/plan_build.cpp
--- a/ggad_amd/csrc/plan_build.cpp
+++ b/ggad_amd/csrc/plan_build.cpp
@@ -7,9 +7,16 @@
 #include <vector>
 
 #include "common.h"
+#include "plan_roles.h"
 
 namespace {
 inline int64_t align4(int64_t x) { return (x + 3) & ~(int64_t)3; }
+
+constexpr int FUSE_AFTER_GATHER1 = 1, FUSE_X2 = 2, FUSE_UPLOAD = 4, FUSE_RECORDS_LATE = 8;
+inline int fuse_mask() {
+  const char *e = getenv("GGAD_ONECHUNK_FUSE");
+  return e && *e ? atoi(e) : (FUSE_AFTER_GATHER1 | FUSE_X2 | FUSE_RECORDS_LATE);
+}
 }
 
 extern "C" {
@@ -50,7 +57,17 @@
 int ggad_mb_plan_build(const ggad_mb_plan *P, const int64_t *nodes_host, const int32_t *batch_ptr_host, int32_t n_batches,
                        const int64_t *labels_host, ggad_mb_plan_info *info, int64_t *ent_ptr_host_out,
                        int64_t *batch_ent_ptr_host_out, int32_t *batch_max_row_host_out, ggad_stream_t stream) {
+  return ggad_mb_plan_build_records(P, nodes_host, batch_ptr_host, n_batches, labels_host, info, ent_ptr_host_out, batch_ent_ptr_host_out,
+                                    batch_max_row_host_out, nullptr, 0, 0, nullptr, stream);
+}
+
+int ggad_mb_plan_build_records(const ggad_mb_plan *P, const int64_t *nodes_host, const int32_t *batch_ptr_host, int32_t n_batches,
+                               const int64_t *labels_host, ggad_mb_plan_info *info, int64_t *ent_ptr_host_out,
+                               int64_t *batch_ent_ptr_host_out, int32_t *batch_max_row_host_out, int32_t *records, int64_t rec_rows_cap,
+                               int64_t rec_pieces_cap, int32_t *records_done, ggad_stream_t stream) {
+  if (records_done) *records_done = 0;
   GGAD_REQUIRE(P && nodes_host && batch_ptr_host && info);
+  GGAD_REQUIRE(!records || (records_done && rec_rows_cap >= 0 && rec_pieces_cap >= 0));
   GGAD_REQUIRE(P->rowptr && P->col && P->feat && P->closed_deg_host && P->stage_host && P->stage && P->stage_event);
   GGAD_REQUIRE(P->cnt1 && P->own1 && P->ent_col && P->ent_slot && P->ent_row && P->ent_own && P->ent_c1 && P->x1 && P->ck_part);
   GGAD_REQUIRE(P->feat_dim >= 1 && P->feat_dim <= GGAD_MAX_F && P->feat_stride >= P->feat_dim && P->n_nodes >= 1);
@@ -112,10 +129,26 @@
   int mode = train ? P->hop2 : 0;
   if (mode == 1 && (max_batch_ents >= 65536 || bound >= (1LL << 31) - 1 || P->n_nodes * (int64_t)P->feat_stride * 4 >= (1LL << 32)))
     mode = 2;
-  const int64_t off_bp = 0, off_bep = align4(nb + 1), off_nodes = off_bep + align4(nb + 1), off_labels = off_nodes + align4(rows),
-                off_meta = off_labels + align4(rows), off_rpos = off_meta + align4(rows), off_slot = off_rpos + align4(rows),
-                off_eptr = off_slot + align4(rows), off_ckp = off_eptr + align4(rows + 1), off_ckrc = off_ckp + align4(rows + 1),
-                off_cke0 = off_ckrc + align4(n_chunks), stage_need = off_cke0 + align4(n_chunks);
+  const int fuse = mode == 1 ? fuse_mask() : 0;
+  const bool split_upload = (fuse & FUSE_UPLOAD) != 0;
+  ggad_plan_fuse Z;
+  Z.after_gather1 = (fuse & FUSE_AFTER_GATHER1) != 0;
+  Z.reset_now = 1;
+  Z.records_late = (fuse & FUSE_RECORDS_LATE) != 0;
+  const bool with_records = records && Z.after_gather1 && (fuse & FUSE_X2) && P->node_major && P->feat_dim <= 64 &&
+                            rows <= rec_rows_cap && n_chunks <= rec_pieces_cap;
+  int64_t off_bp = 0, off_bep = align4(nb + 1), off_nodes = off_bep + align4(nb + 1), off_labels, off_meta, off_rpos, off_slot, off_eptr,
+          off_ckp, off_ckrc, off_cke0, stage_need, first_part;
+  if (!split_upload) {
+    off_labels = off_nodes + align4(rows); off_meta = off_labels + align4(rows); off_rpos = off_meta + align4(rows);
+    off_slot = off_rpos + align4(rows); off_eptr = off_slot + align4(rows); off_ckp = off_eptr + align4(rows + 1);
+    off_ckrc = off_ckp + align4(rows + 1); off_cke0 = off_ckrc + align4(n_chunks); stage_need = off_cke0 + align4(n_chunks);
+    first_part = stage_need;
+  } else {
+    off_slot = off_nodes + align4(rows); off_eptr = off_slot + align4(rows); off_ckp = off_eptr + align4(rows + 1);
+    off_ckrc = off_ckp + align4(rows + 1); off_cke0 = off_ckrc + align4(n_chunks); first_part = off_cke0 + align4(n_chunks);
+    off_labels = first_part; off_meta = off_labels + align4(rows); off_rpos = off_meta + align4(rows); stage_need = off_rpos + align4(rows);
+  }
   const int64_t seg_stride = (n_ents + 63) / 64 * 64;
   const int64_t n_tiles1 = ((P->n_nodes + (1LL << ggad_mb_ldsw_tile_shift()) - 1) >> ggad_mb_ldsw_tile_shift()) + 1;
   info->pair_bound = bound;
@@ -150,6 +183,9 @@
   int32_t *bp = S + off_bp, *bep = S + off_bep, *nd = S + off_nodes, *lb = S + off_labels, *meta = S + off_meta,
           *rpos = S + off_rpos, *slot = S + off_slot, *eptr = S + off_eptr, *ckp = S + off_ckp, *ckrc = S + off_ckrc,
           *cke0 = S + off_cke0;
+  if (split_upload)
+    for (int64_t i = 0; i < rows; ++i)
+      if (labels_host[i] != 0 && labels_host[i] != 1) return GGAD_E_INVALID;
   int64_t e = 0, c = 0;
   for (int b = 0; b < nb; ++b) {
     const int r0 = batch_ptr_host[b], r1 = batch_ptr_host[b + 1];
@@ -174,12 +210,21 @@
       max_r = std::max(max_r, r);
     }
     if (batch_max_row_host_out) batch_max_row_host_out[b] = max_r;
-    if (train) {
+  }
+  bp[nb] = (int32_t)rows;
+  bep[nb] = (int32_t)e;
+  eptr[rows] = (int32_t)e;
+  ckp[rows] = (int32_t)c;
+  if (batch_ent_ptr_host_out) batch_ent_ptr_host_out[nb] = e;
+  if (ent_ptr_host_out) ent_ptr_host_out[rows] = e;
+  auto fill_labels = [&]() -> bool {
+    for (int b = 0; b < nb; ++b) {
+      const int r0 = batch_ptr_host[b], r1 = batch_ptr_host[b + 1];
       int q = 0;
       for (int pass = 0; pass < 2; ++pass)
         for (int i = r0; i < r1; ++i) {
           const int64_t l = labels_host[i];
-          if (l != 0 && l != 1) return GGAD_E_INVALID;
+          if (l != 0 && l != 1) return false;
           if ((int)l != pass) continue;
           meta[r0 + q] = (i << 2) | ((int)l << 1);
           rpos[i] = q;
@@ -190,18 +235,16 @@
         meta[i] |= (int32_t)labels_host[i];
       }
     }
-  }
-  bp[nb] = (int32_t)rows;
-  bep[nb] = (int32_t)e;
-  eptr[rows] = (int32_t)e;
-  ckp[rows] = (int32_t)c;
-  if (batch_ent_ptr_host_out) batch_ent_ptr_host_out[nb] = e;
-  if (ent_ptr_host_out) ent_ptr_host_out[rows] = e;
+    return true;
+  };
+  if (train && !split_upload && !fill_labels()) return GGAD_E_INVALID;
   const auto tt3 = std::chrono::steady_clock::now();
-  he = hipMemcpyAsync(P->stage, S, (size_t)stage_need * sizeof(int32_t), hipMemcpyHostToDevice, st);
+  he = hipMemcpyAsync(P->stage, S, (size_t)first_part * sizeof(int32_t), hipMemcpyHostToDevice, st);
   if (he != hipSuccess) { ggad_set_error(he, "mb_plan_build (upload)"); return GGAD_E_LAUNCH; }
-  he = hipEventRecord(static_cast<hipEvent_t>(P->stage_event), st);
-  if (he != hipSuccess) { ggad_set_error(he, "mb_plan_build (stage event record)"); return GGAD_E_LAUNCH; }
+  if (!split_upload) {
+    he = hipEventRecord(static_cast<hipEvent_t>(P->stage_event), st);
+    if (he != hipSuccess) { ggad_set_error(he, "mb_plan_build (stage event record)"); return GGAD_E_LAUNCH; }
+  }
 
   const auto tt4 = std::chrono::steady_clock::now();
   ggad_plan_view V;
@@ -211,16 +254,32 @@
   V.n_batches = nb; V.n_rows = (int32_t)rows; V.n_ents = (int32_t)n_ents; V.n_chunks = (int32_t)n_chunks;
   V.seg_stride = (int32_t)seg_stride;
   V.pair_bound = bound;
-  int rc = ggad_int_hop1(P, V, mode == 1 ? 1 : 0, mode != 2 ? 1 : 0, st);
+  int rc = ggad_int_hop1(P, V, mode == 1 ? 1 : 0, mode != 2 ? 1 : 0, st, Z.after_gather1);
   if (rc) return rc;
+  auto tt4b = tt4, tt4c = tt4;
+  if (split_upload) {
+    tt4b = std::chrono::steady_clock::now();
+    (void)fill_labels();
+    he = hipMemcpyAsync(P->stage + first_part, S + first_part, (size_t)(stage_need - first_part) * sizeof(int32_t), hipMemcpyHostToDevice, st);
+    if (he != hipSuccess) { ggad_set_error(he, "mb_plan_build (upload of the label tables)"); return GGAD_E_LAUNCH; }
+    he = hipEventRecord(static_cast<hipEvent_t>(P->stage_event), st);
+    if (he != hipSuccess) { ggad_set_error(he, "mb_plan_build (stage event record)"); return GGAD_E_LAUNCH; }
+    tt4c = std::chrono::steady_clock::now();
+  }
+  if (with_records) {
+    ggad_roles::record_views(records, rec_rows_cap, rec_pieces_cap, Z.pos_rec, Z.ck_rec, Z.batch_n0);
+    Z.labels = D + off_labels; Z.pos_meta = D + off_meta; Z.row_pos = D + off_rpos;
+  }
   hipEvent_t ev0 = static_cast<hipEvent_t>(P->ev_gather0), ev1 = static_cast<hipEvent_t>(P->ev_gather1);
-  if (mode == 1) rc = ggad_int_ldsw_hop2(P, V, st, ev0, ev1);
+  if (mode == 1) rc = ggad_int_ldsw_hop2(P, V, st, ev0, ev1, Z);
   else if (mode == 2) rc = ggad_int_global_hop2(P, V, st, ev0, ev1);
+  if (rc == GGAD_OK && with_records) *records_done = 1;
   if (timing) {
     const auto tt5 = std::chrono::steady_clock::now();
     auto us = [](auto a, auto b) { return std::chrono::duration<double, std::micro>(b - a).count(); };
-    fprintf(stderr, "[ggad_mb_plan_build] %d batches: sizes %.1f  stage-event wait %.1f  fill %.1f  copy + event %.1f  launches %.1f us (%lld KB staged)\n", nb,
-            us(tt0, tt1), us(tt1, tt2), us(tt2, tt3), us(tt3, tt4), us(tt4, tt5), (long long)(stage_need * 4 / 1024));
+    fprintf(stderr, "[ggad_mb_plan_build] %d batches: sizes %.1f  stage-event wait %.1f  fill %.1f  copy + event %.1f  launches %.1f us (%lld KB staged)  lead %.1f  labels fill + copy %.1f  fuse %d\n", nb,
+            us(tt0, tt1), us(tt1, tt2), us(tt2, tt3), us(tt3, tt4), us(tt4, tt5), (long long)(stage_need * 4 / 1024), us(tt0, tt4),
+            us(tt4b, tt4c), fuse);
   }
   return rc;
 }
diff --git a/ggad_amd/csrc/plan_roles.h b/ggad_amd/csrc/plan_roles.h
--- /dev/null
+++ b/ggad_amd/csrc/plan_roles.h
@@ -0,0 +1,113 @@
+#pragma once
+#include "common.h"
+
+namespace ggad_roles {
+
+__device__ __forceinline__ float reduce_groups(float acc, int F, int rpi) {
+  float tot = acc;
+  for (int gg = 1; gg < rpi; ++gg) tot += __shfl(acc, (lane_id() + gg * F) & 63, GGAD_WAVE);
+  return tot;
+}
+
+__device__ __forceinline__ void combine1_reset_role(unsigned vbx, int row_blocks, int n_rows, const int32_t *__restrict__ row_ck_ptr,
+                                                    const float *__restrict__ part1, int pstride, int F, float *__restrict__ x1,
+                                                    int do_reset, int n_ents, const int32_t *__restrict__ ent_col,
+                                                    const int32_t *__restrict__ ent_slot, int64_t n_nodes,
+                                                    int32_t *__restrict__ cnt1) {
+  if ((int)vbx >= row_blocks) {
+    if (!do_reset) return;
+    const int e = (vbx - row_blocks) * 256 + threadIdx.x;
+    if (e < n_ents) cnt1[(int64_t)ent_slot[e] * n_nodes + ent_col[e]] = 0;
+    return;
+  }
+  const int row = vbx * 4 + (threadIdx.x >> 6);
+  if (row >= n_rows) return;
+  const int c0 = row_ck_ptr[row];
+  const int nck = row_ck_ptr[row + 1] - c0;
+  if (nck <= 1) return;
+  const int lane = lane_id();
+  const int rpi = F <= 64 ? 64 / F : 1;
+  const int fchunks = F <= 64 ? 1 : (F + 63) / 64;
+  for (int fc = 0; fc < fchunks; ++fc) {
+    const int fbase = fc * 64;
+    const int fw = F <= 64 ? F : min(64, F - fbase);
+    const int g = lane / fw, f = lane - g * fw;
+    float acc = 0.0f;
+    if (g < rpi) {
+      const float *__restrict__ src = part1 + (int64_t)c0 * pstride + fbase + f;
+      int c = g;
+      for (; c + 7 * rpi < nck; c += 8 * rpi) {
+        float v[8];
+#pragma unroll
+        for (int u = 0; u < 8; ++u) v[u] = src[(int64_t)(c + u * rpi) * pstride];
+#pragma unroll
+        for (int u = 0; u < 8; ++u) acc += v[u];
+      }
+      for (; c < nck; c += rpi) acc += src[(int64_t)c * pstride];
+    }
+    const float tot = (F <= 64) ? reduce_groups(acc, fw, rpi) : acc;
+    if (lane < fw) x1[(int64_t)row * F + fbase + lane] = tot;
+  }
+}
+
+constexpr int REC = 8;
+struct XcdPrepArgs {
+  const int32_t *batch_ptr, *ent_ptr, *row_ck_ptr, *ck_rc, *ck_e0, *ent_own, *labels, *pos_meta, *row_pos;
+  float *x2;
+  int32_t *ck_rec, *pos_rec, *batch_n0;
+  float *adam_sc;
+  const int32_t *step_counter;
+  float lr;
+  int n_batches, n_rows, n_pieces, n_ents;
+  unsigned *ctrl_clear;
+  int ctrl_words;
+};
+inline void record_views(int32_t *recs, int64_t rows_cap, int64_t pieces_cap, int32_t *&pos_rec, int32_t *&ck_rec, int32_t *&batch_n0) {
+  pos_rec = recs;
+  ck_rec = recs + (rows_cap + 1) * REC;
+  batch_n0 = recs + (rows_cap + pieces_cap + 2) * REC;
+}
+
+__device__ __forceinline__ void records_role(int tid, const XcdPrepArgs &P) {
+  auto batch_row0 = [&](int row) {
+    int lo = 0, hi = P.n_batches;
+    while (hi - lo > 1) { const int mid = (lo + hi) >> 1; if (P.batch_ptr[mid] <= row) lo = mid; else hi = mid; }
+    return P.batch_ptr[lo];
+  };
+  if (tid < P.n_pieces) {
+    const int c = tid;
+    const int rc = P.ck_rc[c], row = rc >> 6;
+    const int row0 = batch_row0(row);
+    const int q1 = P.row_pos[row];
+    int32_t *o = P.ck_rec + (int64_t)c * REC;
+    o[0] = rc;
+    o[1] = P.ck_e0[c];
+    o[2] = (P.labels[row] & 1) | ((c == P.row_ck_ptr[row]) ? 2 : 0) | ((P.pos_meta[row0 + q1] & 1) << 2);
+    o[3] = P.ent_ptr[row + 1] - P.ent_ptr[row];
+    o[4] = q1;
+    o[5] = P.pos_meta[row];
+    o[6] = 0; o[7] = 0;
+  }
+  if (tid < P.n_rows) {
+    const int row = tid;
+    const int meta = P.pos_meta[row];
+    int32_t *o = P.pos_rec + (int64_t)row * REC;
+    o[0] = meta;
+    o[1] = P.row_ck_ptr[row];
+    o[2] = P.row_ck_ptr[row + 1] - P.row_ck_ptr[row];
+    o[3] = P.ent_ptr[row + 1] - P.ent_ptr[row];
+    int sa = 0, ns = 0, rs = 1;
+    if (meta & 2) {
+      const int src = meta >> 2;
+      sa = P.row_ck_ptr[src]; ns = P.row_ck_ptr[src + 1] - sa; rs = P.ent_ptr[src + 1] - P.ent_ptr[src];
+    }
+    o[4] = sa; o[5] = ns; o[6] = rs; o[7] = 0;
+    int lo = 0, hi = P.n_batches;
+    while (hi - lo > 1) { const int mid = (lo + hi) >> 1; if (P.batch_ptr[mid] <= row) lo = mid; else hi = mid; }
+    const int r0 = P.batch_ptr[lo], r1 = P.batch_ptr[lo + 1];
+    if ((meta & 2) && (row == r0 || !(P.pos_meta[row - 1] & 2))) P.batch_n0[lo] = row - r0;
+    if (!(meta & 2) && row == r1 - 1) P.batch_n0[lo] = r1 - r0;
+  }
+}
+
+}
diff --git a/ggad_amd/csrc/step_xcd.hip b/ggad_amd/csrc/step_xcd.hip
--- a/ggad_amd/csrc/step_xcd.hip
+++ b/ggad_amd/csrc/step_xcd.hip
@@ -2,6 +2,7 @@
 #include <cstdlib>
 
 #include "common.h"
+#include "plan_roles.h"
 #include <cstddef>
 #include "step_common.h"
 
@@ -156,7 +157,9 @@
   return a;
 }
 
-constexpr int REC = 8;
+using ggad_roles::REC;
+using ggad_roles::XcdPrepArgs;
+using ggad_roles::record_views;
 struct RowIn { float H1, NB, Gl, pp, nbq, c2, xr; };
 
 __device__ __forceinline__ void adam_apply(float *__restrict__ params, float *__restrict__ m, float *__restrict__ v, ParamLayout L,
@@ -803,65 +806,16 @@
   if (rank == 0 && threadIdx.x == 0) C->done = 1;
 }
 
-struct XcdPrepArgs {
-  const int32_t *batch_ptr, *ent_ptr, *row_ck_ptr, *ck_rc, *ck_e0, *ent_own, *labels, *pos_meta, *row_pos;
-  float *x2;
-  int32_t *ck_rec, *pos_rec, *batch_n0;
-  float *adam_sc;
-  const int32_t *step_counter;
-  float lr;
-  int n_batches, n_rows, n_pieces, n_ents;
-  unsigned *ctrl_clear;
-  int ctrl_words;
-};
 __global__ void __launch_bounds__(256) k_xcd_prep(XcdPrepArgs P) {
   const int tid = blockIdx.x * 256 + threadIdx.x;
   if (P.ctrl_clear && tid < P.ctrl_words) P.ctrl_clear[tid] = 0u;
-  auto batch_row0 = [&](int row) {
-    int lo = 0, hi = P.n_batches;
-    while (hi - lo > 1) { const int mid = (lo + hi) >> 1; if (P.batch_ptr[mid] <= row) lo = mid; else hi = mid; }
-    return P.batch_ptr[lo];
-  };
   if (P.adam_sc && tid < P.n_batches) {
     const double ts = (double)(*P.step_counter + tid + 1);
     const double bc1 = 1.0 - pow(0.9, ts), bc2 = 1.0 - pow(0.999, ts);
     P.adam_sc[2 * tid] = (float)((double)P.lr / bc1);
     P.adam_sc[2 * tid + 1] = (float)sqrt(bc2);
   }
-  if (tid < P.n_pieces) {
-    const int c = tid;
-    const int rc = P.ck_rc[c], row = rc >> 6;
-    const int row0 = batch_row0(row);
-    const int q1 = P.row_pos[row];
-    int32_t *o = P.ck_rec + (int64_t)c * REC;
-    o[0] = rc;
-    o[1] = P.ck_e0[c];
-    o[2] = (P.labels[row] & 1) | ((c == P.row_ck_ptr[row]) ? 2 : 0) | ((P.pos_meta[row0 + q1] & 1) << 2);
-    o[3] = P.ent_ptr[row + 1] - P.ent_ptr[row];
-    o[4] = q1;
-    o[5] = P.pos_meta[row];
-    o[6] = 0; o[7] = 0;
-  }
-  if (tid < P.n_rows) {
-    const int row = tid;
-    const int meta = P.pos_meta[row];
-    int32_t *o = P.pos_rec + (int64_t)row * REC;
-    o[0] = meta;
-    o[1] = P.row_ck_ptr[row];
-    o[2] = P.row_ck_ptr[row + 1] - P.row_ck_ptr[row];
-    o[3] = P.ent_ptr[row + 1] - P.ent_ptr[row];
-    int sa = 0, ns = 0, rs = 1;
-    if (meta & 2) {
-      const int src = meta >> 2;
-      sa = P.row_ck_ptr[src]; ns = P.row_ck_ptr[src + 1] - sa; rs = P.ent_ptr[src + 1] - P.ent_ptr[src];
-    }
-    o[4] = sa; o[5] = ns; o[6] = rs; o[7] = 0;
-    int lo = 0, hi = P.n_batches;
-    while (hi - lo > 1) { const int mid = (lo + hi) >> 1; if (P.batch_ptr[mid] <= row) lo = mid; else hi = mid; }
-    const int r0 = P.batch_ptr[lo], r1 = P.batch_ptr[lo + 1];
-    if ((meta & 2) && (row == r0 || !(P.pos_meta[row - 1] & 2))) P.batch_n0[lo] = row - r0;
-    if (!(meta & 2) && row == r1 - 1) P.batch_n0[lo] = r1 - r0;
-  }
+  ggad_roles::records_role(tid, P);
   const int f = min((int)(threadIdx.x & 31), XFT - 1);
   const bool fl = (threadIdx.x & 31) < XFT;
   const int64_t stride = ((int64_t)gridDim.x * 256) >> 5;
@@ -981,11 +935,6 @@
 }
 
 namespace {
-inline void record_views(int32_t *recs, int64_t rows_cap, int64_t pieces_cap, int32_t *&pos_rec, int32_t *&ck_rec, int32_t *&batch_n0) {
-  pos_rec = recs;
-  ck_rec = recs + (rows_cap + 1) * REC;
-  batch_n0 = recs + (rows_cap + pieces_cap + 2) * REC;
-}
 int launch_records(const ggad_mb_step &s, int32_t n_batches, const int32_t *batch_ptr_dev, int32_t n_rows, int32_t n_pieces, int32_t n_ents,
                    int32_t *pos_rec, int32_t *ck_rec, int32_t *batch_n0, float *adam_sc, hipStream_t st, void *ctrl_clear = nullptr) {
   XcdPrepArgs Q;
diff --git a/ggad_amd/minibatch.py b/ggad_amd/minibatch.py
--- a/ggad_amd/minibatch.py
+++ b/ggad_amd/minibatch.py
@@ -133,6 +133,8 @@
         self.n_batches = self.n_rows = self.n_ents = self.n_chunks = 0
         self.last_hop2 = "none"
         self.build_count = 0
+        self.record_request = None
+        self.records_built = None
         self.x2 = self.pc = self.part2 = self.seg_t = self.items = self.grp = None
         if self.train and self.hop2 == "ldsw":
             self.node_head = torch.zeros(graph.n, dtype=torch.int32, device=d)
@@ -290,11 +292,18 @@
             P.ev_gather0 = P.ev_gather1 = None
         P.ev_tile0, P.ev_tile1 = self.tile_events if self.tile_events is not None else (None, None)
         stream = _lib.current_stream()
+        req, self.record_request = self.record_request, None
+        done = ctypes.c_int32(0)
         for attempt in range(3):
             if _BUILD_TIMING:
                 print("[BatchChunk.build] python before the native call %.1f us" % ((time.perf_counter() - self._t_build0) * 1e6), file=sys.stderr)
-            rc = self.lib.ggad_mb_plan_build(ctypes.byref(P), _addr(nodes), _addr(bp), nb, _addr(lab) if lab is not None else None,
-                                             ctypes.byref(I), _addr(self._ep_host), _addr(self._bep_host), _addr(self._bmr_host), stream)
+            if req is None:
+                rc = self.lib.ggad_mb_plan_build(ctypes.byref(P), _addr(nodes), _addr(bp), nb, _addr(lab) if lab is not None else None,
+                                                 ctypes.byref(I), _addr(self._ep_host), _addr(self._bep_host), _addr(self._bmr_host), stream)
+            else:
+                rc = self.lib.ggad_mb_plan_build_records(ctypes.byref(P), _addr(nodes), _addr(bp), nb, _addr(lab) if lab is not None else None,
+                                                         ctypes.byref(I), _addr(self._ep_host), _addr(self._bep_host), _addr(self._bmr_host),
+                                                         ptr(req[0]), req[1], req[2], ctypes.byref(done), stream)
             if rc != -3:
                 break
             _check_i32(int(I.need_ents))
@@ -315,6 +324,8 @@
         self.n_batches, self.n_rows, self.n_ents, self.n_chunks = nb, int(I.n_rows), int(I.n_ents), int(I.n_chunks)
         self.last_hop2 = ("none", "ldsw", "global")[int(I.mode)]
         self.build_count += 1
+        if req is not None and done.value:
+            self.records_built = (self.build_count, (req[1], req[2]))
         st = self.stage
         R, C = self.n_rows, self.n_chunks
         self.batch_ptr = st[I.off_batch_ptr:I.off_batch_ptr + nb + 1]
@@ -534,20 +545,41 @@
             raise err[0]
         _lib.check(rc, "ggad_mb_train_chunk_dp")
 
-    def xcd_prepare(self, ch: BatchChunk) -> None:
-        if not (self.resident and ch.train and getattr(ch, "row_ck_ptr", None) is not None and ch.n_batches > 0):
-            return
+    def _xcd_record_block(self, ch: BatchChunk):
+        if not (self.resident and ch.train and getattr(ch, "row_ck_ptr", None) is not None):
+            return None
         if os.environ.get("GGAD_XCD_PREP_ON_PLAN", "1") == "0":
-            return
+            return None
         caps = self._xcd_caps
-        if self.xcd_ws is None or caps[0] < ch.n_rows or caps[1] < ch.n_chunks:
-            return
+        if self.xcd_ws is None:
+            return None
         need = int(self.lib.ggad_mb_xcd_record_elems(*caps))
         recs = getattr(ch, "xcd_recs", None)
         if recs is None or recs.numel() < need:
             if recs is not None:
                 torch.cuda.synchronize(self.dev)
             ch.xcd_recs = torch.empty(need, dtype=torch.int32, device=self.dev)
+        return ch.xcd_recs
+
+    def xcd_attach(self, ch: BatchChunk) -> None:
+        ch.record_request = None
+        if self.F != 17 or not getattr(ch, "train", False):
+            return
+        recs = self._xcd_record_block(ch)
+        if recs is not None:
+            ch.record_request = (recs, int(self._xcd_caps[0]), int(self._xcd_caps[1]))
+
+    def xcd_prepare(self, ch: BatchChunk) -> None:
+        if not (self.resident and ch.train and getattr(ch, "row_ck_ptr", None) is not None and ch.n_batches > 0):
+            return
+        caps = self._xcd_caps
+        if ch.records_built == (ch.build_count, caps):
+            ch.xcd_prepared = (ch.build_count, caps)
+            return
+        if self.xcd_ws is None or caps[0] < ch.n_rows or caps[1] < ch.n_chunks:
+            return
+        if self._xcd_record_block(ch) is None:
+            return
         s = self.step_desc(ch, 0, 0)
         _lib.check(self.lib.ggad_mb_xcd_prepare(ctypes.byref(s), ch.n_batches, ptr(ch.batch_ptr), ch.n_rows, ch.n_chunks, ch.n_ents,
                                                 caps[0], caps[1], ptr(ch.xcd_recs), _lib.current_stream()), "ggad_mb_xcd_prepare")
diff --git a/ggad_amd/trainer.py b/ggad_amd/trainer.py
--- a/ggad_amd/trainer.py
+++ b/ggad_amd/trainer.py
@@ -385,6 +385,7 @@
             return bn, bl
 
         def build(ch, bn, bl):
+            self.engine.xcd_attach(ch)
             ch.build(bn, bl) if gather_hook is None else gather_hook(ch, bn, bl)
             self._t_built = time.perf_counter()
             self.engine.xcd_prepare(ch)
diff --git a/include/ggad_hip.h b/include/ggad_hip.h
--- a/include/ggad_hip.h
+++ b/include/ggad_hip.h
@@ -75,6 +75,10 @@
 int ggad_mb_plan_build(const ggad_mb_plan *plan, const int64_t *nodes_host, const int32_t *batch_ptr_host, int32_t n_batches,
                        const int64_t *labels_host, ggad_mb_plan_info *info, int64_t *ent_ptr_host_out,
                        int64_t *batch_ent_ptr_host_out, int32_t *batch_max_row_host_out, ggad_stream_t stream);
+int ggad_mb_plan_build_records(const ggad_mb_plan *plan, const int64_t *nodes_host, const int32_t *batch_ptr_host, int32_t n_batches,
+                               const int64_t *labels_host, ggad_mb_plan_info *info, int64_t *ent_ptr_host_out,
+                               int64_t *batch_ent_ptr_host_out, int32_t *batch_max_row_host_out, int32_t *records,
+                               int64_t rec_rows_cap, int64_t rec_pieces_cap, int32_t *records_done, ggad_stream_t stream);
 
 int ggad_event_create(int32_t timing, void **out);
 int ggad_event_destroy(void *event);
```

Result: no change. 3.278 million nodes/s (-0.3%).
